# gonewest818/raytrace-clj

Measured on NVIDIA B200. Metric: samples_per_sec, higher is better.
Workload: dtype f32

## Files before the change

raytrace_clj_b200/csrc/rt_api.cu:

```cuda
#include "../../include/raytrace_b200.h"

#include <cuda_runtime.h>
#include <dlfcn.h>
#include <math_constants.h>
#include <nccl.h>

#include <algorithm>
#include <cmath>
#include <cstdio>
#include <cstdlib>
#include <cstring>
#include <atomic>
#include <mutex>
#include <thread>
#include <string>
#include <vector>

#include "rt_bvh_build.cuh"
#include "rt_kernels.cuh"

using namespace rt;

namespace {

constexpr int kR = 4;
constexpr int kBlock = 256;
constexpr int kMinBlocks = 1;
constexpr int kTileCap = 4096;

thread_local std::string g_create_error;

struct DeviceBuffers {
    int dev = 0;
    cudaStream_t stream = nullptr;
    cudaEvent_t ev0 = nullptr, ev1 = nullptr, ev_done = nullptr;
    void* scene_blob = nullptr;
    void* scene_stage = nullptr;
    size_t scene_bytes = 0;
    DevScene sc{};
    float* d_sum = nullptr;
    float* d_mean = nullptr;
    uint8_t* d_rgb8 = nullptr;
    size_t frame_px = 0;
    unsigned long long* d_counters = nullptr;
    struct WaveLane {
        float4* queue = nullptr;
        unsigned long long* best = nullptr;
        uint2* pairs = nullptr;
        uint2* cands = nullptr;
        double* cand_t = nullptr;
        unsigned* cand_count = nullptr;
        WaveState* state = nullptr;
        LaneStatus* h_status = nullptr;
        LaneStatus* d_status = nullptr;
        cudaEvent_t ev_done = nullptr;
        cudaStream_t stream = nullptr;
        cudaStream_t stage_stream = nullptr;
        cudaEvent_t ev_culled = nullptr, ev_shaded = nullptr;
        size_t entries = 0;
        bool best_clean = false;
    } lanes[kMaxLanes];
    cudaEvent_t ev_lane_start = nullptr;
    TraceRec* d_trace = nullptr;
    struct TraceMeta { const char* kernel; int lane, iter; };
    std::vector<TraceMeta> trace_meta;
    void* scratch = nullptr;
    size_t scratch_bytes = 0;
    int sm_count = 0, clock_khz = 0;
    char name[64] = {0};
    float last_ms = 0.f;
    bool timed = false;
    float4* bvh_nodes = nullptr;
    size_t bvh_cap = 0;
    int bvh_builder = 0, bvh_depth = 0;
    long long bvh_build_ns = 0;
    void* bvh_scratch = nullptr;
    size_t bvh_scratch_bytes = 0;
    int* h_bvh_depth = nullptr;
    cudaEvent_t ev_b0 = nullptr, ev_b1 = nullptr;
    void* h_stage = nullptr;
    size_t h_stage_bytes = 0;
    cudaEvent_t ev_r0 = nullptr, ev_r1 = nullptr;
    cudaEvent_t ev_chunk[4] = {};
};

struct NcclApi {
    void* handle = nullptr;
    ncclResult_t (*CommInitAll)(ncclComm_t*, int, const int*) = nullptr;
    ncclResult_t (*CommDestroy)(ncclComm_t) = nullptr;
    ncclResult_t (*Reduce)(const void*, void*, size_t, ncclDataType_t, ncclRedOp_t, int, ncclComm_t, cudaStream_t) = nullptr;
    ncclResult_t (*GroupStart)() = nullptr;
    ncclResult_t (*GroupEnd)() = nullptr;
    const char* (*GetErrorString)(ncclResult_t) = nullptr;
    std::vector<ncclComm_t> comms;
};

}

struct Options {
    int wave_lanes = 2;
    long long wave_capacity = 1ll << 24;
    int cull_claims = 2;
    int cull_ctas_per_sm = 4;
    int cull_shape = 0;
    int light_block = 128;
    long long tail_entries = 1 << 19;
    int tail_ctas_per_sm = 0;
    int tile_records = 1024;
    int direct_spheres = 1;
    int common_origin = 1;
    int reduce = 0;
    int rows = 0;
    int tail_block = 256;
    int tail_rays = 1;
    int tail_solo = 24;
    int tail_lpp = 32;
    int mega_regcap = 0;
    int wave_depth = 2;
    int cull_tc = 1;
    int tc_tiles_per_cta = 0;
    int tc_ctas = 0;
    int bvh_build = 1;
};

struct rt_ctx {
    std::mutex mu;
    std::string err;
    std::vector<DeviceBuffers> devs;
    Options opt;
    bool has_scene = false, has_cam = false;
    int n_spheres = 0;
    int n_total = 0;
    int n_list = 0, n_cull = 0;
    int cull_cap = 0, preloaded = 0;
    int tc_tiles = 0;
    std::vector<std::vector<float>> tc_scratch_rows;
    std::vector<int> tc_row_k;
    int generic = 0;
    int accel = RT_ACCEL_BRUTE_FORCE;
    bool bvh_dirty = true;
    double win_lo = 0.0, win_hi = 0.0;
    std::vector<float> h_c0r, h_c1, h_t0t1;
    std::vector<unsigned> h_flags;
    std::vector<double> h_bs_c0, h_bs_c1, h_bs_r;
    DevCamera cam{};
    std::atomic<uint64_t> n_launches{0};
    std::mutex err_mu;
    bool profile = false;
    double stage_ms[4] = {0, 0, 0, 0};
    double reduce_ms = 0.0;
    std::vector<bool> peer_ok;
    NcclApi nccl;
};

namespace {

int fail(rt_ctx* ctx, int code, const std::string& msg) {
    if (ctx) {
        std::lock_guard<std::mutex> lk(ctx->err_mu);
        ctx->err = msg;
    } else {
        g_create_error = msg;
    }
    return code;
}

#define RT_CUDA(ctx, expr)                                                                          \
    do {                                                                                            \
        cudaError_t e__ = (expr);                                                                   \
        if (e__ != cudaSuccess)                                                                     \
            return fail(ctx, RT_ERR_CUDA, std::string(#expr) + ": " + cudaGetErrorString(e__));     \
    } while (0)

int ensure_scratch(rt_ctx* ctx, DeviceBuffers& d, size_t bytes) {
    if (d.scratch_bytes >= bytes) return RT_OK;
    if (d.scratch) cudaFree(d.scratch);
    d.scratch = nullptr;
    d.scratch_bytes = 0;
    RT_CUDA(ctx, cudaMalloc(&d.scratch, bytes));
    d.scratch_bytes = bytes;
    return RT_OK;
}

int ensure_frame(rt_ctx* ctx, DeviceBuffers& d, size_t px) {
    if (d.frame_px >= px) return RT_OK;
    if (d.d_sum) cudaFree(d.d_sum);
    if (d.d_mean) cudaFree(d.d_mean);
    if (d.d_rgb8) cudaFree(d.d_rgb8);
    d.d_sum = d.d_mean = nullptr;
    d.d_rgb8 = nullptr;
    d.frame_px = 0;
    RT_CUDA(ctx, cudaMalloc(&d.d_sum, px * 3 * sizeof(float)));
    RT_CUDA(ctx, cudaMalloc(&d.d_mean, px * 3 * sizeof(float)));
    RT_CUDA(ctx, cudaMalloc(&d.d_rgb8, px * 3));
    d.frame_px = px;
    return RT_OK;
}


void free_lane(DeviceBuffers::WaveLane& L) {
    if (L.queue) cudaFree(L.queue);
    if (L.best) cudaFree(L.best);
    if (L.pairs) cudaFree(L.pairs);
    if (L.cands) cudaFree(L.cands);
    if (L.cand_t) cudaFree(L.cand_t);
    if (L.cand_count) cudaFree(L.cand_count);
    L.queue = nullptr; L.best = nullptr; L.pairs = nullptr; L.cands = nullptr; L.cand_t = nullptr; L.cand_count = nullptr;
    L.entries = 0;
}

void free_wave(DeviceBuffers& d) {
    for (auto& L : d.lanes) {
        free_lane(L);
        if (L.state) cudaFree(L.state);
        if (L.h_status) cudaFreeHost(L.h_status);
        if (L.ev_done) cudaEventDestroy(L.ev_done);
        if (L.stream) cudaStreamDestroy(L.stream);
        if (L.stage_stream) cudaStreamDestroy(L.stage_stream);
        if (L.ev_culled) cudaEventDestroy(L.ev_culled);
        if (L.ev_shaded) cudaEventDestroy(L.ev_shaded);
        L = DeviceBuffers::WaveLane();
    }
    if (d.ev_lane_start) cudaEventDestroy(d.ev_lane_start);
    d.ev_lane_start = nullptr;
    if (d.d_trace) cudaFree(d.d_trace);
    d.d_trace = nullptr;
}

int ensure_lane(rt_ctx* ctx, DeviceBuffers& d, int lane, size_t entries) {
    DeviceBuffers::WaveLane& L = d.lanes[lane];
    if (!L.state) {
        RT_CUDA(ctx, cudaMalloc(&L.state, sizeof(WaveState)));
        RT_CUDA(ctx, cudaHostAlloc(&L.h_status, sizeof(LaneStatus), cudaHostAllocMapped));
        RT_CUDA(ctx, cudaHostGetDevicePointer((void**)&L.d_status, L.h_status, 0));
        RT_CUDA(ctx, cudaEventCreateWithFlags(&L.ev_done, cudaEventDisableTiming));
        if (lane > 0) RT_CUDA(ctx, cudaStreamCreateWithFlags(&L.stream, cudaStreamNonBlocking));
        int prio_least = 0, prio_greatest = 0;
        RT_CUDA(ctx, cudaDeviceGetStreamPriorityRange(&prio_least, &prio_greatest));
        RT_CUDA(ctx, cudaStreamCreateWithPriority(&L.stage_stream, cudaStreamNonBlocking, prio_greatest));
        RT_CUDA(ctx, cudaEventCreateWithFlags(&L.ev_culled, cudaEventDisableTiming));
        RT_CUDA(ctx, cudaEventCreateWithFlags(&L.ev_shaded, cudaEventDisableTiming));
        if (!d.ev_lane_start) RT_CUDA(ctx, cudaEventCreateWithFlags(&d.ev_lane_start, cudaEventDisableTiming));
    }
    if (L.entries >= entries) return RT_OK;
    free_lane(L);
    RT_CUDA(ctx, cudaMalloc(&L.queue, entries * 2 * 3 * sizeof(float4)));
    RT_CUDA(ctx, cudaMalloc(&L.best, entries * 2 * sizeof(unsigned long long)));
    RT_CUDA(ctx, cudaMalloc(&L.pairs, entries * kPairsPerEntry * sizeof(uint2)));
    const size_t cand_slots = entries * kPairsPerEntry + (size_t)d.sm_count * 8 * 8 * 32;
    RT_CUDA(ctx, cudaMalloc(&L.cands, cand_slots * sizeof(uint2)));
    RT_CUDA(ctx, cudaMalloc(&L.cand_t, cand_slots * sizeof(double)));
    RT_CUDA(ctx, cudaMalloc(&L.cand_count, (size_t)d.sm_count * 8 * 8 * sizeof(unsigned)));
    L.entries = entries;
    L.best_clean = false;
    return RT_OK;
}

size_t align_up(size_t x, size_t a) { return (x + a - 1) / a * a; }

float round_up_f32(double x) {
    float f = (float)x;
    if ((double)f < x) f = nextafterf(f, INFINITY);
    return f;
}

size_t mega_smem_bytes(int cull_cap) { return (size_t)cull_cap * sizeof(float4) + Culler<kR, kBlock>::LIST_BYTES; }

template <typename Kern>
int configure_kernel(rt_ctx* ctx, Kern kern, size_t smem, int* blocks_per_sm) {
    RT_CUDA(ctx, cudaFuncSetAttribute(kern, cudaFuncAttributeMaxDynamicSharedMemorySize, (int)smem));
    int b = 0;
    RT_CUDA(ctx, cudaOccupancyMaxActiveBlocksPerMultiprocessor(&b, kern, kBlock, smem));
    if (b < 1) return fail(ctx, RT_ERR_CUDA, "kernel does not fit on an SM");
    *blocks_per_sm = b;
    return RT_OK;
}

long long env_ll(const char* name, long long dflt) {
    const char* v = getenv(name);
    return (v && *v) ? atoll(v) : dflt;
}
int env_int(const char* name, int dflt) { return (int)env_ll(name, dflt); }

Options options_from_env() {
    Options o;
    o.wave_lanes = env_int("RT_WAVE_LANES", o.wave_lanes);
    o.wave_capacity = env_ll("RT_WAVE_CAPACITY", o.wave_capacity);
    o.cull_claims = env_int("RT_CULL_CLAIMS", o.cull_claims);
    o.cull_ctas_per_sm = env_int("RT_CULL_CTAS_PER_SM", o.cull_ctas_per_sm);
    const char* shape = getenv("RT_CULL_SHAPE");
    if (shape && !strcmp(shape, "128x6")) o.cull_shape = 1;
    if (shape && !strcmp(shape, "256x2")) o.cull_shape = 2;
    o.light_block = env_int("RT_LIGHT_BLOCK", o.light_block);
    o.tail_entries = env_ll("RT_TAIL_ENTRIES", o.tail_entries);
    o.tail_ctas_per_sm = env_int("RT_TAIL_CTAS_PER_SM", o.tail_ctas_per_sm);
    o.tile_records = env_int("RT_TILE_RECORDS", o.tile_records);
    o.direct_spheres = env_int("RT_DIRECT_SPHERES", o.direct_spheres);
    o.common_origin = env_int("RT_COMMON_ORIGIN", o.common_origin);
    o.reduce = env_int("RT_REDUCE", o.reduce);
    o.rows = env_int("RT_ROWS", o.rows);
    o.wave_depth = env_int("RT_WAVE_DEPTH", o.wave_depth);
    o.tail_rays = env_int("RT_TAIL_RAYS", o.tail_rays);
    o.tail_solo = env_int("RT_TAIL_SOLO", o.tail_solo);
    o.tail_lpp = env_int("RT_TAIL_LPP", o.tail_lpp);
    o.tail_block = env_int("RT_TAIL_BLOCK", o.tail_block);
    o.cull_tc = env_int("RT_CULL_TC", o.cull_tc);
    o.tc_tiles_per_cta = env_int("RT_TC_TILES_PER_CTA", o.tc_tiles_per_cta);
    o.tc_ctas = env_int("RT_TC_CTAS", o.tc_ctas);
    o.bvh_build = env_int("RT_BVH_BUILD", o.bvh_build);
    return o;
}

template <int BLOCK, int MINB>
int cull_config(rt_ctx* ctx, size_t* smem, int* bps, void (**kern)(const WaveParams)) {
    *kern = wf_cull<kR, BLOCK, MINB>;
    *smem = (ctx->preloaded ? 2 : 1) * (size_t)ctx->cull_cap * sizeof(float4) + Culler<kR, BLOCK>::LIST_BYTES;
    RT_CUDA(ctx, cudaFuncSetAttribute(*kern, cudaFuncAttributeMaxDynamicSharedMemorySize, (int)*smem));
    RT_CUDA(ctx, cudaOccupancyMaxActiveBlocksPerMultiprocessor(bps, *kern, BLOCK, *smem));
    if (*bps < 1) return fail(ctx, RT_ERR_CUDA, "cull kernel does not fit on an SM");
    return RT_OK;
}

int launch_wave(rt_ctx* ctx, DeviceBuffers& d, const RenderParams& P, unsigned long long, cudaStream_t stream) {
    const Options& opt = ctx->opt;
    void (*cull)(const WaveParams) = nullptr;
    size_t smem = 0;
    int bps = 0, cull_block = 256, rc;
    if (opt.cull_shape == 2) rc = cull_config<256, 2>(ctx, &smem, &bps, &cull);
    else if (opt.cull_shape == 1) { rc = cull_config<128, 6>(ctx, &smem, &bps, &cull); cull_block = 128; }
    else { rc = cull_config<128, 5>(ctx, &smem, &bps, &cull); cull_block = 128; }
    if (rc) return rc;
    const int cull_ctas_env = opt.cull_ctas_per_sm;
    if (cull_ctas_env > 0) bps = std::min(bps, cull_ctas_env);
    const size_t cap_env = (size_t)std::max<long long>(64, opt.wave_capacity);
    const int lanes_env = std::max(1, std::min(kMaxLanes, opt.wave_lanes));
    const int n_lanes = (ctx->profile || P.total_work < 65536) ? 1 : lanes_env;
    const size_t capacity = align_up((size_t)std::min<unsigned long long>(cap_env / n_lanes, (P.total_work + n_lanes - 1) / n_lanes), 32);

    bool done[kMaxLanes] = {};
    const unsigned tail_entries = (unsigned)std::max<long long>(0, opt.tail_entries);
    const bool gen = ctx->generic != 0;
    const bool tail4 = opt.tail_rays == 4;
    const int tail_block = (gen || tail4) ? 256 : (opt.tail_block == 32 || opt.tail_block == 64 || opt.tail_block == 128 ? opt.tail_block : 256);
    const size_t tail_smem = (size_t)ctx->cull_cap * sizeof(float4) +
                             (tail4 ? Culler<4, 256>::LIST_BYTES : (size_t)Culler<1, 256>::LIST_WORDS * tail_block * sizeof(uint32_t));
    int tail_bps = 0;
    void (*k_tail)(const WaveParams) = gen ? wf_tail<256, true, 1> : (tail4 ? wf_tail<256, false, 4> : wf_tail<256, false, 1>);
    if (tail_block == 128) k_tail = wf_tail<128, false, 1>;
    if (tail_block == 64) k_tail = wf_tail<64, false, 1>;
    if (tail_block == 32) k_tail = wf_tail<32, false, 1>;
    void (*k_refine)(const WaveParams) = gen ? wf_refine<true> : wf_refine<false>;
    void (*k_shade)(const WaveParams) = gen ? wf_shade<true> : wf_shade<false>;
    RT_CUDA(ctx, cudaFuncSetAttribute(k_tail, cudaFuncAttributeMaxDynamicSharedMemorySize, (int)tail_smem));
    RT_CUDA(ctx, cudaOccupancyMaxActiveBlocksPerMultiprocessor(&tail_bps, k_tail, tail_block, tail_smem));
    const int tail_auto = (n_lanes > 1 ? 1 : std::max(1, std::min((int)(tail_bps * tail_block / 256), 2))) * (256 / tail_block);
    const int tail_grid = d.sm_count * (opt.tail_ctas_per_sm > 0 ? opt.tail_ctas_per_sm : tail_auto);
    const bool bvh = ctx->accel == RT_ACCEL_BVH;
    void (*k_bvh)(const WaveParams) = gen ? wf_bvh<true> : wf_bvh<false>;
    const bool tail_ok = tail_bps >= 1 && tail_entries > 0 && !ctx->profile && !bvh;
    const bool use_tc = opt.cull_tc != 0 && ctx->tc_tiles > 0 && !bvh && ((ctx->n_list >= tc::MIN_LEAVES && !ctx->generic) || opt.cull_tc == 3);
    const int tc_launch_tiles = std::min(ctx->tc_tiles, (int)tc::MAX_TILES);
    const int tc_slots = tc::slots_for(tc_launch_tiles, 227 * 1024);
    const size_t tc_smem = tc::smem_bytes(tc_launch_tiles, tc_slots);
    if (use_tc) RT_CUDA(ctx, cudaFuncSetAttribute(wf_cull_tc, cudaFuncAttributeMaxDynamicSharedMemorySize, (int)tc_smem));
    const int tc_per_cta = std::max(0, opt.tc_tiles_per_cta);
    const int tc_grid = opt.tc_ctas > 0 ? std::min(opt.tc_ctas, 4 * d.sm_count) : d.sm_count;
    auto launch_tc = [&](const WaveParams& Wl, int per_cta, unsigned ctas, cudaStream_t s_) {
        WaveParams Wt = Wl;
        Wt.claims_per_warp = per_cta;
        Wt.tc_slots = tc_slots;
        for (int t0 = 0, pass = 0; t0 < ctx->tc_tiles; t0 += tc::MAX_TILES, ++pass) {
            Wt.tc_tile0 = t0;
            Wt.tc_launch_tiles = std::min((int)tc::MAX_TILES, ctx->tc_tiles - t0);
            Wt.tc_pass = pass;
            wf_cull_tc<<<ctas, tc::THREADS, tc_smem, s_>>>(Wt);
            if (pass) ctx->n_launches += 1;
        }
    };

    const int light_block = std::max(64, std::min(256, opt.light_block / 32 * 32));
    const int light_grid = d.sm_count * 8 * 256 / light_block;
    const int cull_grid = d.sm_count * bps;
    const int claims_env = std::max(0, opt.cull_claims);
    const int claims = (ctx->profile || !ctx->preloaded || n_lanes < 2 || bvh) ? 0 : claims_env;
    const int cull_warps = cull_block / 32, resident_warps = cull_grid * cull_warps;
    unsigned n_bound[kMaxLanes];
    WaveParams W[kMaxLanes];
    cudaStream_t st[kMaxLanes];
    unsigned long long first = 0;
    for (int l = 0; l < n_lanes; ++l) {
        if ((rc = ensure_lane(ctx, d, l, capacity))) return rc;
        DeviceBuffers::WaveLane& L = d.lanes[l];
        W[l] = WaveParams{};
        W[l].base = P;
        W[l].queue[0] = L.queue;
        W[l].queue[1] = L.queue + 3 * capacity;
        W[l].best_t = L.best;
        W[l].best_key = L.best + L.entries;
        W[l].pairs = L.pairs;
        W[l].cands = L.cands;
        W[l].cand_t = L.cand_t;
        W[l].cand_count = L.cand_count;
        W[l].st = L.state;
        W[l].capacity = (int)capacity;
        W[l].pair_cap = (unsigned)std::min<size_t>(capacity * kPairsPerEntry, 0xfffffff0u);
        W[l].cur = 0;
        W[l].claims_per_warp = claims;
        W[l].resident_warps = claims ? resident_warps : 0;
        W[l].tail_solo = (unsigned)std::max(0, opt.tail_solo);
        W[l].tail_lpp = opt.tail_lpp == 8 ? 8u : (opt.tail_lpp == 16 ? 16u : 32u);
        st[l] = l == 0 ? stream : L.stream;
    }
    static const char* trace_path = getenv("RT_TRACE");
    constexpr int kTraceMax = 8192;
    const bool tracing = trace_path && *trace_path;
    if (tracing) {
        if (!d.d_trace) RT_CUDA(ctx, cudaMalloc(&d.d_trace, kTraceMax * sizeof(TraceRec)));
        static const std::vector<TraceRec> init((size_t)kTraceMax, TraceRec{~0ull, 0ull});
        RT_CUDA(ctx, cudaMemcpyAsync(d.d_trace, init.data(), init.size() * sizeof(TraceRec), cudaMemcpyHostToDevice, stream));
        d.trace_meta.clear();
    }
    auto trace_slot = [&](const char* kernel, int lane, int iter) -> TraceRec* {
        if (!tracing || (int)d.trace_meta.size() >= kTraceMax) return nullptr;
        d.trace_meta.push_back({kernel, lane, iter});
        return d.d_trace + (d.trace_meta.size() - 1);
    };
    int iter_no[kMaxLanes] = {};
    static const bool debug_sync = getenv("RT_DEBUG_SYNC") && *getenv("RT_DEBUG_SYNC") == '1';
    auto dbg = [&](const char* what, int lane, int it) -> int {
        if (!debug_sync) return RT_OK;
        cudaError_t e = cudaDeviceSynchronize();
        if (e != cudaSuccess) return fail(ctx, RT_ERR_CUDA, std::string(what) + " (lane " + std::to_string(lane) + ", iteration " + std::to_string(it) + "): " + cudaGetErrorString(e));
        return RT_OK;
    };
    unsigned count0[kMaxLanes];
    unsigned long long total0 = 0;
    for (int l = 0; l < n_lanes; ++l) {
        count0[l] = (unsigned)std::min<unsigned long long>(capacity, P.total_work - total0);
        total0 += count0[l];
        n_bound[l] = count0[l];
    }
    InitParams I{};
    I.n_lanes = n_lanes;
    I.work_counter = P.work_counter;
    I.counters = P.counters;
    I.total0 = total0;
    I.total_work = P.total_work;
    for (int l = 0; l < n_lanes; ++l) {
        DeviceBuffers::WaveLane& L = d.lanes[l];
        I.st[l] = L.state;
        I.first[l] = first;
        I.count[l] = count0[l];
        first += count0[l];
        if (!L.best_clean) {
            wf_fill_best<<<d.sm_count * 4, 256, 0, stream>>>(L.best, L.best + L.entries, L.entries);
            ctx->n_launches += 1;
        }
        L.best_clean = false;
    }
    wf_init<<<1, 1, 0, stream>>>(I);
    ctx->n_launches += 1;
    RT_CUDA(ctx, cudaGetLastError());
    RT_CUDA(ctx, cudaEventRecord(d.ev_lane_start, stream));
    for (int l = 1; l < n_lanes; ++l) RT_CUDA(ctx, cudaStreamWaitEvent(st[l], d.ev_lane_start, 0));

    const int depth = std::max(1, std::min(16, opt.wave_depth));
    int enq[kMaxLanes] = {}, seen[kMaxLanes] = {};
    bool tailed[kMaxLanes] = {};
    for (int l = 0; l < n_lanes; ++l) {
        DeviceBuffers::WaveLane& L = d.lanes[l];
        memset(L.h_status, 0, sizeof(LaneStatus));
        W[l].status = L.d_status;
        if (count0[l] == 0) done[l] = true;
    }
    std::vector<cudaEvent_t> evs;
    unsigned idle_spins = 0;
    for (;;) {
        bool progressed = false, all_done = true;
        for (int l = 0; l < n_lanes; ++l) {
            if (done[l]) continue;
            all_done = false;
            DeviceBuffers::WaveLane& L = d.lanes[l];
            while (!tailed[l] && enq[l] - seen[l] < depth) {
                cudaEvent_t e[5] = {nullptr, nullptr, nullptr, nullptr, nullptr};
                if (ctx->profile)
                    for (auto& x : e) { RT_CUDA(ctx, cudaEventCreate(&x)); evs.push_back(x); }
                if (ctx->profile) cudaEventRecord(e[0], st[l]);
                W[l].iter = (unsigned)(enq[l] + 1);
                const bool tc_now = use_tc && !(enq[l] == 0 && P.common_origin && opt.cull_tc == 2);
                if (bvh) {
                    W[l].trace = trace_slot("bvh", l, iter_no[l]);
                    k_bvh<<<light_grid, 128, 0, st[l]>>>(W[l]);
                    if (ctx->profile) { cudaEventRecord(e[1], st[l]); cudaEventRecord(e[2], st[l]); cudaEventRecord(e[3], st[l]); }
                    W[l].trace = trace_slot("shade", l, iter_no[l]);
                    k_shade<<<light_grid, light_block, 0, st[l]>>>(W[l]);
                    if (ctx->profile) cudaEventRecord(e[4], st[l]);
                    ctx->n_launches -= 2;
                } else if (claims) {
                    W[l].trace = trace_slot("cull", l, iter_no[l]);
                    if (debug_sync) {
                        WaveState hs{};
                        cudaMemcpy(&hs, W[l].st, sizeof hs, cudaMemcpyDeviceToHost);
                        fprintf(stderr, "lane %d iteration %d cur %d: in flight %u fresh %u | other queue %u %u | mode %u exhausted %u npairs %u\n", l, enq[l], W[l].cur,
                                hs.cnt[W[l].cur][0], hs.cnt[W[l].cur][1], hs.cnt[W[l].cur ^ 1][0], hs.cnt[W[l].cur ^ 1][1], hs.mode, hs.exhausted, hs.npairs);
                    }
                    if (tc_now) {
                        const unsigned tiles = (n_bound[l] + tc::TILE_M - 1) / tc::TILE_M;
                        const unsigned ctas = tc_per_cta ? (tiles + (unsigned)tc_per_cta - 1u) / (unsigned)tc_per_cta : (unsigned)tc_grid;
                        launch_tc(W[l], tc_per_cta, std::max(1u, ctas), st[l]);
                    } else {
                    const unsigned items = n_bound[l] / (32u * kR) + 2u * (unsigned)resident_warps + 8u;
                    const unsigned ctas = (items + (unsigned)(cull_warps * claims) - 1u) / (unsigned)(cull_warps * claims);
                    cull<<<ctas, cull_block, smem, st[l]>>>(W[l]);
                    }
                    if ((rc = dbg(tc_now ? "wf_cull_tc" : "wf_cull", l, enq[l]))) return rc;
                    RT_CUDA(ctx, cudaEventRecord(L.ev_culled, st[l]));
                    RT_CUDA(ctx, cudaStreamWaitEvent(L.stage_stream, L.ev_culled, 0));
                    W[l].trace = trace_slot("refine", l, iter_no[l]);
                    k_refine<<<light_grid, light_block, 0, L.stage_stream>>>(W[l]);
                    if ((rc = dbg("wf_refine", l, enq[l]))) return rc;
                    W[l].trace = trace_slot("tiebreak", l, iter_no[l]);
                    wf_tiebreak<<<light_grid, light_block, 0, L.stage_stream>>>(W[l]);
                    if ((rc = dbg("wf_tiebreak", l, enq[l]))) return rc;
                    W[l].trace = trace_slot("shade", l, iter_no[l]);
                    k_shade<<<light_grid, light_block, 0, L.stage_stream>>>(W[l]);
                    if ((rc = dbg("wf_shade", l, enq[l]))) return rc;
                    RT_CUDA(ctx, cudaEventRecord(L.ev_shaded, L.stage_stream));
                    RT_CUDA(ctx, cudaStreamWaitEvent(st[l], L.ev_shaded, 0));
                } else {
                    W[l].trace = trace_slot("cull", l, iter_no[l]);
                    if (tc_now) {
                        launch_tc(W[l], 0, (unsigned)tc_grid, st[l]);
                    } else {
                        cull<<<cull_grid, cull_block, smem, st[l]>>>(W[l]);
                    }
                    if (ctx->profile) cudaEventRecord(e[1], st[l]);
                    W[l].trace = trace_slot("refine", l, iter_no[l]);
                    k_refine<<<light_grid, light_block, 0, st[l]>>>(W[l]);
                    if (ctx->profile) cudaEventRecord(e[2], st[l]);
                    W[l].trace = trace_slot("tiebreak", l, iter_no[l]);
                    wf_tiebreak<<<light_grid, light_block, 0, st[l]>>>(W[l]);
                    if (ctx->profile) cudaEventRecord(e[3], st[l]);
                    W[l].trace = trace_slot("shade", l, iter_no[l]);
                    k_shade<<<light_grid, light_block, 0, st[l]>>>(W[l]);
                    if (ctx->profile) cudaEventRecord(e[4], st[l]);
                }
                RT_CUDA(ctx, cudaGetLastError());
                W[l].cur ^= 1;
                ++iter_no[l];
                ctx->n_launches += 4;
                ++enq[l];
                progressed = true;
            }
        }
        if (all_done) break;
        for (int l = 0; l < n_lanes; ++l) {
            if (done[l]) continue;
            DeviceBuffers::WaveLane& L = d.lanes[l];
            const volatile LaneStatus* hs = L.h_status;
            const unsigned seq = hs->seq;
            if ((int)seq == seen[l] && hs->mode != MODE_DONE) continue;
            std::atomic_thread_fence(std::memory_order_acquire);
            const unsigned n_next = hs->n_next, n_fresh = hs->n_fresh, exhausted = hs->exhausted, mode = hs->mode;
            if (hs->seq != seq) continue;
            seen[l] = (int)seq;
            progressed = true;
            if (exhausted) n_bound[l] = std::min(n_bound[l], n_next);
            if (mode == MODE_DONE) { done[l] = true; continue; }
            if (tail_ok && !tailed[l] && exhausted && n_fresh == 0 && n_next <= tail_entries) {
                W[l].iter = (unsigned)(enq[l] + 1);
                W[l].trace = trace_slot("tail", l, iter_no[l]);
                k_tail<<<tail_grid, tail_block, tail_smem, st[l]>>>(W[l]);
                if ((rc = dbg("wf_tail", l, enq[l]))) return rc;
                RT_CUDA(ctx, cudaGetLastError());
                ctx->n_launches += 1;
                tailed[l] = true;
            }
        }
        if (!progressed) {
            if (++idle_spins > 200) {
                if (cudaSuccess != cudaPeekAtLastError()) RT_CUDA(ctx, cudaGetLastError());
                if (idle_spins > 20000 && (idle_spins % 1000) == 0) {
                    for (int l = 0; l < n_lanes; ++l)
                        if (!done[l] && cudaStreamQuery(st[l]) == cudaSuccess && d.lanes[l].h_status->seq == (unsigned)seen[l] &&
                            enq[l] > seen[l])
                            return fail(ctx, RT_ERR_CUDA, "wavefront lane finished its queue without reporting status");
                }
                std::this_thread::yield();
            }
        } else {
            idle_spins = 0;
        }
    }
    for (int l = 1; l < n_lanes; ++l) {
        RT_CUDA(ctx, cudaEventRecord(d.lanes[l].ev_done, st[l]));
        RT_CUDA(ctx, cudaStreamWaitEvent(stream, d.lanes[l].ev_done, 0));
    }
    for (int l = 0; l < n_lanes; ++l) d.lanes[l].best_clean = true;
    if (ctx->profile) {
        RT_CUDA(ctx, cudaStreamSynchronize(stream));
        for (size_t i = 0; i + 4 < evs.size(); i += 5)
            for (int sgi = 0; sgi < 4; ++sgi) {
                float ms = 0.f;
                if (cudaEventElapsedTime(&ms, evs[i + sgi], evs[i + sgi + 1]) == cudaSuccess) ctx->stage_ms[sgi] += ms;
            }
        for (auto x : evs) cudaEventDestroy(x);
    }
    return RT_OK;
}

int launch_params(rt_ctx* ctx, DeviceBuffers& d, RenderParams& P, int variant, cudaStream_t stream);

int launch_render(rt_ctx* ctx, DeviceBuffers& d, int nx, int ny, int sample_begin, int sample_count, int row_offset,
                  int row_stride, int max_depth, uint64_t seed, int variant, float* d_sum, cudaStream_t stream) {
    RenderParams P{};
    P.sc = d.sc;
    P.cam = ctx->cam;
    P.nx = nx;
    P.ny = ny;
    P.sample_begin = sample_begin;
    P.sample_count = sample_count;
    P.row_offset = row_offset;
    P.row_stride = row_stride;
    P.rows_in_shard = (ny - row_offset + row_stride - 1) / row_stride;
    P.max_depth = max_depth;
    P.key = make_uint2((uint32_t)seed, (uint32_t)(seed >> 32));
    P.sum = d_sum;
    P.counters = d.d_counters;
    P.work_counter = d.d_counters + DC_COUNT;
    P.total_work = (unsigned long long)sample_count * (unsigned long long)nx * (unsigned long long)P.rows_in_shard;
    if ((sample_begin + sample_count) >= (1 << 24)) return fail(ctx, RT_ERR_ARG, "sample index must stay below 2^24");
    return launch_params(ctx, d, P, variant, stream);
}

int launch_params(rt_ctx* ctx, DeviceBuffers& d, RenderParams& P, int variant, cudaStream_t stream) {
    if (variant != RT_VARIANT_MEGAKERNEL && variant != RT_VARIANT_WAVEFRONT)
        return fail(ctx, RT_ERR_ARG, "unknown render variant");
    if (variant == RT_VARIANT_WAVEFRONT && P.max_depth > 255)
        return fail(ctx, RT_ERR_ARG, "the wavefront variant packs the depth in 8 bits: max_depth <= 255");
    P.sc = d.sc;
    P.cam = ctx->cam;
    P.counters = d.d_counters;
    P.work_counter = d.d_counters + DC_COUNT;
    P.cull_cap = ctx->cull_cap;
    P.preloaded = ctx->preloaded;
    P.common_origin = (ctx->opt.common_origin && (ctx->cam.type == CAM_PINHOLE || ctx->cam.lens_radius == 0.f)) ? 1 : 0;
    RT_CUDA(ctx, cudaMemsetAsync(P.work_counter, 0, sizeof(unsigned long long), stream));
    if (P.total_work == 0) return RT_OK;
    size_t smem = mega_smem_bytes(ctx->cull_cap);
    unsigned long long want = (P.total_work + (unsigned long long)kBlock * kR - 1) / ((unsigned long long)kBlock * kR);
    int bps = 0;
    if (variant == RT_VARIANT_MEGAKERNEL) {
        void (*kern)(const RenderParams) = ctx->generic ? mega_kernel<kR, kBlock, kMinBlocks, true>
                                           : (ctx->opt.mega_regcap ? mega_kernel<kR, kBlock, 2, false> : mega_kernel<kR, kBlock, kMinBlocks, false>);
        int rc = configure_kernel(ctx, kern, smem, &bps);
        if (rc) return rc;
        int grid = (int)std::min<unsigned long long>((unsigned long long)d.sm_count * bps, want);
        if (grid < 1) grid = 1;
        kern<<<grid, kBlock, smem, stream>>>(P);
        RT_CUDA(ctx, cudaGetLastError());
        ctx->n_launches += 1;
        return RT_OK;
    }
    return launch_wave(ctx, d, P, want, stream);
}

void build_cull_records(rt_ctx* ctx, double win_lo, double win_hi, float* cull_all, float* tc_out) {
    const double eps = std::ldexp(1.0, -20), u = std::ldexp(1.0, -24);
    for (int i = 0; i < ctx->n_spheres; ++i) {
        float* cull_a = i < ctx->n_list ? cull_all : cull_all + 4 * (size_t)(ctx->n_cull - ctx->n_list);
        double r = std::fabs(ctx->h_bs_r[(size_t)i]);
        double mid[3], half2 = 0.0, cmax = 0.0;
        const bool moving = (ctx->h_flags[i] & RT_SPHERE_MOVING) != 0;
        for (int c = 0; c < 3; ++c) {
            double p0 = ctx->h_bs_c0[3 * (size_t)i + c];
            if (moving) {
                double p1 = ctx->h_bs_c1[3 * (size_t)i + c], t0 = ctx->h_t0t1[2 * i], t1 = ctx->h_t0t1[2 * i + 1];
                double fa = (win_lo - t0) / (t1 - t0), fb = (win_hi - t0) / (t1 - t0);
                double pa = p0 * (1.0 - fa) + p1 * fa, pb = p0 * (1.0 - fb) + p1 * fb;
                mid[c] = 0.5 * (pa + pb);
                half2 += 0.25 * (pb - pa) * (pb - pa);
            } else {
                mid[c] = p0;
            }
            cmax = std::max(cmax, std::fabs(mid[c]));
        }
        double rb = r + std::sqrt(half2);
        double e = (moving || ctx->generic) ? std::ldexp(1.0, -21) * (cmax + rb) : 0.0;
        double cc = 0.0;
        for (int c = 0; c < 3; ++c) {
            const float neg = (float)(-mid[c]);
            cull_a[4 * i + c] = neg;
            cc += (double)neg * (double)neg;
        }
        double re = rb + e;
        double r2i = re * re * (1.0 + eps) + 48.0 * u * cc + 8.0 * u * re * re;
        cull_a[4 * i + 3] = round_up_f32(r2i - cc);
        if (tc_out && i < ctx->n_list) {
            const double c[3] = {-(double)cull_a[4 * i], -(double)cull_a[4 * i + 1], -(double)cull_a[4 * i + 2]};
            const double Wtc = re * re * (1.0 + eps) + 96.0 * u * cc + 24.0 * u * re * re - cc;
            float row[tc::KTOT];
            tc::sphere_slots(c, Wtc, row);
            ctx->tc_scratch_rows[(size_t)i].assign(row, row + tc::KTOT);
        }
    }
    for (int k = ctx->n_list; k < ctx->n_cull; ++k) {
        cull_all[4 * k] = cull_all[4 * k + 1] = cull_all[4 * k + 2] = 0.f;
        cull_all[4 * k + 3] = -INFINITY;
    }
    if (tc_out) {
        float pad[tc::KTOT];
        tc::padding_slots(pad);
        for (int p = 0; p < ctx->tc_tiles * tc::TILE_N; ++p) {
            const int k = ctx->tc_row_k[(size_t)p];
            const float* row = k >= 0 ? ctx->tc_scratch_rows[(size_t)k].data() : pad;
            float* tile = tc_out + (size_t)(p / tc::TILE_N) * (tc::B_TILE_BYTES / 4);
            for (int q = 0; q < tc::KTOT; ++q) tile[tc::canon_off(tc::TILE_N, p % tc::TILE_N, q) / 4] = row[q];
        }
    }
}

int ensure_window(rt_ctx* ctx, double lo, double hi) {
    if (lo >= ctx->win_lo && hi <= ctx->win_hi) return RT_OK;
    if (!(lo <= hi) || !std::isfinite(lo) || !std::isfinite(hi)) return fail(ctx, RT_ERR_ARG, "ray time is not finite");
    ctx->win_lo = std::min(ctx->win_lo, lo);
    ctx->win_hi = std::max(ctx->win_hi, hi);
    bool any_moving = false;
    for (unsigned f : ctx->h_flags) any_moving |= (f & RT_SPHERE_MOVING) != 0;
    if (!any_moving) return RT_OK;
    ctx->bvh_dirty = true;
    std::vector<float> cull((size_t)(ctx->n_cull + ctx->n_spheres - ctx->n_list) * 4);
    std::vector<float> tcr((size_t)ctx->tc_tiles * (tc::B_TILE_BYTES / 4));
    build_cull_records(ctx, ctx->win_lo, ctx->win_hi, cull.data(), tcr.empty() ? nullptr : tcr.data());
    if (cull.empty()) return RT_OK;
    for (auto& d : ctx->devs) {
        RT_CUDA(ctx, cudaSetDevice(d.dev));
        RT_CUDA(ctx, cudaDeviceSynchronize());
        RT_CUDA(ctx, cudaMemcpy((void*)d.sc.cull_a, cull.data(), cull.size() * sizeof(float), cudaMemcpyHostToDevice));
        if (!tcr.empty()) RT_CUDA(ctx, cudaMemcpy((void*)d.sc.cull_tc, tcr.data(), tcr.size() * sizeof(float), cudaMemcpyHostToDevice));
    }
    cudaSetDevice(ctx->devs[0].dev);
    return RT_OK;
}

struct BuildLeaf {
    float lo[3], hi[3];
    float c[3];
    int k;
};
int bvh_build_node(std::vector<BuildLeaf>& L, int begin, int end, std::vector<float>& nodes, float lo[3], float hi[3], int depth,
                   int* max_depth) {
    if (end - begin == 1) {
        for (int a = 0; a < 3; ++a) { lo[a] = L[(size_t)begin].lo[a]; hi[a] = L[(size_t)begin].hi[a]; }
        *max_depth = std::max(*max_depth, depth);
        return ~L[(size_t)begin].k;
    }
    float cmin[3] = {INFINITY, INFINITY, INFINITY}, cmax[3] = {-INFINITY, -INFINITY, -INFINITY};
    for (int i = begin; i < end; ++i)
        for (int a = 0; a < 3; ++a) { cmin[a] = std::min(cmin[a], L[(size_t)i].c[a]); cmax[a] = std::max(cmax[a], L[(size_t)i].c[a]); }
    int axis = 0;
    for (int a = 1; a < 3; ++a) if (cmax[a] - cmin[a] > cmax[axis] - cmin[axis]) axis = a;
    const int mid = begin + (end - begin + 1) / 2;
    std::nth_element(L.begin() + begin, L.begin() + mid, L.begin() + end,
                     [axis](const BuildLeaf& x, const BuildLeaf& y) { return x.c[axis] < y.c[axis]; });
    const size_t me = nodes.size() / 16;
    nodes.resize(nodes.size() + 16, 0.f);
    float llo[3], lhi[3], rlo[3], rhi[3];
    const int left = bvh_build_node(L, begin, mid, nodes, llo, lhi, depth + 1, max_depth);
    const int right = bvh_build_node(L, mid, end, nodes, rlo, rhi, depth + 1, max_depth);
    float* N = nodes.data() + 16 * me;
    N[0] = llo[0]; N[1] = llo[1]; N[2] = llo[2]; N[3] = lhi[0]; N[4] = lhi[1]; N[5] = lhi[2];
    N[6] = rlo[0]; N[7] = rlo[1]; N[8] = rlo[2]; N[9] = rhi[0]; N[10] = rhi[1]; N[11] = rhi[2];
    memcpy(&N[12], &left, 4);
    memcpy(&N[13], &right, 4);
    for (int a = 0; a < 3; ++a) { lo[a] = std::min(llo[a], rlo[a]); hi[a] = std::max(lhi[a], rhi[a]); }
    return (int)me;
}

int ensure_bvh_nodes(rt_ctx* ctx, DeviceBuffers& d, size_t bytes) {
    if (d.bvh_cap >= bytes) return RT_OK;
    if (d.bvh_nodes) cudaFree(d.bvh_nodes);
    d.bvh_nodes = nullptr;
    d.bvh_cap = 0;
    RT_CUDA(ctx, cudaMalloc(&d.bvh_nodes, bytes));
    d.bvh_cap = bytes;
    return RT_OK;
}

int bvh_build_host(rt_ctx* ctx) {
    const int n = ctx->n_list;
    std::vector<BuildLeaf> L((size_t)n);
    for (int k = 0; k < n; ++k) {
        BuildLeaf& b = L[(size_t)k];
        b.k = k;
        const bool moving = (ctx->h_flags[(size_t)k] & RT_SPHERE_MOVING) != 0;
        const double r = std::fabs(ctx->h_bs_r[(size_t)k]);
        for (int a = 0; a < 3; ++a) {
            double pa = ctx->h_bs_c0[3 * (size_t)k + a], pb = pa;
            if (moving) {
                const double p0 = ctx->h_bs_c0[3 * (size_t)k + a], p1 = ctx->h_bs_c1[3 * (size_t)k + a];
                const double t0 = ctx->h_t0t1[2 * k], t1 = ctx->h_t0t1[2 * k + 1];
                const double fa = (ctx->win_lo - t0) / (t1 - t0), fb = (ctx->win_hi - t0) / (t1 - t0);
                pa = p0 * (1.0 - fa) + p1 * fa;
                pb = p0 * (1.0 - fb) + p1 * fb;
            }
            const double lo = std::min(pa, pb) - r, hi = std::max(pa, pb) + r;
            const double m = 1e-6 * (std::fabs(lo) + std::fabs(hi) + r) + 1e-30;
            b.lo[a] = nextafterf((float)(lo - m), -INFINITY);
            b.hi[a] = nextafterf((float)(hi + m), INFINITY);
            b.c[a] = (float)(0.5 * (lo + hi));
        }
    }
    std::vector<float> nodes;
    nodes.reserve(16 * (size_t)std::max(1, n));
    float lo[3], hi[3];
    int depth = 1;
    if (n == 1) {
        nodes.assign(16, 0.f);
        for (int a = 0; a < 3; ++a) { nodes[(size_t)a] = nodes[6 + (size_t)a] = L[0].lo[a]; nodes[3 + (size_t)a] = nodes[9 + (size_t)a] = L[0].hi[a]; }
        const int leaf = ~0;
        memcpy(&nodes[12], &leaf, 4);
        memcpy(&nodes[13], &leaf, 4);
    } else {
        const int root = bvh_build_node(L, 0, n, nodes, lo, hi, 0, &depth);
        if (root != 0) return fail(ctx, RT_ERR_STATE, "BVH build: the root is not node 0");
    }
    for (auto& d : ctx->devs) {
        RT_CUDA(ctx, cudaSetDevice(d.dev));
        RT_CUDA(ctx, cudaDeviceSynchronize());
        const size_t bytes = nodes.size() * sizeof(float);
        if (int rc = ensure_bvh_nodes(ctx, d, bytes)) return rc;
        RT_CUDA(ctx, cudaMemcpy(d.bvh_nodes, nodes.data(), bytes, cudaMemcpyHostToDevice));
        d.sc.bvh = d.bvh_nodes;
        d.sc.bvh_nodes = (int)(nodes.size() / 16);
        d.bvh_builder = 0;
        d.bvh_depth = depth;
        d.bvh_build_ns = 0;
    }
    cudaSetDevice(ctx->devs[0].dev);
    return RT_OK;
}

int bvh_enqueue_device(rt_ctx* ctx, DeviceBuffers& d) {
    const int n = ctx->n_list;
    const int n_nodes = std::max(1, n - 1);
    RT_CUDA(ctx, cudaSetDevice(d.dev));
    RT_CUDA(ctx, cudaDeviceSynchronize());
    if (int rc = ensure_bvh_nodes(ctx, d, (size_t)n_nodes * 4 * sizeof(float4))) return rc;
    size_t sort_bytes = 0;
    RT_CUDA(ctx, cub::DeviceRadixSort::SortPairs(nullptr, sort_bytes, (const unsigned long long*)nullptr, (unsigned long long*)nullptr,
                                                 (const int*)nullptr, (int*)nullptr, n, 0, 3 * (int)kMortonAxisBits, d.stream));
    size_t off = 0;
    auto take = [&](size_t bytes) { const size_t o = off; off = align_up(off + bytes, 256); return o; };
    const size_t n_ = (size_t)n;
    const size_t o_c0 = take(n_ * 3 * 8), o_c1 = take(n_ * 3 * 8), o_r = take(n_ * 8), o_t = take(n_ * 2 * 4), o_fl = take(n_ * 4);
    const size_t o_box = take(n_ * 6 * 4), o_cb = take(6 * 4), o_code = take(n_ * 8), o_code2 = take(n_ * 8);
    const size_t o_leaf = take(n_ * 4), o_leaf2 = take(n_ * 4), o_par = take((2 * n_ - 1) * 4), o_arr = take((size_t)n_nodes * 4);
    const size_t o_h = take((size_t)n_nodes * 4), o_depth = take(4), o_sort = take(sort_bytes);
    if (d.bvh_scratch_bytes < off) {
        if (d.bvh_scratch) cudaFree(d.bvh_scratch);
        d.bvh_scratch = nullptr;
        d.bvh_scratch_bytes = 0;
        RT_CUDA(ctx, cudaMalloc(&d.bvh_scratch, off));
        d.bvh_scratch_bytes = off;
    }
    if (!d.h_bvh_depth) {
        RT_CUDA(ctx, cudaHostAlloc(&d.h_bvh_depth, sizeof(int), cudaHostAllocDefault));
        RT_CUDA(ctx, cudaEventCreate(&d.ev_b0));
        RT_CUDA(ctx, cudaEventCreate(&d.ev_b1));
    }
    char* S = (char*)d.bvh_scratch;
    const cudaStream_t st = d.stream;
    BvhLeafInput in{(const double*)(S + o_c0), (const double*)(S + o_c1), (const double*)(S + o_r), (const float*)(S + o_t),
                    (const unsigned*)(S + o_fl)};
    float* boxes = (float*)(S + o_box);
    unsigned* cb = (unsigned*)(S + o_cb);
    int* depth = (int*)(S + o_depth);
    RT_CUDA(ctx, cudaEventRecord(d.ev_b0, st));
    RT_CUDA(ctx, cudaMemcpyAsync(S + o_c0, ctx->h_bs_c0.data(), n_ * 3 * 8, cudaMemcpyHostToDevice, st));
    RT_CUDA(ctx, cudaMemcpyAsync(S + o_c1, ctx->h_bs_c1.data(), n_ * 3 * 8, cudaMemcpyHostToDevice, st));
    RT_CUDA(ctx, cudaMemcpyAsync(S + o_r, ctx->h_bs_r.data(), n_ * 8, cudaMemcpyHostToDevice, st));
    RT_CUDA(ctx, cudaMemcpyAsync(S + o_t, ctx->h_t0t1.data(), n_ * 2 * 4, cudaMemcpyHostToDevice, st));
    RT_CUDA(ctx, cudaMemcpyAsync(S + o_fl, ctx->h_flags.data(), n_ * 4, cudaMemcpyHostToDevice, st));
    RT_CUDA(ctx, cudaMemsetAsync(cb, 0xff, 3 * 4, st));
    RT_CUDA(ctx, cudaMemsetAsync(cb + 3, 0, 3 * 4, st));
    const int grid = (n + 255) / 256;
    bvh_leaf_boxes<<<grid, 256, 0, st>>>(in, n, ctx->win_lo, ctx->win_hi, boxes, cb);
    if (n == 1) {
        bvh_single_leaf<<<1, 32, 0, st>>>(boxes, d.bvh_nodes, depth);
    } else {
        unsigned long long* code = (unsigned long long*)(S + o_code);
        unsigned long long* code2 = (unsigned long long*)(S + o_code2);
        int* leaf = (int*)(S + o_leaf);
        int* leaf2 = (int*)(S + o_leaf2);
        int* parent = (int*)(S + o_par);
        bvh_morton<<<grid, 256, 0, st>>>(boxes, n, cb, code, leaf);
        RT_CUDA(ctx, cub::DeviceRadixSort::SortPairs(S + o_sort, sort_bytes, code, code2, leaf, leaf2, n, 0, 3 * (int)kMortonAxisBits, st));
        RT_CUDA(ctx, cudaMemsetAsync(S + o_arr, 0, (size_t)n_nodes * 4, st));
        bvh_hierarchy<<<(n - 1 + 255) / 256, 256, 0, st>>>(code2, leaf2, n, d.bvh_nodes, parent);
        bvh_fit<<<grid, 256, 0, st>>>(boxes, parent, n, d.bvh_nodes, (unsigned*)(S + o_arr), (int*)(S + o_h), depth);
    }
    RT_CUDA(ctx, cudaGetLastError());
    RT_CUDA(ctx, cudaMemcpyAsync(d.h_bvh_depth, depth, sizeof(int), cudaMemcpyDeviceToHost, st));
    RT_CUDA(ctx, cudaEventRecord(d.ev_b1, st));
    d.sc.bvh_nodes = n_nodes;
    return RT_OK;
}
// ... 749 lines not shown
        int bad = RT_OK;
        for (int g = 0; g < G; ++g)
            if (rcs[(size_t)g] && !bad) bad = rcs[(size_t)g];
        if (bad) {
            for (auto& dv : ctx->devs) { cudaSetDevice(dv.dev); cudaDeviceSynchronize(); }
            cudaSetDevice(ctx->devs[0].dev);
            return bad;
        }
    }
    DeviceBuffers& root = ctx->devs[0];
    RT_CUDA(ctx, cudaSetDevice(root.dev));
    ResolveParams P{};
    P.sum = root.d_sum; P.n_peers = 0; P.nx = nx; P.ny = ny; P.nr = nsamples;
    P.rgb8 = out_rgb8 ? root.d_rgb8 : nullptr;
    P.mean = out_linear_rgb ? root.d_mean : nullptr;
    P.sum_out = nullptr;
    const int total = nx * ny * 3;
    if (use_nccl) {
        NcclApi& N = ctx->nccl;
        for (int g = 1; g < G; ++g) RT_CUDA(ctx, cudaStreamWaitEvent(root.stream, ctx->devs[g].ev_done, 0));
        RT_CUDA(ctx, cudaEventRecord(root.ev_r0, root.stream));
        ncclResult_t nr = N.GroupStart();
        for (int g = 0; g < G && nr == ncclSuccess; ++g)
            nr = N.Reduce(ctx->devs[g].d_sum, ctx->devs[g].d_sum, (size_t)total, ncclFloat, ncclSum, 0, N.comms[(size_t)g], ctx->devs[g].stream);
        const ncclResult_t ge = N.GroupEnd();
        if (nr == ncclSuccess) nr = ge;
        if (nr != ncclSuccess) {
            for (auto& dv : ctx->devs) { cudaSetDevice(dv.dev); cudaDeviceSynchronize(); }
            cudaSetDevice(root.dev);
            return fail(ctx, RT_ERR_NCCL, std::string("ncclReduce: ") + N.GetErrorString(nr));
        }
        RT_CUDA(ctx, cudaSetDevice(root.dev));
        RT_CUDA(ctx, cudaEventRecord(root.ev_r1, root.stream));
        resolve_kernel<<<(total + 255) / 256, 256, 0, root.stream>>>(P);
    } else {
        for (int g = 1; g < G; ++g) {
            DeviceBuffers& d = ctx->devs[g];
            RT_CUDA(ctx, cudaStreamWaitEvent(root.stream, d.ev_done, 0));
            if (ctx->peer_ok[g]) {
                P.peers[P.n_peers++] = d.d_sum;
            } else {
                if ((rc = ensure_scratch(ctx, root, (size_t)(G - 1) * px * 3 * sizeof(float)))) return rc;
                float* stage = (float*)root.scratch + (size_t)(g - 1) * px * 3;
                RT_CUDA(ctx, cudaMemcpyPeerAsync(stage, root.dev, d.d_sum, d.dev, px * 3 * sizeof(float), root.stream));
                P.peers[P.n_peers++] = stage;
            }
        }
        RT_CUDA(ctx, cudaEventRecord(root.ev_r0, root.stream));
        resolve_kernel<<<(total + 255) / 256, 256, 0, root.stream>>>(P);
        RT_CUDA(ctx, cudaEventRecord(root.ev_r1, root.stream));
    }
    RT_CUDA(ctx, cudaGetLastError());
    ctx->n_launches += 1;
    auto host_pinned = [](const void* p) {
        cudaPointerAttributes at{};
        if (cudaPointerGetAttributes(&at, p) != cudaSuccess) { cudaGetLastError(); return false; }
        return at.type == cudaMemoryTypeHost;
    };
    const size_t b_lin = out_linear_rgb ? align_up(px * 3 * sizeof(float), 256) : 0, b_rgb = out_rgb8 ? px * 3 : 0;
    if (b_lin + b_rgb) {
        if ((rc = ensure_stage(ctx, root, b_lin + b_rgb))) return rc;
        constexpr int NCH = 4;
        for (auto& e : root.ev_chunk)
            if (!e) RT_CUDA(ctx, cudaEventCreateWithFlags(&e, cudaEventDisableTiming));
        struct Part { char* dst; const char* src; char* stage; size_t bytes; };
        const Part parts[2] = {{(char*)out_linear_rgb, (const char*)root.d_mean, (char*)root.h_stage, out_linear_rgb ? px * 3 * sizeof(float) : 0},
                               {(char*)out_rgb8, (const char*)root.d_rgb8, (char*)root.h_stage + b_lin, b_rgb}};
        for (const Part& pt : parts) {
            if (!pt.bytes) continue;
            if (host_pinned(pt.dst)) {
                RT_CUDA(ctx, cudaMemcpyAsync(pt.dst, pt.src, pt.bytes, cudaMemcpyDeviceToHost, root.stream));
                continue;
            }
            const size_t step = align_up((pt.bytes + NCH - 1) / NCH, 4096);
            for (int c = 0; c < NCH; ++c) {
                const size_t off = std::min(pt.bytes, (size_t)c * step), len = std::min(pt.bytes - off, step);
                if (len) RT_CUDA(ctx, cudaMemcpyAsync(pt.stage + off, pt.src + off, len, cudaMemcpyDeviceToHost, root.stream));
                RT_CUDA(ctx, cudaEventRecord(root.ev_chunk[c], root.stream));
            }
            for (int c = 0; c < NCH; ++c) {
                const size_t off = std::min(pt.bytes, (size_t)c * step), len = std::min(pt.bytes - off, step);
                RT_CUDA(ctx, cudaEventSynchronize(root.ev_chunk[c]));
                if (len) memcpy(pt.dst + off, pt.stage + off, len);
            }
        }
    }
    RT_CUDA(ctx, cudaStreamSynchronize(root.stream));
    for (int g = 1; g < G; ++g) {
        RT_CUDA(ctx, cudaSetDevice(ctx->devs[g].dev));
        RT_CUDA(ctx, cudaStreamSynchronize(ctx->devs[g].stream));
    }
    cudaSetDevice(root.dev);
    if (G > 1) {
        float ms = 0.f;
        if (cudaEventElapsedTime(&ms, root.ev_r0, root.ev_r1) == cudaSuccess) ctx->reduce_ms += ms;
        cudaGetLastError();
    }
    return RT_OK;
}

int rt_host_alloc(rt_ctx* ctx, size_t bytes, void** out) {
    if (!out || bytes == 0) return ctx ? fail(ctx, RT_ERR_ARG, "rt_host_alloc: bad arguments") : RT_ERR_ARG;
    *out = nullptr;
    if (ctx && !ctx->devs.empty()) cudaSetDevice(ctx->devs[0].dev);
    const cudaError_t e = cudaHostAlloc(out, bytes, cudaHostAllocPortable);
    if (e != cudaSuccess) {
        cudaGetLastError();
        return fail(ctx, RT_ERR_CUDA, std::string("cudaHostAlloc: ") + cudaGetErrorString(e));
    }
    return RT_OK;
}

int rt_host_free(rt_ctx* ctx, void* p) {
    if (!p) return RT_OK;
    const cudaError_t e = cudaFreeHost(p);
    if (e != cudaSuccess) {
        cudaGetLastError();
        return fail(ctx, RT_ERR_CUDA, std::string("cudaFreeHost: ") + cudaGetErrorString(e));
    }
    return RT_OK;
}

int rt_trace_paths(rt_ctx* ctx, int nx, int ny, int n, const int32_t* pixel, const int32_t* sample, int max_depth, uint64_t seed,
                   int variant, float* out_radiance, int32_t* out_nrays, int32_t* out_term, int log_bounces, rt_path_bounce* out_log) {
    int rc = check_ready(ctx);
    if (rc) return rc;
    std::lock_guard<std::mutex> lk(ctx->mu);
    if ((rc = check_camera_times(ctx))) return rc;
    if (nx <= 0 || ny <= 0 || n < 0 || max_depth < 0 || log_bounces < 0 || (n > 0 && (!pixel || !sample || !out_radiance || !out_nrays || !out_term)) ||
        (log_bounces > 0 && n > 0 && !out_log))
        return fail(ctx, RT_ERR_ARG, "bad trace_paths arguments");
    if ((long long)nx * ny > 0x7fffffffLL / 3) return fail(ctx, RT_ERR_ARG, "image too large");
    if (n == 0) return RT_OK;
    for (int q = 0; q < n; ++q)
        if (pixel[q] < 0 || pixel[q] >= nx * ny || sample[q] < 0 || sample[q] >= (1 << 24))
            return fail(ctx, RT_ERR_ARG, "pixel / sample index out of range");
    static_assert(sizeof(rt_path_bounce) == sizeof(PathBounce) && sizeof(PathBounce) == 40, "rt_path_bounce layout");
    DeviceBuffers& d = ctx->devs[0];
    RT_CUDA(ctx, cudaSetDevice(d.dev));
    const size_t b_i = align_up((size_t)n * 4, 256), b_f = align_up((size_t)n * 12, 256), b_l = align_up((size_t)n * log_bounces * sizeof(PathBounce), 256);
    char* buf = nullptr;
    RT_CUDA(ctx, cudaMalloc(&buf, 4 * b_i + b_f + b_l + 256));
    int* d_pix = (int*)buf;
    int* d_smp = (int*)(buf + b_i);
    int* d_nr = (int*)(buf + 2 * b_i);
    int* d_term = (int*)(buf + 3 * b_i);
    float* d_rad = (float*)(buf + 4 * b_i);
    PathBounce* d_log = log_bounces > 0 ? (PathBounce*)(buf + 4 * b_i + b_f) : nullptr;
    auto cleanup = [&](int code) { cudaStreamSynchronize(d.stream); cudaFree(buf); return code; };
    cudaError_t e;
    if ((e = cudaMemcpyAsync(d_pix, pixel, (size_t)n * 4, cudaMemcpyHostToDevice, d.stream)) != cudaSuccess ||
        (e = cudaMemcpyAsync(d_smp, sample, (size_t)n * 4, cudaMemcpyHostToDevice, d.stream)) != cudaSuccess ||
        (e = cudaMemsetAsync(d_nr, 0, 2 * b_i + b_f, d.stream)) != cudaSuccess ||
        (d_log && (e = cudaMemsetAsync(d_log, 0xff, (size_t)n * log_bounces * sizeof(PathBounce), d.stream)) != cudaSuccess))
        return cleanup(fail(ctx, RT_ERR_CUDA, std::string("trace_paths upload: ") + cudaGetErrorString(e)));
    RenderParams P{};
    P.nx = nx; P.ny = ny;
    P.sample_begin = 0; P.sample_count = 1;
    P.row_offset = 0; P.row_stride = 1; P.rows_in_shard = ny;
    P.max_depth = max_depth;
    P.key = make_uint2((uint32_t)seed, (uint32_t)(seed >> 32));
    P.sum = d_rad;
    P.total_work = (unsigned long long)n;
    P.path_pixel = d_pix; P.path_sample = d_smp; P.path_nrays = d_nr; P.path_term = d_term;
    P.path_log = d_log; P.path_log_n = log_bounces;
    if ((rc = launch_params(ctx, d, P, variant, d.stream))) return cleanup(rc);
    if ((e = cudaMemcpyAsync(out_radiance, d_rad, (size_t)n * 12, cudaMemcpyDeviceToHost, d.stream)) != cudaSuccess ||
        (e = cudaMemcpyAsync(out_nrays, d_nr, (size_t)n * 4, cudaMemcpyDeviceToHost, d.stream)) != cudaSuccess ||
        (e = cudaMemcpyAsync(out_term, d_term, (size_t)n * 4, cudaMemcpyDeviceToHost, d.stream)) != cudaSuccess ||
        (d_log && (e = cudaMemcpyAsync(out_log, d_log, (size_t)n * log_bounces * sizeof(PathBounce), cudaMemcpyDeviceToHost, d.stream)) != cudaSuccess) ||
        (e = cudaStreamSynchronize(d.stream)) != cudaSuccess)
        return cleanup(fail(ctx, RT_ERR_CUDA, std::string("trace_paths: ") + cudaGetErrorString(e)));
    if (out_log)
        for (size_t q = 0; q < (size_t)n * log_bounces; ++q)
            if (out_log[q].hit_id == -1 && std::isnan(out_log[q].t)) { memset(&out_log[q], 0, sizeof(rt_path_bounce)); out_log[q].hit_id = -2; }
    d.timed = false;
    return cleanup(RT_OK);
}

int rt_sample_device(rt_ctx* ctx, int kind, int n, uint64_t seed, float* out) {
    if (!ctx) return RT_ERR_ARG;
    std::lock_guard<std::mutex> lk(ctx->mu);
    if ((kind != 0 && kind != 1) || n < 0 || (n > 0 && !out)) return fail(ctx, RT_ERR_ARG, "bad sample_device arguments");
    if (n == 0) return RT_OK;
    DeviceBuffers& d = ctx->devs[0];
    RT_CUDA(ctx, cudaSetDevice(d.dev));
    const int dim = kind == 0 ? 3 : 2;
    int rc;
    if ((rc = ensure_scratch(ctx, d, (size_t)n * dim * 4))) return rc;
    sampler_kernel<<<(n + 255) / 256, 256, 0, d.stream>>>(kind, n, make_uint2((uint32_t)seed, (uint32_t)(seed >> 32)), (float*)d.scratch);
    RT_CUDA(ctx, cudaGetLastError());
    RT_CUDA(ctx, cudaMemcpyAsync(out, d.scratch, (size_t)n * dim * 4, cudaMemcpyDeviceToHost, d.stream));
    RT_CUDA(ctx, cudaStreamSynchronize(d.stream));
    return RT_OK;
}

int rt_trace_primary(rt_ctx* ctx, int n, const float* origins, const float* dirs, const float* times, double tmin,
                     double tmax, double* out_t, int32_t* out_id) {
    int rc = check_ready(ctx);
    if (rc) return rc;
    std::lock_guard<std::mutex> lk(ctx->mu);
    if (n < 0 || (n > 0 && (!origins || !dirs || !out_t || !out_id))) return fail(ctx, RT_ERR_ARG, "bad trace arguments");
    if (!(tmin >= 0.0)) return fail(ctx, RT_ERR_ARG, "tmin must be >= 0: the cull discards spheres behind the origin");
    if (n == 0) return RT_OK;
    {
        double lo = 0.0, hi = 0.0;
        if (times) {
            lo = INFINITY; hi = -INFINITY;
            for (int i = 0; i < n; ++i) { lo = std::min(lo, (double)times[i]); hi = std::max(hi, (double)times[i]); }
        }
        if ((rc = ensure_window(ctx, lo, hi))) return rc;
    }
    DeviceBuffers& d = ctx->devs[0];
    RT_CUDA(ctx, cudaSetDevice(d.dev));
    size_t b_o = align_up((size_t)n * 12, 256), b_t = align_up((size_t)n * 4, 256), b_ot = align_up((size_t)n * 8, 256);
    if ((rc = ensure_scratch(ctx, d, 2 * b_o + 2 * b_t + b_ot))) return rc;
    char* base = (char*)d.scratch;
    float* d_o = (float*)base;
    float* d_d = (float*)(base + b_o);
    float* d_tm = (float*)(base + 2 * b_o);
    int* d_id = (int*)(base + 2 * b_o + b_t);
    double* d_t = (double*)(base + 2 * b_o + 2 * b_t);
    RT_CUDA(ctx, cudaMemcpyAsync(d_o, origins, (size_t)n * 12, cudaMemcpyHostToDevice, d.stream));
    RT_CUDA(ctx, cudaMemcpyAsync(d_d, dirs, (size_t)n * 12, cudaMemcpyHostToDevice, d.stream));
    if (times) RT_CUDA(ctx, cudaMemcpyAsync(d_tm, times, (size_t)n * 4, cudaMemcpyHostToDevice, d.stream));
    if (ctx->accel == RT_ACCEL_BVH) {
        if ((rc = ensure_bvh(ctx))) return rc;
        TraceParamsB B{};
        B.sc = d.sc; B.n = n; B.origins = d_o; B.dirs = d_d; B.times = times ? d_tm : nullptr;
        B.tmin = tmin; B.tmax = tmax; B.out_t = d_t; B.out_id = d_id;
        B.stats = nullptr;
        if (ctx->generic) trace_bvh_kernel<true><<<(n + 127) / 128, 128, 0, d.stream>>>(B);
        else trace_bvh_kernel<false><<<(n + 127) / 128, 128, 0, d.stream>>>(B);
        RT_CUDA(ctx, cudaGetLastError());
        RT_CUDA(ctx, cudaMemcpyAsync(out_t, d_t, (size_t)n * 8, cudaMemcpyDeviceToHost, d.stream));
        RT_CUDA(ctx, cudaMemcpyAsync(out_id, d_id, (size_t)n * 4, cudaMemcpyDeviceToHost, d.stream));
        RT_CUDA(ctx, cudaStreamSynchronize(d.stream));
        return RT_OK;
    }
    TraceParams P{};
    P.sc = d.sc; P.n = n; P.origins = d_o; P.dirs = d_d; P.times = times ? d_tm : nullptr;
    P.tmin = tmin; P.tmax = tmax; P.out_t = d_t; P.out_id = d_id; P.cull_cap = ctx->cull_cap; P.preloaded = ctx->preloaded;
    void (*kern)(const TraceParams) = ctx->generic ? trace_kernel<kR, kBlock, true> : trace_kernel<kR, kBlock, false>;
    size_t smem = mega_smem_bytes(ctx->cull_cap);
    int bps = 0;
    if ((rc = configure_kernel(ctx, kern, smem, &bps))) return rc;
    int want = (int)(((long long)n + kBlock * kR - 1) / (kBlock * kR));
    int grid = std::max(1, std::min(d.sm_count * bps, want));
    kern<<<grid, kBlock, smem, d.stream>>>(P);
    RT_CUDA(ctx, cudaGetLastError());
    RT_CUDA(ctx, cudaMemcpyAsync(out_t, d_t, (size_t)n * 8, cudaMemcpyDeviceToHost, d.stream));
    RT_CUDA(ctx, cudaMemcpyAsync(out_id, d_id, (size_t)n * 4, cudaMemcpyDeviceToHost, d.stream));
    RT_CUDA(ctx, cudaStreamSynchronize(d.stream));
    return RT_OK;
}

int rt_cull_check(rt_ctx* ctx, int n, const float* origins, const float* dirs, const float* times, double tmin, double tmax,
                  uint64_t out[3]) {
    int rc = check_ready(ctx);
    if (rc) return rc;
    std::lock_guard<std::mutex> lk(ctx->mu);
    if (n < 0 || !out || (n > 0 && (!origins || !dirs))) return fail(ctx, RT_ERR_ARG, "bad cull_check arguments");
    if (!(tmin >= 0.0)) return fail(ctx, RT_ERR_ARG, "tmin must be >= 0: the cull discards spheres behind the origin");
    out[0] = out[1] = out[2] = 0;
    if (n == 0) return RT_OK;
    {
        double lo = 0.0, hi = 0.0;
        if (times) {
            lo = INFINITY; hi = -INFINITY;
            for (int i = 0; i < n; ++i) { lo = std::min(lo, (double)times[i]); hi = std::max(hi, (double)times[i]); }
        }
        if ((rc = ensure_window(ctx, lo, hi))) return rc;
    }
    DeviceBuffers& d = ctx->devs[0];
    RT_CUDA(ctx, cudaSetDevice(d.dev));
    size_t b_o = align_up((size_t)n * 12, 256), b_t = align_up((size_t)n * 4, 256);
    if ((rc = ensure_scratch(ctx, d, 2 * b_o + b_t + 256))) return rc;
    char* base = (char*)d.scratch;
    float* d_o = (float*)base;
    float* d_d = (float*)(base + b_o);
    float* d_tm = (float*)(base + 2 * b_o);
    unsigned long long* d_out = (unsigned long long*)(base + 2 * b_o + b_t);
    RT_CUDA(ctx, cudaMemcpyAsync(d_o, origins, (size_t)n * 12, cudaMemcpyHostToDevice, d.stream));
    RT_CUDA(ctx, cudaMemcpyAsync(d_d, dirs, (size_t)n * 12, cudaMemcpyHostToDevice, d.stream));
    if (times) RT_CUDA(ctx, cudaMemcpyAsync(d_tm, times, (size_t)n * 4, cudaMemcpyHostToDevice, d.stream));
    RT_CUDA(ctx, cudaMemsetAsync(d_out, 0, 3 * sizeof(unsigned long long), d.stream));
    if (ctx->opt.cull_tc && ctx->tc_tiles > 0) {
        const size_t cap = align_up(std::max<size_t>((size_t)n, 1u << 18), 128);
        if ((rc = ensure_lane(ctx, d, 0, cap))) return rc;
        DeviceBuffers::WaveLane& L = d.lanes[0];
        L.best_clean = false;
        const int words = (ctx->n_cull + 31) / 32;
        unsigned* d_mask = nullptr;
        RT_CUDA(ctx, cudaMalloc(&d_mask, (size_t)n * words * sizeof(unsigned)));
        RT_CUDA(ctx, cudaMemsetAsync(d_mask, 0, (size_t)n * words * sizeof(unsigned), d.stream));
        WaveParams W{};
        W.base.sc = d.sc;
        W.base.cam = ctx->cam;
        W.base.counters = d.d_counters;
        W.base.work_counter = d.d_counters + DC_COUNT;
        W.base.max_depth = 1;
        W.queue[0] = L.queue;
        W.queue[1] = L.queue + 3 * L.entries;
        W.best_t = L.best;
        W.best_key = L.best + L.entries;
        W.pairs = L.pairs;
        W.cands = L.cands;
        W.cand_t = L.cand_t;
        W.cand_count = L.cand_count;
        W.st = L.state;
        W.capacity = (int)L.entries;
        W.pair_cap = (unsigned)std::min<size_t>(L.entries * kPairsPerEntry, 0xfffffff0u);
        wf_fill_best<<<d.sm_count * 4, 256, 0, d.stream>>>(L.best, L.best + L.entries, L.entries);
#ifdef RT_TC_CHECK
        RT_CUDA(ctx, cudaMemsetAsync(L.pairs, 0xDD, (size_t)W.pair_cap * sizeof(uint2), d.stream));
#endif
        tc_check_fill<<<(n + 127) / 128, 128, 0, d.stream>>>(W, n, d_o, d_d, times ? d_tm : nullptr);
        const int launch_tiles = std::min(ctx->tc_tiles, (int)tc::MAX_TILES);
        W.tc_slots = tc::slots_for(launch_tiles, 227 * 1024);
        const size_t tc_smem = tc::smem_bytes(launch_tiles, W.tc_slots);
        RT_CUDA(ctx, cudaFuncSetAttribute(wf_cull_tc, cudaFuncAttributeMaxDynamicSharedMemorySize, (int)tc_smem));
        for (int t0 = 0, pass = 0; t0 < ctx->tc_tiles; t0 += tc::MAX_TILES, ++pass) {
            W.tc_tile0 = t0;
            W.tc_launch_tiles = std::min((int)tc::MAX_TILES, ctx->tc_tiles - t0);
            W.tc_pass = pass;
            wf_cull_tc<<<d.sm_count, tc::THREADS, tc_smem, d.stream>>>(W);
        }
        tc_check_mark<<<d.sm_count * 4, 256, 0, d.stream>>>(W, d_mask, words);
        tc_check_compare<<<(n + 127) / 128, 128, 0, d.stream>>>(W, n, tmin, tmax, d_mask, words, d_out);
        cudaError_t e = cudaStreamSynchronize(d.stream);
        cudaFree(d_mask);
        if (e != cudaSuccess) return fail(ctx, RT_ERR_CUDA, std::string("tensor-core cull check: ") + cudaGetErrorString(e));
    } else {
        cull_check_kernel<<<(n + 127) / 128, 128, 0, d.stream>>>(d.sc, n, d_o, d_d, times ? d_tm : nullptr, tmin, tmax, d_out);
    }
    RT_CUDA(ctx, cudaGetLastError());
    unsigned long long h[3];
    RT_CUDA(ctx, cudaMemcpyAsync(h, d_out, sizeof(h), cudaMemcpyDeviceToHost, d.stream));
    RT_CUDA(ctx, cudaStreamSynchronize(d.stream));
    for (int i = 0; i < 3; ++i) out[i] = h[i];
    return RT_OK;
}

int rt_generate_rays(rt_ctx* ctx, int n, int nx, int ny, const int32_t* ij, const int32_t* s, uint64_t seed,
                     float* out_origin, float* out_dir, float* out_time, float* out_rand) {
    if (!ctx) return RT_ERR_ARG;
    std::lock_guard<std::mutex> lk(ctx->mu);
    if (!ctx->has_cam) return fail(ctx, RT_ERR_STATE, "rt_set_camera has not been called");
    if (n < 0 || nx <= 0 || ny <= 0 || (n > 0 && (!ij || !s || !out_origin || !out_dir || !out_time)))
        return fail(ctx, RT_ERR_ARG, "bad generate_rays arguments");
    if (n == 0) return RT_OK;
    DeviceBuffers& d = ctx->devs[0];
    RT_CUDA(ctx, cudaSetDevice(d.dev));
    size_t b_ij = align_up((size_t)n * 8, 256), b_s = align_up((size_t)n * 4, 256), b_v = align_up((size_t)n * 12, 256),
           b_r = align_up((size_t)n * 20, 256);
    int rc;
    if ((rc = ensure_scratch(ctx, d, b_ij + 2 * b_s + 2 * b_v + b_r))) return rc;
    char* base = (char*)d.scratch;
    int* d_ij = (int*)base;
    int* d_s = (int*)(base + b_ij);
    float* d_o = (float*)(base + b_ij + b_s);
    float* d_d = (float*)(base + b_ij + b_s + b_v);
    float* d_t = (float*)(base + b_ij + b_s + 2 * b_v);
    float* d_r = (float*)(base + b_ij + 2 * b_s + 2 * b_v);
    RT_CUDA(ctx, cudaMemcpyAsync(d_ij, ij, (size_t)n * 8, cudaMemcpyHostToDevice, d.stream));
    RT_CUDA(ctx, cudaMemcpyAsync(d_s, s, (size_t)n * 4, cudaMemcpyHostToDevice, d.stream));
    genrays_kernel<<<(n + 255) / 256, 256, 0, d.stream>>>(ctx->cam, n, nx, ny, d_ij, d_s,
                                                         make_uint2((uint32_t)seed, (uint32_t)(seed >> 32)), d_o, d_d, d_t,
                                                         out_rand ? d_r : nullptr);
    RT_CUDA(ctx, cudaGetLastError());
    RT_CUDA(ctx, cudaMemcpyAsync(out_origin, d_o, (size_t)n * 12, cudaMemcpyDeviceToHost, d.stream));
    RT_CUDA(ctx, cudaMemcpyAsync(out_dir, d_d, (size_t)n * 12, cudaMemcpyDeviceToHost, d.stream));
    RT_CUDA(ctx, cudaMemcpyAsync(out_time, d_t, (size_t)n * 4, cudaMemcpyDeviceToHost, d.stream));
    if (out_rand) RT_CUDA(ctx, cudaMemcpyAsync(out_rand, d_r, (size_t)n * 20, cudaMemcpyDeviceToHost, d.stream));
    RT_CUDA(ctx, cudaStreamSynchronize(d.stream));
    return RT_OK;
}

int rt_shade_batch(rt_ctx* ctx, int n, const float* origins, const float* dirs, const float* times, const int32_t* hit_id,
                   const double* hit_t, const float* ball, const float* u01v, float* out_origin, float* out_dir,
                   float* out_atten, float* out_emitted, int32_t* out_flags) {
    int rc = check_ready(ctx);
    if (rc) return rc;
    std::lock_guard<std::mutex> lk(ctx->mu);
    if (n < 0 || (n > 0 && (!origins || !dirs || !hit_id || !hit_t || !ball || !u01v || !out_origin || !out_dir ||
                            !out_atten || !out_emitted || !out_flags)))
        return fail(ctx, RT_ERR_ARG, "bad shade_batch arguments");
    if (n == 0) return RT_OK;
    DeviceBuffers& d = ctx->devs[0];
    RT_CUDA(ctx, cudaSetDevice(d.dev));
    size_t b3 = align_up((size_t)n * 12, 256), b1 = align_up((size_t)n * 4, 256), b8 = align_up((size_t)n * 8, 256);
    if ((rc = ensure_scratch(ctx, d, 7 * b3 + 4 * b1 + b8))) return rc;
    char* p = (char*)d.scratch;
    float* d_o = (float*)p; p += b3;
    float* d_d = (float*)p; p += b3;
    float* d_ball = (float*)p; p += b3;
    float* d_oo = (float*)p; p += b3;
    float* d_od = (float*)p; p += b3;
    float* d_oa = (float*)p; p += b3;
    float* d_oe = (float*)p; p += b3;
    float* d_tm = (float*)p; p += b1;
    float* d_u = (float*)p; p += b1;
    int* d_id = (int*)p; p += b1;
    int* d_fl = (int*)p; p += b1;
    double* d_ht = (double*)p;
    RT_CUDA(ctx, cudaMemcpyAsync(d_o, origins, (size_t)n * 12, cudaMemcpyHostToDevice, d.stream));
    RT_CUDA(ctx, cudaMemcpyAsync(d_d, dirs, (size_t)n * 12, cudaMemcpyHostToDevice, d.stream));
    RT_CUDA(ctx, cudaMemcpyAsync(d_ball, ball, (size_t)n * 12, cudaMemcpyHostToDevice, d.stream));
    if (times) RT_CUDA(ctx, cudaMemcpyAsync(d_tm, times, (size_t)n * 4, cudaMemcpyHostToDevice, d.stream));
    RT_CUDA(ctx, cudaMemcpyAsync(d_u, u01v, (size_t)n * 4, cudaMemcpyHostToDevice, d.stream));
    RT_CUDA(ctx, cudaMemcpyAsync(d_id, hit_id, (size_t)n * 4, cudaMemcpyHostToDevice, d.stream));
    RT_CUDA(ctx, cudaMemcpyAsync(d_ht, hit_t, (size_t)n * 8, cudaMemcpyHostToDevice, d.stream));
    shade_kernel<<<(n + 255) / 256, 256, 0, d.stream>>>(d.sc, n, d_o, d_d, times ? d_tm : nullptr, d_id, d_ht, d_ball, d_u,
                                                       d_oo, d_od, d_oa, d_oe, d_fl);
    RT_CUDA(ctx, cudaGetLastError());
    RT_CUDA(ctx, cudaMemcpyAsync(out_origin, d_oo, (size_t)n * 12, cudaMemcpyDeviceToHost, d.stream));
    RT_CUDA(ctx, cudaMemcpyAsync(out_dir, d_od, (size_t)n * 12, cudaMemcpyDeviceToHost, d.stream));
    RT_CUDA(ctx, cudaMemcpyAsync(out_atten, d_oa, (size_t)n * 12, cudaMemcpyDeviceToHost, d.stream));
    RT_CUDA(ctx, cudaMemcpyAsync(out_emitted, d_oe, (size_t)n * 12, cudaMemcpyDeviceToHost, d.stream));
    RT_CUDA(ctx, cudaMemcpyAsync(out_flags, d_fl, (size_t)n * 4, cudaMemcpyDeviceToHost, d.stream));
    RT_CUDA(ctx, cudaStreamSynchronize(d.stream));
    return RT_OK;
}

int rt_measure_fp32_peak(rt_ctx* ctx, double* out_ffma_tflops, double* out_ffma2_tflops) {
    if (!ctx) return RT_ERR_ARG;
    std::lock_guard<std::mutex> lk(ctx->mu);
    DeviceBuffers& d = ctx->devs[0];
    RT_CUDA(ctx, cudaSetDevice(d.dev));
    const int blocks = d.sm_count * 8, threads = 256, iters = 1 << 15;
    int rc;
    if ((rc = ensure_scratch(ctx, d, (size_t)blocks * threads * 4))) return rc;
    float* out = (float*)d.scratch;
    double best[2] = {0, 0};
    for (int variant = 0; variant < 2; ++variant) {
        for (int rep = 0; rep < 4; ++rep) {
            RT_CUDA(ctx, cudaEventRecord(d.ev0, d.stream));
            if (variant == 0) ffma_peak_kernel<false><<<blocks, threads, 0, d.stream>>>(out, iters, 1.0000001f, 1e-7f);
            else ffma_peak_kernel<true><<<blocks, threads, 0, d.stream>>>(out, iters, 1.0000001f, 1e-7f);
            RT_CUDA(ctx, cudaGetLastError());
            RT_CUDA(ctx, cudaEventRecord(d.ev1, d.stream));
            RT_CUDA(ctx, cudaEventSynchronize(d.ev1));
            float ms = 0;
            RT_CUDA(ctx, cudaEventElapsedTime(&ms, d.ev0, d.ev1));
            double flops = 2.0 * 16.0 * (double)iters * (double)blocks * threads;
            if (rep > 0) best[variant] = std::max(best[variant], flops / (ms * 1e-3) / 1e12);
        }
    }
    if (out_ffma_tflops) *out_ffma_tflops = best[0];
    if (out_ffma2_tflops) *out_ffma2_tflops = best[1];
    d.timed = false;
    return RT_OK;
}

int rt_get_counters(rt_ctx* ctx, uint64_t out[RT_CTR_COUNT]) {
    if (!ctx || !out) return RT_ERR_ARG;
    std::lock_guard<std::mutex> lk(ctx->mu);
    unsigned long long dc[DC_COUNT];
    uint64_t total[DC_COUNT] = {0};
    float max_ms = 0.f;
    for (auto& d : ctx->devs) {
        RT_CUDA(ctx, cudaSetDevice(d.dev));
        RT_CUDA(ctx, cudaDeviceSynchronize());
        RT_CUDA(ctx, cudaMemcpy(dc, d.d_counters, sizeof(dc), cudaMemcpyDeviceToHost));
        for (int i = 0; i < DC_COUNT; ++i) total[i] += dc[i];
        if (!d.trace_meta.empty() && d.d_trace && getenv("RT_TRACE")) {
            std::vector<TraceRec> rec(d.trace_meta.size());
            RT_CUDA(ctx, cudaMemcpy(rec.data(), d.d_trace, rec.size() * sizeof(TraceRec), cudaMemcpyDeviceToHost));
            unsigned long long t0 = ~0ull;
            for (auto& r : rec) if (r.t_end) t0 = std::min(t0, r.t_start);
            if (FILE* f = fopen(getenv("RT_TRACE"), "a")) {
                fprintf(f, "# device %d, %zu launches: kernel lane iteration start_us end_us duration_us (%%globaltimer, relative to the first kernel)\n", d.dev, rec.size());
                for (size_t i = 0; i < rec.size(); ++i) {
                    if (!rec[i].t_end) continue;
                    fprintf(f, "%-9s %d %3d %10.1f %10.1f %9.1f\n", d.trace_meta[i].kernel, d.trace_meta[i].lane, d.trace_meta[i].iter,
                            (rec[i].t_start - t0) * 1e-3, (rec[i].t_end - t0) * 1e-3, (rec[i].t_end - rec[i].t_start) * 1e-3);
                }
                fclose(f);
            }
            d.trace_meta.clear();
        }
        if (d.timed) {
            float ms = 0.f;
            if (cudaEventElapsedTime(&ms, d.ev0, d.ev1) == cudaSuccess) d.last_ms = ms;
            cudaGetLastError();
        }
        max_ms = std::max(max_ms, d.last_ms);
    }
    cudaSetDevice(ctx->devs[0].dev);
    memset(out, 0, sizeof(uint64_t) * RT_CTR_COUNT);
    out[RT_CTR_RAYS] = total[DC_RAYS];
    out[RT_CTR_SPHERE_TESTS] = total[DC_RAYS] * (uint64_t)ctx->n_spheres;
    out[RT_CTR_SAMPLES] = total[DC_SAMPLES];
    out[RT_CTR_TERM_LIGHT] = total[DC_TERM_LIGHT];
    out[RT_CTR_TERM_ABSORB] = total[DC_TERM_ABSORB];
    out[RT_CTR_TERM_DEPTH] = total[DC_TERM_DEPTH];
    out[RT_CTR_TERM_MISS] = total[DC_TERM_MISS];
    out[RT_CTR_KERNEL_NS] = (uint64_t)((double)max_ms * 1e6);
    out[RT_CTR_CANDIDATES] = total[DC_CANDIDATES];
    out[RT_CTR_DIRECT_TESTS] = total[DC_DIRECT];
    out[RT_CTR_BVH_NODE_TESTS] = total[DC_BVH_NODES];
    if (ctx->accel == RT_ACCEL_BVH) out[RT_CTR_SPHERE_TESTS] = total[DC_CANDIDATES] + total[DC_DIRECT];
    out[RT_CTR_KERNEL_LAUNCHES] = ctx->n_launches.load();
    out[RT_CTR_CULL_NS] = (uint64_t)(ctx->stage_ms[0] * 1e6);
    out[RT_CTR_REFINE_NS] = (uint64_t)(ctx->stage_ms[1] * 1e6);
    out[RT_CTR_TIEBREAK_NS] = (uint64_t)(ctx->stage_ms[2] * 1e6);
    out[RT_CTR_SHADE_NS] = (uint64_t)(ctx->stage_ms[3] * 1e6);
    out[RT_CTR_REDUCE_NS] = (uint64_t)(ctx->reduce_ms * 1e6);
    return RT_OK;
}

int rt_reset_counters(rt_ctx* ctx) {
    if (!ctx) return RT_ERR_ARG;
    std::lock_guard<std::mutex> lk(ctx->mu);
    for (auto& d : ctx->devs) {
        RT_CUDA(ctx, cudaSetDevice(d.dev));
        RT_CUDA(ctx, cudaDeviceSynchronize());
        RT_CUDA(ctx, cudaMemset(d.d_counters, 0, (DC_COUNT + 1) * sizeof(unsigned long long)));
    }
    cudaSetDevice(ctx->devs[0].dev);
    ctx->n_launches = 0;
    for (double& x : ctx->stage_ms) x = 0.0;
    ctx->reduce_ms = 0.0;
    return RT_OK;
}

int rt_set_profile(rt_ctx* ctx, int on) {
    if (!ctx) return RT_ERR_ARG;
    std::lock_guard<std::mutex> lk(ctx->mu);
    ctx->profile = on != 0;
    return RT_OK;
}

}
```

raytrace_clj_b200/csrc/rt_cull_tc.cuh:

```cuda

namespace tc {

constexpr int EW = 16;
constexpr int PG = 1;
constexpr int PW = 4 * PG;
constexpr int THREADS = (EW + 1 + PW) * 32;
constexpr int MAX_SLOTS = 4;
constexpr int TILE_M = 128;
constexpr int TILE_N = 256;
constexpr int KTOT = 32;
constexpr int A_BYTES = TILE_M * KTOT * 4;
constexpr int B_TILE_BYTES = TILE_N * KTOT * 4;
constexpr int MAX_TILES = 4;
constexpr int MIN_LEAVES = 160;
constexpr int CAND_CAP = 256;
constexpr int PAIR_CHUNK = 64;
constexpr float RAY_DEFLATE = 1.0f - 5.0e-6f;
constexpr float DEAD = -1.0e30f;

__host__ __device__ inline size_t canon_off(int rows, int r, int k) {
    return (size_t)(k / 4) * ((size_t)rows * 16) + (size_t)(r / 8) * 128 + (size_t)(r % 8) * 16 + (size_t)(k % 4) * 4;
}
inline size_t smem_bytes(int tiles, int slots) {
    return (size_t)tiles * B_TILE_BYTES + (size_t)tiles * TILE_N * (16 + 4) + (size_t)slots * (A_BYTES + TILE_M * 32) + (size_t)EW * CAND_CAP * 4 + 1024;
}
inline int slots_for(int tiles, size_t smem_limit) {
    int s = MAX_SLOTS;
    while (s > 2 && smem_bytes(tiles, s) > smem_limit) --s;
    return s;
}

__device__ __forceinline__ uint32_t smem_u32(const void* p) { return (uint32_t)__cvta_generic_to_shared(p); }
__device__ __forceinline__ void mbar_init(uint64_t* bar, int count) {
    asm volatile("mbarrier.init.shared::cta.b64 [%0], %1;" ::"r"(smem_u32(bar)), "r"(count) : "memory");
}
__device__ __forceinline__ void mbar_arrive(uint64_t* bar) {
    asm volatile("mbarrier.arrive.shared::cta.b64 _, [%0];" ::"r"(smem_u32(bar)) : "memory");
}
__device__ __forceinline__ bool mbar_try_wait(uint64_t* bar, uint32_t parity) {
    uint32_t ok;
    asm volatile("{\n .reg .pred p;\n mbarrier.try_wait.parity.shared::cta.b64 p, [%1], %2;\n selp.u32 %0, 1, 0, p;\n}"
                 : "=r"(ok) : "r"(smem_u32(bar)), "r"(parity) : "memory");
    return ok != 0;
}
__device__ __forceinline__ void mbar_wait(uint64_t* bar, uint32_t parity) {
    for (unsigned spin = 0; spin < 0x40000000u; ++spin)
        if (mbar_try_wait(bar, parity)) return;
    __trap();
}
__device__ __forceinline__ uint64_t make_desc(uint32_t saddr, uint32_t lbo_bytes, uint32_t sbo_bytes) {
    return (uint64_t)((saddr >> 4) & 0x3fffu) | ((uint64_t)((lbo_bytes >> 4) & 0x3fffu) << 16) | ((uint64_t)((sbo_bytes >> 4) & 0x3fffu) << 32) |
           (1ull << 46);
}
#ifndef RT_TC_NBLK
#define RT_TC_NBLK 1
#endif
constexpr int NBLK = RT_TC_NBLK;
constexpr int BLOCK_N = TILE_N / NBLK;
constexpr int BLOCK_WARPS = EW / NBLK;
constexpr uint32_t IDESC = (1u << 4) | (2u << 7) | (2u << 10) | ((uint32_t)(BLOCK_N >> 3) << 17) | ((uint32_t)(TILE_M >> 4) << 24);
__device__ __forceinline__ void mma_tf32(uint32_t d_tmem, uint64_t adesc, uint64_t bdesc, uint32_t accumulate) {
    asm volatile("{\n .reg .pred p;\n setp.ne.b32 p, %4, 0;\n tcgen05.mma.cta_group::1.kind::tf32 [%0], %1, %2, %3, p;\n}"
                 ::"r"(d_tmem), "l"(adesc), "l"(bdesc), "r"(IDESC), "r"(accumulate) : "memory");
}
__device__ __forceinline__ void mma_commit(uint64_t* bar) {
    asm volatile("tcgen05.commit.cta_group::1.mbarrier::arrive::one.shared::cluster.b64 [%0];" ::"r"(smem_u32(bar)) : "memory");
}
#define RT_TMEM_LD32(taddr, v)                                                                                                \
    asm volatile("tcgen05.ld.sync.aligned.32x32b.x32.b32 "                                                                   \
                 "{%0, %1, %2, %3, %4, %5, %6, %7, %8, %9, %10, %11, %12, %13, %14, %15, "                                   \
                 "%16, %17, %18, %19, %20, %21, %22, %23, %24, %25, %26, %27, %28, %29, %30, %31}, [%32];"                   \
                 : "=r"(v[0]), "=r"(v[1]), "=r"(v[2]), "=r"(v[3]), "=r"(v[4]), "=r"(v[5]), "=r"(v[6]), "=r"(v[7]),           \
                   "=r"(v[8]), "=r"(v[9]), "=r"(v[10]), "=r"(v[11]), "=r"(v[12]), "=r"(v[13]), "=r"(v[14]), "=r"(v[15]),     \
                   "=r"(v[16]), "=r"(v[17]), "=r"(v[18]), "=r"(v[19]), "=r"(v[20]), "=r"(v[21]), "=r"(v[22]), "=r"(v[23]),   \
                   "=r"(v[24]), "=r"(v[25]), "=r"(v[26]), "=r"(v[27]), "=r"(v[28]), "=r"(v[29]), "=r"(v[30]), "=r"(v[31])    \
                 : "r"(taddr))
__device__ __forceinline__ void tmem_wait_ld() { asm volatile("tcgen05.wait::ld.sync.aligned;" ::: "memory"); }
__device__ __forceinline__ void fence_before() { asm volatile("tcgen05.fence::before_thread_sync;" ::: "memory"); }
__device__ __forceinline__ void fence_after() { asm volatile("tcgen05.fence::after_thread_sync;" ::: "memory"); }
__device__ __forceinline__ void fence_async_smem() { asm volatile("fence.proxy.async.shared::cta;" ::: "memory"); }

__host__ __device__ inline float tf32_rn(float x) {
#ifdef __CUDA_ARCH__
    return __uint_as_float((__float_as_uint(x) + 0x1000u) & 0xffffe000u);
#else
    uint32_t b; memcpy(&b, &x, 4); b = (b + 0x1000u) & 0xffffe000u; memcpy(&x, &b, 4); return x;
#endif
}
__device__ __forceinline__ void split2(float x, float& hi, float& lo) {
    hi = tf32_rn(x);
    lo = tf32_rn(x - hi);
}

inline void sphere_slots(const double c[3], double W, float out[KTOT]) {
    auto sp2 = [](double x, float& hi, float& lo) { hi = tf32_rn((float)x); lo = tf32_rn((float)(x - (double)hi)); };
    float wh = tf32_rn((float)W), wl = tf32_rn((float)(W - (double)wh)), wl2 = tf32_rn((float)(W - (double)wh - (double)wl));
    float ch[3], cl[3], dh[3], dl[3], eh[3], el[3];
    for (int i = 0; i < 3; ++i) { sp2(c[i], ch[i], cl[i]); sp2(c[i] * c[i], dh[i], dl[i]); }
    sp2(2.0 * c[0] * c[1], eh[0], el[0]); sp2(2.0 * c[0] * c[2], eh[1], el[1]); sp2(2.0 * c[1] * c[2], eh[2], el[2]);
    const float s[KTOT] = {1.f, 1.f, wh, wl, ch[0], cl[0], ch[0], wl2, ch[1], cl[1], ch[1], el[2], ch[2], cl[2], ch[2], eh[2],
                           dh[0], dl[0], dh[0], dh[1], dl[1], dh[1], dh[2], dl[2], dh[2], eh[0], el[0], eh[0], eh[1], el[1], eh[1], eh[2]};
    for (int k = 0; k < KTOT; ++k) out[k] = s[k];
}
inline void padding_slots(float out[KTOT]) {
    for (int k = 0; k < KTOT; ++k) out[k] = 0.f;
    out[0] = 1.f;
    out[2] = DEAD;
}

struct Smem {
    float* B;
    float4* rec;
    int* row_k;
    unsigned char* A0;
    float4* ray0;
    uint32_t* cand;
    uint64_t* a_ready;
    uint64_t* a_free;
    uint64_t* ray_free;
    uint64_t* d_full;
    uint64_t* d_empty;
    int* tile_of;
    uint32_t* tmem_base;
    unsigned* cand_n;
    __device__ __forceinline__ float* A(unsigned s) const { return reinterpret_cast<float*>(A0 + (size_t)s * A_BYTES); }
    __device__ __forceinline__ float4* ray(unsigned s) const { return ray0 + (size_t)s * TILE_M * 2; }
};
__device__ __forceinline__ Smem carve(unsigned char* base, int tiles, int slots) {
    Smem S;
    S.B = reinterpret_cast<float*>(base);
    unsigned char* p = base + (size_t)tiles * B_TILE_BYTES;
    S.rec = reinterpret_cast<float4*>(p);
    p += (size_t)tiles * TILE_N * 16;
    S.row_k = reinterpret_cast<int*>(p);
    p += (size_t)tiles * TILE_N * 4;
    S.A0 = p;
    p += (size_t)slots * A_BYTES;
    S.ray0 = reinterpret_cast<float4*>(p);
    p += (size_t)slots * TILE_M * 32;
    S.cand = reinterpret_cast<uint32_t*>(p);
    p += (size_t)EW * CAND_CAP * 4;
    uint64_t* bars = reinterpret_cast<uint64_t*>(p);
    S.a_ready = bars; S.a_free = bars + MAX_SLOTS; S.ray_free = bars + 2 * MAX_SLOTS;
    S.d_full = bars + 3 * MAX_SLOTS; S.d_empty = bars + 3 * MAX_SLOTS + 2 * NBLK;
    int* ints = reinterpret_cast<int*>(bars + 3 * MAX_SLOTS + 4 * NBLK);
    S.tile_of = ints;
    S.tmem_base = reinterpret_cast<uint32_t*>(ints + MAX_SLOTS);
    S.cand_n = reinterpret_cast<unsigned*>(ints + MAX_SLOTS + 4);
    return S;
}

}

#ifdef RT_TC_CHECK
#define TC_CHECK(cond, what, a, b) do { if (!(cond)) { printf("wf_cull_tc check failed: %s (%u, %u) block %u thread %u\n", what, (unsigned)(a), (unsigned)(b), blockIdx.x, threadIdx.x); __trap(); } } while (0)
#else
#define TC_CHECK(cond, what, a, b)
#endif

__device__ __forceinline__ void tc_produce_ray(const WaveParams& W, const tc::Smem& S, int slot, int rl, bool live, unsigned v, unsigned n_g,
                                               unsigned p0, unsigned long long gen_base, int cur) {
    const RenderParams& P = W.base;
    float f[tc::KTOT];
    float4 r0, r1;
    if (live) {
        float4* qc = cur ? W.queue[1] : W.queue[0];
        float4 a, b;
        if (v >= n_g && W.tc_pass != 0) {
            const size_t e = (size_t)(p0 + (v - n_g));
            a = qc[3 * e];
            b = qc[3 * e + 1];
        } else if (v >= n_g) {
            float4 c;
            float4* q = qc + 3 * (size_t)(p0 + (v - n_g));
            TC_CHECK(p0 + (v - n_g) < (unsigned)W.capacity, "fresh entry", p0 + (v - n_g), W.capacity);
            TC_CHECK(gen_base + (v - n_g) < P.total_work, "work item", (unsigned)(gen_base + (v - n_g)), (unsigned)P.total_work);
            make_path(P, gen_base + (v - n_g), a, b, c);
            q[0] = a; q[1] = b; q[2] = c;
        } else {
            TC_CHECK(v < (unsigned)W.capacity, "entry in flight", v, W.capacity);
            a = qc[3 * (size_t)v];
            b = qc[3 * (size_t)v + 1];
        }
        const float aa = fmaf(b.z, b.z, fmaf(b.y, b.y, b.x * b.x));
        const float inv = rsqrtf(aa);
        const float qq = fmaf(a.z, a.z, fmaf(a.y, a.y, a.x * a.x));
        {
            const float s = inv * ((1.0f + 0.5f * CULL_EPS) * 0.70710678118654752f);
            const float hx = b.x * s, hy = b.y * s, hz = b.z * s;
            r0 = make_float4(hx, hy, hz, fmaf(a.z, hz, fmaf(a.y, hy, a.x * hx)));
            r1 = make_float4(-2.0f * a.x, -2.0f * a.y, -2.0f * a.z, qq * RAY_DEFLATE);
        }
        const float s = inv * (1.0f + 0.5f * CULL_EPS);
        const float hx = b.x * s, hy = b.y * s, hz = b.z * s;
        const float Pd = fmaf(a.z, hz, fmaf(a.y, hy, a.x * hx));
        const float g0 = fmaf(Pd, Pd, -(qq * tc::RAY_DEFLATE));
        const float gx = 2.0f * fmaf(-Pd, hx, a.x), gy = 2.0f * fmaf(-Pd, hy, a.y), gz = 2.0f * fmaf(-Pd, hz, a.z);
        float h_, l_;
        tc::split2(g0, h_, l_); f[0] = h_; f[1] = l_;
        f[2] = 1.f; f[3] = 1.f; f[7] = 1.f;
        tc::split2(gx, h_, l_); f[4] = h_; f[5] = h_; f[6] = l_;
        tc::split2(gy, h_, l_); f[8] = h_; f[9] = h_; f[10] = l_;
        tc::split2(gz, h_, l_); f[12] = h_; f[13] = h_; f[14] = l_;
        tc::split2(hx * hx, h_, l_); f[16] = h_; f[17] = h_; f[18] = l_;
        tc::split2(hy * hy, h_, l_); f[19] = h_; f[20] = h_; f[21] = l_;
        tc::split2(hz * hz, h_, l_); f[22] = h_; f[23] = h_; f[24] = l_;
        tc::split2(hx * hy, h_, l_); f[25] = h_; f[26] = h_; f[27] = l_;
        tc::split2(hx * hz, h_, l_); f[28] = h_; f[29] = h_; f[30] = l_;
        tc::split2(hy * hz, h_, l_); f[31] = h_; f[11] = h_; f[15] = l_;
    } else {
#pragma unroll
        for (int k = 0; k < tc::KTOT; ++k) f[k] = 0.f;
        f[0] = tc::DEAD;
        f[2] = 1.f;
        r0 = make_float4(1.f, 0.f, 0.f, 0.f);
        r1 = make_float4(0.f, 0.f, 0.f, CUDART_INF_F);
    }
    unsigned char* Ab = reinterpret_cast<unsigned char*>(S.A((unsigned)slot)) + (size_t)(rl >> 3) * 128 + (size_t)(rl & 7) * 16;
#pragma unroll
    for (int kc = 0; kc < tc::KTOT / 4; ++kc)
        *reinterpret_cast<float4*>(Ab + (size_t)kc * (tc::TILE_M * 16)) = make_float4(f[4 * kc], f[4 * kc + 1], f[4 * kc + 2], f[4 * kc + 3]);
    S.ray((unsigned)slot)[2 * rl] = r0;
    S.ray((unsigned)slot)[2 * rl + 1] = r1;
}

struct TcEmit {
    unsigned pos, end;
    unsigned next;
    bool ahead;
    unsigned pads;
};
__device__ __forceinline__ void tc_pad(const WaveParams& W, TcEmit& E, unsigned from, unsigned to, unsigned lane) {
    TC_CHECK(to <= W.pair_cap, "pad", from, to);
#ifdef RT_TC_CHECK
    for (unsigned i = from + lane; i < to; i += 32) W.pairs[i] = make_uint2(PAIR_NULL, (blockIdx.x << 8) | (threadIdx.x >> 5));
#else
    for (unsigned i = from + lane; i < to; i += 32) W.pairs[i] = make_uint2(PAIR_NULL, 0u);
#endif
    if (to > from) E.pads += to - from;
}
__device__ __forceinline__ void tc_request(const WaveParams& W, TcEmit& E, unsigned lane) {
    unsigned b = 0;
    if (lane == 0) b = atomicAdd(&W.st->npairs, (unsigned)tc::PAIR_CHUNK);
    E.next = b;
    E.ahead = true;
}

__device__ __forceinline__ void tc_emit(const WaveParams& W, TcEmit& E, bool emit, unsigned entry, unsigned k, unsigned lane) {
    const unsigned bal = __ballot_sync(0xffffffffu, emit);
    const unsigned total = __popc(bal);
    if (total == 0) return;
    if (E.pos + total > E.end) {
        tc_pad(W, E, E.pos, E.end, lane);
        if (!E.ahead) tc_request(W, E, lane);
        const unsigned b = __shfl_sync(0xffffffffu, E.next, 0);
        E.pos = min(b, W.pair_cap);
        E.end = min(b + (unsigned)tc::PAIR_CHUNK, W.pair_cap);
        tc_request(W, E, lane);
    }
    if (emit) {
        const unsigned w = E.pos + __popc(bal & ((1u << lane) - 1u));
        TC_CHECK(entry < (unsigned)W.capacity && k < (unsigned)W.base.sc.n_list, "pair", entry, k);
        if (w < E.end) W.pairs[w] = make_uint2(entry, k);
        else W.best_key[entry] = BEST_KEY_OVERFLOW;
    }
    E.pos = min(E.pos + total, E.end);
}

__device__ __forceinline__ bool tc_confirm(const tc::Smem& S, float4 r0, float4 r1, unsigned row, int& kk) {
    const float4 R = S.rec[row];
    kk = S.row_k[row];
    const float cc = fmaf(R.x, r0.x, fmaf(R.y, r0.y, fmaf(R.z, r0.z, r0.w)));
    const float s = fmaf(R.x, r1.x, fmaf(R.y, r1.y, fmaf(R.z, r1.z, R.w)));
    const float key = fmaf(-cc, fabsf(cc), fmaf(cc, cc, s - r1.w));
    return (__float_as_uint(key) >> 31) == 0u && kk >= 0;
}

__device__ __noinline__ void tc_redo_fp32(const WaveParams& W, const tc::Smem& S, int slot, unsigned tile, unsigned n, unsigned n_g, unsigned n_p,
                                          int tiles, unsigned cb, unsigned rl) {
    if (tile * tc::TILE_M + rl >= n) return;
    const float4 r0 = S.ray((unsigned)slot)[2 * rl], r1 = S.ray((unsigned)slot)[2 * rl + 1];
    const unsigned entry = wf_entry(tile * tc::TILE_M + rl, n_g, n_p, (unsigned)W.capacity);
    for (int j = 0; j < tiles; ++j)
        for (unsigned q = 0; q < 64u; ++q) {
            int kk;
            if (!tc_confirm(S, r0, r1, (unsigned)j * tc::TILE_N + cb * 64u + q, kk)) continue;
            const unsigned w = atomicAdd(&W.st->npairs, 1u);
            if (w < W.pair_cap) W.pairs[w] = make_uint2(entry, (unsigned)kk);
            else W.best_key[entry] = BEST_KEY_OVERFLOW;
        }
}

__device__ __forceinline__ void tc_drain(const WaveParams& W, const tc::Smem& S, int slot, unsigned tile, unsigned n_g, unsigned n_p,
                                         const uint32_t* cand, unsigned ncand, TcEmit& E, unsigned lane) {
    for (unsigned base = 0; base < ncand; base += 32) {
        const unsigned idx = base + lane;
        bool emit = false;
        unsigned k = 0, entry = 0;
        if (idx < ncand) {
            const uint32_t c = cand[idx];
            const unsigned rl = c >> 20, row = c & 0xfffffu;
            TC_CHECK(rl < 128u && row < (unsigned)W.tc_launch_tiles * 256u, "candidate", c, ncand);
            int kk;
            emit = tc_confirm(S, S.ray((unsigned)slot)[2 * rl], S.ray((unsigned)slot)[2 * rl + 1], row, kk);
            k = (unsigned)kk;
            entry = wf_entry(tile * tc::TILE_M + rl, n_g, n_p, (unsigned)W.capacity);
        }
        tc_emit(W, E, emit, entry, k, lane);
    }
}

#ifdef RT_TC_TIMING
#define TC_T(var) const long long var = clock64()
#define TC_ACC(slot, since) tacc[slot] += clock64() - (since)
#else
#define TC_T(var)
#define TC_ACC(slot, since)
#endif
__global__ void __launch_bounds__(tc::THREADS, 1) wf_cull_tc(const __grid_constant__ WaveParams W) {
    TraceScope trace(W.trace);
    const RenderParams& P = W.base;
    extern __shared__ __align__(1024) unsigned char tc_smem[];
    if (W.st->mode != MODE_RUN) return;
    const unsigned n_g = W.st->cnt[W.cur][0], n_p = W.st->cnt[W.cur][1], n = n_g + n_p;
    if (n == 0) return;
    const unsigned long long gen_base = W.st->gen_base[W.cur];
    const unsigned p0 = (unsigned)W.capacity - n_p;
    const int tiles = W.tc_launch_tiles;
    const unsigned slots = (unsigned)W.tc_slots;
    const tc::Smem S = tc::carve(tc_smem, tiles, (int)slots);
    const unsigned tid = threadIdx.x, warp = tid >> 5, lane = tid & 31u;
    if (blockIdx.x == 0 && tid == 0 && W.tc_pass == 0) atomicAdd(&P.counters[DC_RAYS], (unsigned long long)n);

    const unsigned total_tiles = (n + tc::TILE_M - 1) / tc::TILE_M;
    const unsigned per_cta = W.claims_per_warp > 0 ? (unsigned)W.claims_per_warp : (total_tiles + gridDim.x - 1) / gridDim.x;
    const unsigned first = blockIdx.x * per_cta, last = min(first + per_cta, total_tiles);
    if (first >= last) return;

    if (tid == 0) {
        for (unsigned i = 0; i < slots; ++i) {
            tc::mbar_init(&S.a_ready[i], tc::TILE_M);
            tc::mbar_init(&S.a_free[i], 1);
            tc::mbar_init(&S.ray_free[i], tc::EW);
        }
        for (int i = 0; i < 2 * tc::NBLK; ++i) {
            tc::mbar_init(&S.d_full[i], 1);
            tc::mbar_init(&S.d_empty[i], tc::BLOCK_WARPS);
        }
        asm volatile("fence.mbarrier_init.release.cluster;" ::: "memory");
    }
    if (warp == tc::EW) {
        asm volatile("tcgen05.alloc.cta_group::1.sync.aligned.shared::cta.b32 [%0], %1;" ::"r"(tc::smem_u32(S.tmem_base)), "r"(512) : "memory");
        asm volatile("tcgen05.relinquish_alloc_permit.cta_group::1.sync.aligned;" ::: "memory");
    }
    if (tid < tc::EW) S.cand_n[tid] = 0u;
    {
        const float4* src = reinterpret_cast<const float4*>(P.sc.cull_tc) + (size_t)W.tc_tile0 * (tc::B_TILE_BYTES / 16);
        float4* dst = reinterpret_cast<float4*>(S.B);
        const int n4 = tiles * (tc::B_TILE_BYTES / 16);
        for (int i = (int)tid; i < n4; i += tc::THREADS) dst[i] = __ldg(&src[i]);
        for (int i = (int)tid; i < tiles * tc::TILE_N; i += tc::THREADS) {
            const int k = __ldg(&P.sc.tc_row_k[(size_t)W.tc_tile0 * tc::TILE_N + i]);
            S.row_k[i] = k;
            S.rec[i] = k >= 0 ? __ldg(&P.sc.cull_a[k]) : make_float4(0.f, 0.f, 0.f, -CUDART_INF_F);
        }
    }
    tc::fence_async_smem();
    tc::fence_before();
    __syncthreads();
    tc::fence_after();
    const uint32_t tmem = *S.tmem_base;
    const unsigned n_it = last - first;
#ifdef RT_TC_TIMING
    long long tacc[6] = {0, 0, 0, 0, 0, 0};
    const long long t_begin = clock64();
#endif

    if (warp > tc::EW) {
        const unsigned pt = tid - (tc::EW + 1) * 32, rl = pt & (tc::TILE_M - 1), q = pt / tc::TILE_M;
        for (unsigned it = q; it <= n_it; it += tc::PG) {
            const unsigned s = it % slots, ph = (it / slots) & 1u;
            TC_T(t0);
            if (it >= slots) {
                tc::mbar_wait(&S.a_free[s], ph ^ 1u);
                TC_ACC(0, t0);
                TC_T(t1);
                tc::mbar_wait(&S.ray_free[s], ph ^ 1u);
                TC_ACC(1, t1);
            }
            TC_T(t2);
            if (it < n_it) {
                const unsigned v = (first + it) * tc::TILE_M + rl;
                tc_produce_ray(W, S, (int)s, (int)rl, v < n, v, n_g, p0, gen_base, W.cur);
            }
            TC_ACC(2, t2);
            if (rl == 0) S.tile_of[s] = it < n_it ? (int)(first + it) : -1;
            tc::fence_async_smem();
            tc::mbar_arrive(&S.a_ready[s]);
        }
    } else if (warp == tc::EW) {
        if (lane == 0) {
            const unsigned total = n_it * (unsigned)tiles;
            unsigned gi[tc::NBLK];
#pragma unroll
            for (int c = 0; c < tc::NBLK; ++c) gi[c] = 0;
            unsigned ready_tiles = 0, freed_tiles = 0;
            const uint32_t b_base = tc::smem_u32(S.B);
            for (unsigned idle = 0;;) {
                bool left = false, progressed = false;
#pragma unroll
                for (int c = 0; c < tc::NBLK; ++c) {
                    const unsigned gq = gi[c];
                    if (gq >= total) continue;
                    left = true;
                    const unsigned it = gq / (unsigned)tiles, jt = gq - it * (unsigned)tiles, s = it % slots, b = gq & 1u;
                    if (it >= ready_tiles) {
                        if (!tc::mbar_try_wait(&S.a_ready[s], (it / slots) & 1u)) continue;
                        ready_tiles = it + 1;
                    }
                    if (!tc::mbar_try_wait(&S.d_empty[b * tc::NBLK + c], ((gq >> 1) & 1u) ^ 1u)) continue;
                    tc::fence_after();
                    const uint32_t a_addr = tc::smem_u32(S.A(s));
                    const uint32_t b_addr = b_base + jt * tc::B_TILE_BYTES + (uint32_t)c * (tc::BLOCK_N / 8) * 128;
#pragma unroll
                    for (int kk = 0; kk < tc::KTOT / 8; ++kk)
                        tc::mma_tf32(tmem + b * tc::TILE_N + (uint32_t)c * tc::BLOCK_N, tc::make_desc(a_addr + kk * 2 * tc::TILE_M * 16, tc::TILE_M * 16, 128),
                                     tc::make_desc(b_addr + kk * 2 * tc::TILE_N * 16, tc::TILE_N * 16, 128), kk > 0);
                    tc::mma_commit(&S.d_full[b * tc::NBLK + c]);
                    gi[c] = gq + 1;
                    progressed = true;
                }
                unsigned mn = gi[0];
#pragma unroll
                for (int c = 1; c < tc::NBLK; ++c) mn = min(mn, gi[c]);
                for (const unsigned done = mn / (unsigned)tiles; freed_tiles < done; ++freed_tiles) tc::mma_commit(&S.a_free[freed_tiles % slots]);
                if (!left) break;
                if (progressed) idle = 0;
                else if (++idle > 0x20000000u) __trap();
            }
            tc::mbar_wait(&S.a_free[(n_it - 1) % slots], ((n_it - 1) / slots) & 1u);
        }
        __syncwarp();
    } else {
        const unsigned rl = (warp & 3u) * 32u + lane;
        const unsigned cb = warp >> 2;
        const unsigned blk = warp / tc::BLOCK_WARPS;
        const uint32_t t_lane = ((warp & 3u) * 32u) << 16;
        uint32_t* cand = S.cand + warp * tc::CAND_CAP;
        unsigned* cand_n = S.cand_n + warp;
        TcEmit E{0u, 0u, 0u, false, 0u};
        unsigned g = 0;
        for (unsigned it = 0; it < n_it; ++it) {
            const unsigned s = it % slots, a_ph = (it / slots) & 1u, tile = first + it;
            for (int j = 0; j < tiles; ++j, ++g) {
                const unsigned b = g & 1u;
                TC_T(t0);
                tc::mbar_wait(&S.d_full[b * tc::NBLK + blk], (g >> 1) & 1u);
                TC_ACC(0, t0);
                tc::fence_after();
                const uint32_t taddr = tmem + t_lane + b * tc::TILE_N + cb * 64u;
                unsigned m0, m1;
                TC_T(t1);
                {
                    uint32_t v0[32], v1[32];
                    RT_TMEM_LD32(taddr, v0);
                    RT_TMEM_LD32(taddr + 32u, v1);
                    tc::tmem_wait_ld();
                    tc::fence_before();
                    __syncwarp();
                    if (lane == 0) tc::mbar_arrive(&S.d_empty[b * tc::NBLK + blk]);
                    unsigned w0 = 0u, w1 = 0u;
#pragma unroll
                    for (int q = 0; q < 32; ++q) { w0 = __funnelshift_l(v0[q], w0, 1); w1 = __funnelshift_l(v1[q], w1, 1); }
                    const bool live_ray = tile * tc::TILE_M + rl < n;
                    m0 = live_ray ? ~w0 : 0u; m1 = live_ray ? ~w1 : 0u;
                }
                TC_ACC(1, t1);
                TC_T(t2);
                const unsigned row0 = (unsigned)j * tc::TILE_N + cb * 64u;
#ifdef RT_TC_CHECK
                {
                    const unsigned char* Ab = reinterpret_cast<const unsigned char*>(S.A(s));
                    const unsigned char* Bb = reinterpret_cast<const unsigned char*>(S.B) + (size_t)j * tc::B_TILE_BYTES;
                    for (int q = 0; q < 64; ++q) {
                        double acc = 0.0, mag = 0.0;
                        for (int k = 0; k < tc::KTOT; ++k) {
                            const double x = (double)*reinterpret_cast<const float*>(Ab + tc::canon_off(tc::TILE_M, (int)rl, k)) *
                                             (double)*reinterpret_cast<const float*>(Bb + tc::canon_off(tc::TILE_N, (int)(cb * 64u) + q, k));
                            acc += x; mag += fabs(x);
                        }
                        const unsigned culled = ((q < 32 ? ~m0 : ~m1) >> (31 - (q & 31))) & 1u;
                        if (acc > 1e-4 * mag && culled && mag < 1e20)
                            printf("TMEM mismatch: tile %u ray %u col %u (row %u) double %g (mag %g) but sign bit set; block %u warp %u buffer %u g %u\n", tile, rl, (unsigned)q, row0 + q,
                                   acc, mag, blockIdx.x, warp, b, g);
                        if (acc < -1e-4 * mag && !culled)
                            printf("TMEM mismatch: tile %u ray %u col %u (row %u) double %g (mag %g) but sign bit clear; block %u warp %u buffer %u g %u\n", tile, rl, (unsigned)q, row0 + q,
                                   acc, mag, blockIdx.x, warp, b, g);
                    }
                }
#endif
#pragma unroll
                for (int h = 0; h < 2; ++h) {
                    unsigned mm = h ? m1 : m0;
                    while (mm != 0u) {
                        const int bit = 31 - __clz((int)mm);
                        mm &= ~(1u << bit);
                        const unsigned pos = atomicAdd(cand_n, 1u);
                        if (pos < (unsigned)tc::CAND_CAP) cand[pos] = (rl << 20) | (row0 + (unsigned)h * 32u + (unsigned)(31 - bit));
                    }
                }
                TC_ACC(2, t2);
            }
            TC_T(t3);
            __syncwarp();
            const unsigned raw = *cand_n;
            const bool overflowed = raw > (unsigned)tc::CAND_CAP;
            const unsigned ncand = overflowed ? 0u : raw;
            if (overflowed) {
                tc::mbar_wait(&S.a_ready[s], a_ph);
                tc_redo_fp32(W, S, (int)s, tile, n, n_g, n_p, tiles, cb, rl);
                __syncwarp();
            }
#ifdef RT_TC_CHECK
            if (lane == 0 && ncand > 48u && n < 300u)
                printf("big candidate list: block %u warp %u tile %u it %u ncand %u raw %u first %x %x %x %x last %x\n", blockIdx.x, warp, tile, it, ncand, raw, cand[0], cand[1], cand[2], cand[3], cand[ncand - 1]);
#endif
            if (ncand) {
                tc::mbar_wait(&S.a_ready[s], a_ph);
                tc_drain(W, S, (int)s, tile, n_g, n_p, cand, ncand, E, lane);
            }
            __syncwarp();
            if (lane == 0) {
                *cand_n = 0u;
                tc::mbar_arrive(&S.ray_free[s]);
            }
            __syncwarp();
            TC_ACC(3, t3);
        }
        tc_pad(W, E, E.pos, E.end, lane);
        if (E.ahead) {
            const unsigned b = __shfl_sync(0xffffffffu, E.next, 0);
            tc_pad(W, E, min(b, W.pair_cap), min(b + (unsigned)tc::PAIR_CHUNK, W.pair_cap), lane);
            if (lane == 0 && E.pads) atomicAdd(&W.st->pad, E.pads);
        }
    }
#ifdef RT_TC_TIMING
    if (blockIdx.x == 0 && lane == 0 && n_it > 8)
        printf("tc warp %2u (%s) tiles %u total %lld : %lld %lld %lld %lld cycles per tile\n", warp, warp < tc::EW ? "epi: d_full wait, ld+shf, cand, drain" : (warp == tc::EW ? "mma: a_ready wait, d_empty wait, issue" : "prod: a_free wait, ray_free wait, produce"),
               n_it, (clock64() - t_begin) / n_it, tacc[0] / n_it, tacc[1] / n_it, tacc[2] / n_it, tacc[3] / n_it);
#endif
    tc::fence_before();
    __syncthreads();
    if (warp == tc::EW) asm volatile("tcgen05.dealloc.cta_group::1.sync.aligned.b32 %0, %1;" ::"r"(tmem), "r"(512) : "memory");
}

__global__ void tc_check_fill(const __grid_constant__ WaveParams W, int n, const float* origins, const float* dirs, const float* times) {
    const int i = blockIdx.x * blockDim.x + threadIdx.x;
    if (i == 0) {
        WaveState* st = W.st;
        st->cnt[0][0] = (unsigned)n; st->cnt[0][1] = 0; st->cnt[1][0] = 0; st->cnt[1][1] = 0;
        st->gen_base[0] = 0; st->gen_base[1] = 0;
        st->batch = 0; st->npairs = 0; st->exhausted = 1; st->done = 0; st->mode = MODE_RUN; st->pad = 0;
    }
    if (i >= n) return;
    float4* q = W.queue[0] + 3 * (size_t)i;
    q[0] = make_float4(origins[3 * i], origins[3 * i + 1], origins[3 * i + 2], times ? times[i] : 0.f);
    q[1] = make_float4(dirs[3 * i], dirs[3 * i + 1], dirs[3 * i + 2], 0.f);
    q[2] = make_float4(0.f, 0.f, 0.f, 0.f);
}
__global__ void tc_check_mark(const __grid_constant__ WaveParams W, unsigned* mask, int words) {
    const unsigned npairs = min(W.st->npairs, W.pair_cap);
#ifdef RT_TC_CHECK
    if (blockIdx.x == 0 && threadIdx.x == 0 && W.st->cnt[0][0] < 300u) {
        for (unsigned c0 = 0; c0 < npairs; c0 += 64) {
            unsigned never = 0, real = 0, tag0 = 0xffffffffu, tags = 0;
            for (unsigned i = c0; i < min(c0 + 64u, npairs); ++i) {
                const uint2 pr = W.pairs[i];
                if (pr.x == 0xddddddddu) ++never;
                else if (pr.x == PAIR_NULL) { if (pr.y != tag0) { ++tags; tag0 = pr.y; } }
                else ++real;
            }
            if (never || tags > 1 || real)
                printf("chunk %u: never written %u, real %u, pad-tag changes %u (last tag block %u warp %u)  first entries (%x %x) (%x %x) (%x %x) ... (%x %x)\n", c0, never, real, tags,
                       tag0 >> 8, tag0 & 255u, W.pairs[c0].x, W.pairs[c0].y, W.pairs[c0 + 1].x, W.pairs[c0 + 1].y, W.pairs[c0 + 2].x, W.pairs[c0 + 2].y, W.pairs[c0 + 63].x, W.pairs[c0 + 63].y);
        }
        printf("npairs %u pad counter %u\n", W.st->npairs, W.st->pad);
    }
#endif
    for (unsigned i = blockIdx.x * blockDim.x + threadIdx.x; i < npairs; i += gridDim.x * blockDim.x) {
        const uint2 pr = W.pairs[i];
        if (pr.x != PAIR_NULL && pr.x < (unsigned)W.capacity) atomicOr(&mask[(size_t)pr.x * words + (pr.y >> 5)], 1u << (pr.y & 31u));
    }
}
__global__ void __launch_bounds__(128) tc_check_compare(const __grid_constant__ WaveParams W, int n, double tmin, double tmax, const unsigned* mask,
                                                        int words, unsigned long long* out) {
    const DevScene& sc = W.base.sc;
    const int idx = blockIdx.x * blockDim.x + threadIdx.x;
    unsigned long long lost = 0, surv = 0, cand = 0;
    if (idx < n) {
        const float4 a = W.queue[0][3 * (size_t)idx], b = W.queue[0][3 * (size_t)idx + 1];
        const bool overflow = W.best_key[idx] == BEST_KEY_OVERFLOW;
        for (int k = 0; k < sc.n_list; ++k) {
            const bool kept = overflow || ((mask[(size_t)idx * words + (k >> 5)] >> (k & 31)) & 1u);
            const double t = sc.generic ? refine_leaf<true>(&W.base.sc, k, a.x, a.y, a.z, b.x, b.y, b.z, a.w, tmin, tmax, false, make_uint2(0u, 0u), 0u, 0u, 0u)
                                        : refine_leaf<false>(&W.base.sc, k, a.x, a.y, a.z, b.x, b.y, b.z, a.w, tmin, tmax, false, make_uint2(0u, 0u), 0u, 0u, 0u);
            surv += kept ? 1u : 0u;
            if (t < CUDART_INF) {
                cand++;
                lost += kept ? 0u : 1u;
#ifdef RT_TC_CHECK
                if (!kept) printf("lost pair: ray %d leaf %d t %.9g  o (%.9g %.9g %.9g) d (%.9g %.9g %.9g)\n", idx, k, t, a.x, a.y, a.z, b.x, b.y, b.z);
#endif
            }
        }
    }
    if (lost) atomicAdd(&out[0], lost);
    if (surv) atomicAdd(&out[1], surv);
    if (cand) atomicAdd(&out[2], cand);
}
```

raytrace_clj_b200/csrc/rt_kernels.cuh:

```cuda
#pragma once

#include "rt_device.cuh"

namespace rt {

#define RT_FOR_R _Pragma("unroll") for (int r = 0; r < R; ++r)

struct PathBounce {
    float o[3];
    float time;
    float d[3];
    int hit_id;
    double t;
};

struct RenderParams {
    DevScene sc;
    DevCamera cam;
    int nx, ny;
    int sample_begin, sample_count;
    int row_offset, row_stride, rows_in_shard;
    int max_depth;
    uint2 key;
    float* sum;
// ... 32 lines not shown

template <bool GEN>
__device__ __forceinline__ double refine_leaf(const DevScene* sc, int k, float ox, float oy, float oz, float dx, float dy, float dz,
                                              float time, double tmin, double tmax, bool has_ctx, uint2 key, uint32_t pixel,
                                              uint32_t sample, uint32_t bounce) {
    if (!GEN)
        return refine_candidate(sc->ex_c0r, sc->ex_c1, sc->ex_t0t1, sc->flags, k, ox, oy, oz, dx, dy, dz, time, tmin, tmax);
    float mu = 0.5f;
    if (has_ctx && __ldg(&sc->prim_type[k]) == PRIM_MEDIUM) mu = medium_uniform(key, pixel, sample, bounce, __ldg(&sc->orig_id[k]));
    return refine_generic(sc, k, ox, oy, oz, dx, dy, dz, time, tmin, tmax, mu);
}

__device__ __forceinline__ float4 lds128(unsigned addr) {
    float4 v;
    asm("ld.shared.v4.f32 {%0, %1, %2, %3}, [%4];" : "=f"(v.x), "=f"(v.y), "=f"(v.z), "=f"(v.w) : "r"(addr));
    return v;
}
__device__ __forceinline__ unsigned smem_addr(const void* p) {
    unsigned a = (unsigned)__cvta_generic_to_shared(p);
    asm volatile("" : "+r"(a));
    return a;
}

__device__ __forceinline__ int slice_lo(int n, int part, int parts) { return (int)(((long long)n * part) / parts); }

constexpr int GROUP = 32;
constexpr int CHUNK_GROUPS = 16;
constexpr int CHUNK = GROUP * CHUNK_GROUPS;
constexpr int CULL_PAD = 8;
constexpr float RAY_DEFLATE = 1.0f - 3.2e-6f;

template <int R, int BLOCK, bool COMMON = false>
struct Culler {
    float hx[R], hy[R], hz[R];
    float mx[R], my[R], mz[R];
    float P[R];
    float Q[R];
    float cox, coy, coz;

    static constexpr int LIST_WORDS = CHUNK_GROUPS * R;
    static constexpr size_t LIST_BYTES = (size_t)LIST_WORDS * BLOCK * sizeof(uint32_t);

    __device__ __forceinline__ void set_ray(int r, float o_x, float o_y, float o_z, float d_x, float d_y, float d_z) {
        float a = fmaf(d_z, d_z, fmaf(d_y, d_y, d_x * d_x));
        float s = rsqrtf(a) * ((1.0f + 0.5f * CULL_EPS) * 0.70710678118654752f);
        hx[r] = d_x * s; hy[r] = d_y * s; hz[r] = d_z * s;
        mx[r] = -2.0f * o_x; my[r] = -2.0f * o_y; mz[r] = -2.0f * o_z;
        P[r] = fmaf(o_z, hz[r], fmaf(o_y, hy[r], o_x * hx[r]));
        Q[r] = fmaf(o_z, o_z, fmaf(o_y, o_y, o_x * o_x)) * RAY_DEFLATE;
    }
    __device__ __forceinline__ void kill(int r) {
        hx[r] = 1.f; hy[r] = 0.f; hz[r] = 0.f;
        mx[r] = my[r] = mz[r] = 0.f;
        P[r] = 0.f;
        Q[r] = CUDART_INF_F;
    }

    __device__ __forceinline__ void pin() {
        if (COMMON) {
            RT_FOR_R asm volatile("" : "+f"(hx[r]), "+f"(hy[r]), "+f"(hz[r]), "+f"(P[r]));
        } else {
            RT_FOR_R asm volatile("" : "+f"(hx[r]), "+f"(hy[r]), "+f"(hz[r]), "+f"(mx[r]), "+f"(my[r]), "+f"(mz[r]), "+f"(P[r]), "+f"(Q[r]));
        }
    }

    static __device__ __forceinline__ unsigned list_begin(const uint32_t* list) {
        return (unsigned)__cvta_generic_to_shared(list + threadIdx.x);
    }
    static __device__ __forceinline__ unsigned word(const uint32_t* list, int g, int r) {
        return list[(g * R + r) * BLOCK + threadIdx.x];
    }

    static __device__ __forceinline__ float4 common_record(float4 S, float o_x, float o_y, float o_z) {
        const float m_x = -2.0f * o_x, m_y = -2.0f * o_y, m_z = -2.0f * o_z;
        const float q = fmaf(o_z, o_z, fmaf(o_y, o_y, o_x * o_x)) * RAY_DEFLATE;
        S.w = fmaf(S.x, m_x, fmaf(S.y, m_y, fmaf(S.z, m_z, S.w))) - q;
        return S;
    }

    __device__ __forceinline__ unsigned key_bits(const float4 S, int r) const {
        float c = fmaf(S.x, hx[r], fmaf(S.y, hy[r], fmaf(S.z, hz[r], P[r])));
        if (COMMON) return __float_as_uint(fmaf(-c, fabsf(c), fmaf(c, c, S.w)));
        float s = fmaf(S.x, mx[r], fmaf(S.y, my[r], fmaf(S.z, mz[r], S.w)));
        return __float_as_uint(fmaf(-c, fabsf(c), fmaf(c, c, s - Q[r])));
    }

    __device__ __forceinline__ unsigned long long cull_chunk(unsigned sa, int count, uint32_t* list) const {
        unsigned la = list_begin(list);
        unsigned nzr[R];
        RT_FOR_R nzr[r] = 0u;
        const int full = count / GROUP;
        for (int g = 0; g < full; ++g, la += R * BLOCK * 4) {
            unsigned acc[R];
            RT_FOR_R acc[r] = 0u;
#pragma unroll 8
            for (int u = 0; u < GROUP; ++u, sa += 16) {
                const float4 S = lds128(sa);
                RT_FOR_R acc[r] = __funnelshift_l(key_bits(S, r), acc[r], 1);
            }
            RT_FOR_R {
                asm volatile("st.shared.u32 [%0], %1;" ::"r"(la + (unsigned)(r * BLOCK * 4)), "r"(acc[r]) : "memory");
                nzr[r] |= (acc[r] != 0xffffffffu ? 1u : 0u) << g;
            }
        }
        const int rem = count - full * GROUP;
        if (rem) {
            unsigned acc[R];
            RT_FOR_R acc[r] = 0xffffffffu;
            for (int u = 0; u < rem; u += CULL_PAD) {
#pragma unroll
                for (int v = 0; v < CULL_PAD; ++v, sa += 16) {
                    const float4 S = lds128(sa);
                    RT_FOR_R acc[r] = __funnelshift_l(key_bits(S, r), acc[r], 1);
                }
            }
            RT_FOR_R {
                asm volatile("st.shared.u32 [%0], %1;" ::"r"(la + (unsigned)(r * BLOCK * 4)), "r"(acc[r]) : "memory");
                nzr[r] |= (acc[r] != 0xffffffffu ? 1u : 0u) << full;
            }
        }
        unsigned long long nz = 0ull;
        RT_FOR_R nz |= (unsigned long long)nzr[r] << (16 * r);
        return nz;
    }

    template <class Sink>
    __device__ __forceinline__ void run_range(const float4* s_cull, int s0, int s1, int kbase, uint32_t* list, Sink& sink) {
        for (int c0 = s0; c0 < s1; c0 += CHUNK) {
            const int cc = min(CHUNK, s1 - c0);
            const unsigned long long nz = cull_chunk(smem_addr(s_cull + c0), cc, list);
            sink.flush(list, nz, cc, kbase + c0);
        }
    }

    template <class Sink>
    __device__ __forceinline__ void run(const DevScene& sc, float4* s_cull, int cap, bool preloaded, uint32_t* list,
                                        Sink& sink) {
        pin();
        for (int base = 0; base < sc.n_cull; base += cap) {
            const int count = min(cap, sc.n_cull - base);
            if (!preloaded) {
                __syncthreads();
                for (int i = threadIdx.x; i < count; i += BLOCK) {
                    float4 S = __ldg(&sc.cull_a[base + i]);
                    if (COMMON) S = common_record(S, cox, coy, coz);
                    s_cull[i] = S;
                }
                __syncthreads();
            }
            run_range(s_cull, 0, count, base, list, sink);
        }
    }

    template <class Sink>
    __device__ __forceinline__ void run_slice(const DevScene& sc, float4* s_cull, uint32_t* list, Sink& sink, int part,
                                              int parts) {
        pin();
        const int groups = (sc.n_cull + GROUP - 1) / GROUP;
        const int s0 = slice_lo(groups, part, parts) * GROUP, s1 = min(slice_lo(groups, part + 1, parts) * GROUP, sc.n_cull);
        run_range(s_cull, s0, s1, 0, list, sink);
    }
};

__device__ __forceinline__ void preload_scene(const DevScene& sc, float4* s_cull, int block) {
    for (int i = threadIdx.x; i < sc.n_cull; i += block) s_cull[i] = __ldg(&sc.cull_a[i]);
    __syncthreads();
}

template <int R, int BLOCK>
struct SurvivorIter {
    unsigned long long z;
    unsigned sv;
    int g, r, m, full, rem;
    __device__ __forceinline__ void begin(unsigned long long nz, int count) {
        z = nz; sv = 0u; g = 0; r = 0; m = 0;
        full = count / GROUP; rem = count - full * GROUP;
    }
    __device__ __forceinline__ bool next(const uint32_t* list, int& ray, int& k) {
        if (sv == 0u) {
            if (z == 0ull) return false;
            const int i = __ffsll((long long)z) - 1;
            z &= z - 1ull;
            r = i >> 4;
            g = i & 15;
            m = g < full ? GROUP : rem;
            sv = ~Culler<R, BLOCK>::word(list, g, r);
        }
        const int bit = __ffs(sv) - 1;
        sv &= sv - 1u;
        ray = r;
        k = g * GROUP + (m - 1 - bit);
        return true;
    }
};

template <int R, int BLOCK, bool GEN = false>
struct RefineSink {
    float ox[R], oy[R], oz[R];
    float dx[R], dy[R], dz[R];
    float tm[R];
    double best_t[R];
    int best_k[R];
    unsigned best_tie[R];
    unsigned ncand;
    double tmin, tmax;
    const DevScene* sc;
    bool has_ctx;
    uint2 key;
    uint32_t pix[R], smp[R], bounce[R];

    __device__ __forceinline__ void begin() {
        RT_FOR_R {
            best_t[r] = CUDART_INF;
            best_k[r] = -1;
            best_tie[r] = 0xffffffffu;
        }
    }

    __device__ __forceinline__ void refine(int r, int k) {
        float sox = ox[0], soy = oy[0], soz = oz[0], sdx = dx[0], sdy = dy[0], sdz = dz[0], stm = tm[0];
        uint32_t spix = 0, ssmp = 0, sb = 0;
        if (has_ctx) { spix = pix[0]; ssmp = smp[0]; sb = bounce[0]; }
#pragma unroll
        for (int q = 1; q < R; ++q)
            if (r == q) {
                sox = ox[q]; soy = oy[q]; soz = oz[q]; sdx = dx[q]; sdy = dy[q]; sdz = dz[q]; stm = tm[q];
                if (has_ctx) { spix = pix[q]; ssmp = smp[q]; sb = bounce[q]; }
            }
        const double t = refine_leaf<GEN>(sc, k, sox, soy, soz, sdx, sdy, sdz, stm, tmin, tmax, has_ctx, key, spix, ssmp, sb);
        ncand++;
        if (t < CUDART_INF) {
            const unsigned tie = __ldg(&sc->tie_hi[k]);
#pragma unroll
            for (int q = 0; q < R; ++q)
                if (r == q && (t < best_t[q] || (t == best_t[q] && tie < best_tie[q]))) {
                    best_t[q] = t;
                    best_k[q] = k;
                    best_tie[q] = tie;
                }
        }
    }

    __device__ __forceinline__ void flush(const uint32_t* list, unsigned long long nz, int count, int kbase) {
        SurvivorIter<R, BLOCK> it;
        it.begin(nz, count);
        int r, k;
        while (it.next(list, r, k)) refine(r, kbase + k);
    }

    __device__ __forceinline__ unsigned direct(unsigned live) {
        unsigned nd = 0;
        for (int k = sc->n_list; k < sc->n; ++k)
            for (int r = 0; r < R; ++r)
                if ((live >> r) & 1u) { refine(r, k); ++nd; }
        ncand -= nd;
        return nd;
    }
};

struct alignas(8) WaveState {
    unsigned cnt[2][2];
    unsigned long long gen_base[2];
    unsigned batch;
    unsigned npairs;
    unsigned exhausted;
    unsigned done;
    unsigned mode;
    unsigned pad;
};
enum { MODE_RUN = 0, MODE_DONE = 2 };
struct LaneStatus {
    unsigned n_next;
    unsigned n_fresh;
    unsigned exhausted;
    unsigned mode;
    unsigned seq;
    unsigned pad[3];
};
__device__ __forceinline__ unsigned wf_entry(unsigned i, unsigned n_g, unsigned n_p, unsigned capacity) {
    return i < n_g ? i : capacity - n_p + (i - n_g);
}

struct TraceRec {
    unsigned long long t_start, t_end;
};
__device__ __forceinline__ unsigned long long global_timer_ns() {
    unsigned long long t;
    asm volatile("mov.u64 %0, %globaltimer;" : "=l"(t));
    return t;
}
struct TraceScope {
    TraceRec* rec;
    __device__ __forceinline__ explicit TraceScope(TraceRec* r) : rec(r) {
        if (rec && threadIdx.x == 0) atomicMin(&rec->t_start, global_timer_ns());
    }
    __device__ __forceinline__ ~TraceScope() {
        if (rec && threadIdx.x == 0) atomicMax(&rec->t_end, global_timer_ns());
    }
};

struct WaveParams {
    RenderParams base;
    float4* queue[2];
    unsigned long long* best_t;
    unsigned long long* best_key;
    uint2* pairs;
    uint2* cands;
    double* cand_t;
    unsigned* cand_count;
    WaveState* st;
    int capacity;
    unsigned pair_cap;
    int cur;
    int claims_per_warp;
    int resident_warps;
    volatile LaneStatus* status;
    unsigned iter;
    TraceRec* trace;
    int tc_slots;
    int tc_tile0, tc_launch_tiles;
    int tc_pass;
    unsigned tail_solo;
    unsigned tail_lpp;
};
__device__ __forceinline__ void publish_status(const WaveParams& W, unsigned n_next, unsigned n_fresh, unsigned exhausted, unsigned mode,
                                               unsigned seq) {
    if (!W.status) return;
    W.status->n_next = n_next;
    W.status->n_fresh = n_fresh;
    W.status->exhausted = exhausted;
    W.status->mode = mode;
    __threadfence_system();
    W.status->seq = seq;
}

constexpr unsigned long long BEST_T_INIT = 0x7ff0000000000000ull;
constexpr unsigned long long BEST_KEY_MISS = ~0ull;
constexpr unsigned long long BEST_KEY_OVERFLOW = 0ull;
constexpr unsigned PAIR_NULL = 0xffffffffu;

__device__ __forceinline__ unsigned warp_claim(unsigned* counter, bool pred, unsigned lane) {
    unsigned m = __ballot_sync(0xffffffffu, pred);
    unsigned base = 0;
    if (m) {
        int leader = __ffs(m) - 1;
        if ((int)lane == leader) base = atomicAdd(counter, (unsigned)__popc(m));
        base = __shfl_sync(0xffffffffu, base, leader);
    }
    return base + __popc(m & ((1u << lane) - 1u));
}

__device__ __forceinline__ void make_path(const RenderParams& P, unsigned long long w, float4& a, float4& b, float4& c) {
    const unsigned pshard = (unsigned)P.nx * (unsigned)P.rows_in_shard;
    unsigned s_local, q;
    if (P.total_work <= 0xffffffffull) {
        s_local = (unsigned)w / pshard;
        q = (unsigned)w - s_local * pshard;
    } else {
        s_local = (unsigned)(w / pshard);
        q = (unsigned)(w - (unsigned long long)s_local * pshard);
    }
    int row_local = (int)(q / (unsigned)P.nx);
    int i = (int)(q - (unsigned)row_local * (unsigned)P.nx);
    int j = P.row_offset + row_local * P.row_stride;
    uint32_t pix = (uint32_t)j * (uint32_t)P.nx + (uint32_t)i;
    uint32_t smp = (uint32_t)(P.sample_begin + (int)s_local);
    uint32_t slot = pix;
    if (P.path_pixel) {
        pix = (uint32_t)__ldg(&P.path_pixel[w]);
        smp = (uint32_t)__ldg(&P.path_sample[w]);
        j = (int)(pix / (uint32_t)P.nx);
        i = (int)(pix - (uint32_t)j * (uint32_t)P.nx);
        slot = (uint32_t)w;
    }
    float3 o, d;
    float tmv;
    generate_ray(P.cam, P.nx, P.ny, i, j, pix, smp, P.key, o, d, tmv, nullptr);
    a = make_float4(o.x, o.y, o.z, tmv);
    b = make_float4(d.x, d.y, d.z, __uint_as_float(slot));
    c = make_float4(1.f, 1.f, 1.f, __uint_as_float((smp << 8) | (uint32_t)P.max_depth));
}

constexpr int kMaxLanes = 2;
struct InitParams {
    WaveState* st[kMaxLanes];
    unsigned long long first[kMaxLanes];
    unsigned count[kMaxLanes];
    int n_lanes;
    unsigned long long* work_counter;
    unsigned long long* counters;
    unsigned long long total0, total_work;
};
__global__ void wf_init(const InitParams I) {
    for (int l = 0; l < I.n_lanes; ++l) {
        WaveState* st = I.st[l];
        st->cnt[0][0] = 0; st->cnt[0][1] = I.count[l];
        st->cnt[1][0] = 0; st->cnt[1][1] = 0;
        st->gen_base[0] = I.first[l]; st->gen_base[1] = 0;
        st->batch = 0; st->npairs = 0; st->done = 0; st->mode = I.count[l] ? MODE_RUN : MODE_DONE; st->pad = 0;
        st->exhausted = I.total0 >= I.total_work ? 1u : 0u;
    }
    *I.work_counter = I.total0;
    atomicAdd(&I.counters[DC_SAMPLES], I.total0);
}
__global__ void wf_fill_best(unsigned long long* best_t, unsigned long long* best_key, size_t n) {
    for (size_t i = blockIdx.x * (size_t)blockDim.x + threadIdx.x; i < n; i += (size_t)gridDim.x * blockDim.x) {
        best_t[i] = 0x7ff0000000000000ull;
        best_key[i] = ~0ull;
    }
}

template <int R, int BLOCK>
struct PairSink {
    unsigned idx0;
    unsigned n;
    unsigned n_g, p0;
    __device__ __forceinline__ unsigned entry(unsigned v) const { return v < n_g ? v : p0 + (v - n_g); }
    unsigned long long live;
    uint2* pairs;
    unsigned pair_cap;
    unsigned long long* best_key;
    WaveState* st;

    __device__ __forceinline__ void flush(const uint32_t* list, unsigned long long nz, int count, int kbase) {
        nz &= live;
        if (!__any_sync(0xffffffffu, nz != 0ull)) return;
        const unsigned lane = threadIdx.x & 31u;
        unsigned np = 0;
        for (unsigned long long z = nz; z; z &= z - 1ull) {
            const int i = __ffsll((long long)z) - 1;
            np += __popc(~Culler<R, BLOCK>::word(list, i & 15, i >> 4));
        }
        unsigned incl = np;
#pragma unroll
        for (int d = 1; d < 32; d <<= 1) {
            unsigned v = __shfl_up_sync(0xffffffffu, incl, d);
            if ((int)lane >= d) incl += v;
        }
        const unsigned total = __shfl_sync(0xffffffffu, incl, 31);
        unsigned base = 0;
        if (lane == 0) base = atomicAdd(&st->npairs, total);
        base = __shfl_sync(0xffffffffu, base, 0);
        const bool fits = base + total <= pair_cap;
        unsigned w = base + incl - np;
        SurvivorIter<R, BLOCK> it;
        it.begin(nz, count);
        int r, k;
        while (it.next(list, r, k)) {
            const unsigned v = idx0 + 32u * (unsigned)r;
            if (fits) {
                pairs[w] = make_uint2(entry(v), (unsigned)(kbase + k));
            } else {
                if (w < pair_cap) pairs[w] = make_uint2(PAIR_NULL, 0u);
                if (v < n) best_key[entry(v)] = BEST_KEY_OVERFLOW;
            }
            ++w;
        }
    }
};

constexpr unsigned ITEM_NONE = 0xffffffffu;
constexpr unsigned ITEM_STOP = 0xfffffffeu;
struct Scope {
    unsigned bid, nblk;
};
__device__ __forceinline__ Scope grid_scope() { return Scope{blockIdx.x, gridDim.x}; }
template <int R, int BLOCK, bool COMMON>
__device__ __forceinline__ unsigned wf_cull_batches(const WaveParams& W, Scope sc_, int cur, unsigned e0, unsigned e1, unsigned n_g,
                                                    unsigned p0, unsigned long long gen0, int parts, unsigned item0, unsigned claimed,
                                                    int& budget, float4* s_cull, uint32_t* s_list) {
    if (claimed == ITEM_STOP) return ITEM_STOP;
    const RenderParams& P = W.base;
    const unsigned lane = threadIdx.x & 31u, warp = threadIdx.x >> 5, warps = BLOCK / 32;
    const unsigned n_batches = (e1 - e0 + 32 * R - 1) / (32 * R);
    const unsigned n_items = n_batches * (unsigned)parts;
    Culler<R, BLOCK, COMMON> K;
    K.cox = P.cam.origin.x; K.coy = P.cam.origin.y; K.coz = P.cam.origin.z;
    PairSink<R, BLOCK> sink;
    sink.n = e1;
    sink.n_g = n_g;
    sink.p0 = p0;
    sink.pairs = W.pairs;
    sink.pair_cap = W.pair_cap;
    sink.best_key = W.best_key;
    sink.st = W.st;
    unsigned item = sc_.bid * warps + warp;
    const unsigned uniform_end = (n_items + warps - 1) / warps * warps;
    for (;;) {
        if (P.preloaded) {
            if (claimed != ITEM_NONE) {
                item = claimed;
                claimed = ITEM_NONE;
            } else {
                unsigned b = 0;
                if (lane == 0) b = atomicAdd(&W.st->batch, 1u);
                item = __shfl_sync(0xffffffffu, b, 0);
            }
            if (item >= item0 + n_items) return item;
            item -= item0;
        } else {
            if (item - warp >= uniform_end) break;
        }
        const unsigned batch = item / (unsigned)parts, part = item - batch * (unsigned)parts;
        sink.idx0 = e0 + batch * (32 * R) + lane;
        sink.live = 0ull;
        RT_FOR_R {
            const unsigned v = sink.idx0 + 32 * r;
            if (v < e1 && batch < n_batches) {
                float4* qc = cur ? W.queue[1] : W.queue[0];
                float4 a, b;
                if (v >= n_g) {
                    float4 c;
                    float4* q = qc + 3 * (size_t)(p0 + (v - n_g));
                    make_path(P, gen0 + (v - n_g), a, b, c);
                    if (part == 0) { q[0] = a; q[1] = b; q[2] = c; }
                } else {
                    a = qc[3 * (size_t)v];
                    b = qc[3 * (size_t)v + 1];
                }
                K.set_ray(r, a.x, a.y, a.z, b.x, b.y, b.z);
                sink.live |= 0xffffull << (16 * r);
            } else {
                K.kill(r);
            }
        }
        if (parts > 1) K.run_slice(P.sc, s_cull, s_list, sink, (int)part, parts);
        else           K.run(P.sc, s_cull, P.cull_cap, P.preloaded != 0, s_list, sink);
        item += sc_.nblk * warps;
        if (P.preloaded && budget > 0 && --budget == 0) return ITEM_STOP;
    }
    return ITEM_NONE;
}

template <int R, int BLOCK>
__device__ __forceinline__ void wf_cull_body(const WaveParams& W, Scope sc_, int cur, unsigned n_g, unsigned n_p, unsigned long long gen_base,
                                             float4* s_cull, float4* s_cullc, uint32_t* s_list) {
    const RenderParams& P = W.base;
    const unsigned n = n_g + n_p, p0 = (unsigned)W.capacity - n_p;
    if (sc_.bid == 0 && threadIdx.x == 0) atomicAdd(&P.counters[DC_RAYS], (unsigned long long)n);
    const unsigned grid_warps = W.resident_warps > 0 ? (unsigned)W.resident_warps : sc_.nblk * (BLOCK / 32);
    int budget = W.claims_per_warp;
    const unsigned n_c = P.common_origin ? n_p : 0u, n_v = n - n_c;
    const unsigned long long genC = gen_base - p0;
    if (R > 1 && !P.preloaded) {
        if (n_c) wf_cull_batches<R, BLOCK, true>(W, sc_, cur, p0, p0 + n_c, 0u, 0u, genC + 0u, 1, 0u, ITEM_NONE, budget, s_cull, s_list);
        if (n_v) wf_cull_batches<R, BLOCK, false>(W, sc_, cur, 0u, n_v, n_g, p0, gen_base, 1, 0u, ITEM_NONE, budget, s_cull, s_list);
    } else if (R > 1 && n >= grid_warps * 64u) {
        const unsigned tail = grid_warps * 64u, per = 32u * R;
        const unsigned g_rest0 = min(n_v, tail), p_rest0 = min(n_c, tail - g_rest0);
        const unsigned g_bulk = (n_v - g_rest0) / per * per, p_bulk = (n_c - p_rest0) / per * per;
        unsigned items = 0;
        unsigned next = wf_cull_batches<R, BLOCK, true>(W, sc_, cur, p0, p0 + p_bulk, 0u, 0u, genC, 1, items, ITEM_NONE, budget, s_cullc, s_list);
        items += p_bulk / per;
        next = wf_cull_batches<R, BLOCK, false>(W, sc_, cur, 0u, g_bulk, n_g, p0, gen_base, 1, items, next, budget, s_cull, s_list);
        items += g_bulk / per;
        next = wf_cull_batches<1, BLOCK, true>(W, sc_, cur, p0 + p_bulk, p0 + n_c, 0u, 0u, genC, 1, items, next, budget, s_cullc, s_list);
        items += (n_c - p_bulk + 31u) / 32u;
        wf_cull_batches<1, BLOCK, false>(W, sc_, cur, g_bulk, n_v, n_g, p0, gen_base, 1, items, next, budget, s_cull, s_list);
    } else {
        const unsigned b1 = (n + 31) / 32;
        int parts = 1;
        if (P.preloaded)
            while (parts < 16 && b1 * (unsigned)parts * 2u <= grid_warps) parts *= 2;
        unsigned next = ITEM_NONE, items = 0;
        if (n_c) {
            next = wf_cull_batches<1, BLOCK, true>(W, sc_, cur, p0, p0 + n_c, 0u, 0u, genC, parts, 0u, ITEM_NONE, budget, P.preloaded ? s_cullc : s_cull, s_list);
            items = (n_c + 31u) / 32u * (unsigned)parts;
        }
        if (n_v) wf_cull_batches<1, BLOCK, false>(W, sc_, cur, 0u, n_v, n_g, p0, gen_base, parts, items, next, budget, s_cull, s_list);
    }
}

template <int R, int BLOCK, int MINB>
__global__ void __launch_bounds__(BLOCK, MINB) wf_cull(const __grid_constant__ WaveParams W) {
    TraceScope trace(W.trace);
    const RenderParams& P = W.base;
    extern __shared__ float4 smem_f4[];
    float4* s_cull = smem_f4;
    uint32_t* s_list = reinterpret_cast<uint32_t*>(smem_f4 + P.cull_cap);
    float4* s_cullc = reinterpret_cast<float4*>(s_list + Culler<R, BLOCK>::LIST_WORDS * BLOCK);
    if (W.st->mode != MODE_RUN) return;
    const unsigned n_g = W.st->cnt[W.cur][0], n_p = W.st->cnt[W.cur][1];
    if (n_g + n_p == 0) return;
    const unsigned long long gen_base = W.st->gen_base[W.cur];
    if (P.preloaded) {
        preload_scene(P.sc, s_cull, BLOCK);
        if (n_p && P.common_origin)
            for (int i = threadIdx.x; i < P.sc.n_cull; i += BLOCK)
                s_cullc[i] = Culler<R, BLOCK, true>::common_record(s_cull[i], P.cam.origin.x, P.cam.origin.y, P.cam.origin.z);
    }
    __syncthreads();
    wf_cull_body<R, BLOCK>(W, grid_scope(), W.cur, n_g, n_p, gen_base, s_cull, s_cullc, s_list);
}

#include "rt_cull_tc.cuh"

__device__ __forceinline__ unsigned wf_cand_region(const WaveParams& W, unsigned total_warps) {
    return ((W.pair_cap + total_warps * 32u - 1u) / (total_warps * 32u)) * 32u;
}

template <bool GEN>
__device__ __forceinline__ void wf_refine_body(const WaveParams& W, const DevScene* scp, Scope sc_, int cur) {
    const RenderParams& P = W.base;
    const unsigned npairs = min(W.st->npairs, W.pair_cap);
    const unsigned lane = threadIdx.x & 31u;
    if (sc_.bid == 0 && threadIdx.x == 0) {
        W.st->batch = 0;
        W.st->cnt[cur ^ 1][0] = 0;
        W.st->cnt[cur ^ 1][1] = 0;
        atomicAdd(&P.counters[DC_CANDIDATES], (unsigned long long)(npairs - min(npairs, W.st->pad)));
        W.st->pad = 0;
    }
    const unsigned total_warps = sc_.nblk * (blockDim.x >> 5);
    const unsigned warp_id = sc_.bid * (blockDim.x >> 5) + (threadIdx.x >> 5);
    const size_t region = (size_t)warp_id * wf_cand_region(W, total_warps);
    unsigned cnt = 0;
    const unsigned stride = sc_.nblk * blockDim.x;
    const unsigned i_first = sc_.bid * blockDim.x + threadIdx.x;
    uint2 pr_next = i_first < npairs ? W.pairs[i_first] : make_uint2(PAIR_NULL, 0u);
    for (unsigned i0 = i_first - lane; i0 < npairs; i0 += stride) {
        const uint2 pr = pr_next;
        const unsigned i_next = i0 + lane + stride;
        pr_next = i_next < npairs ? W.pairs[i_next] : make_uint2(PAIR_NULL, 0u);
        bool cand = false;
        double t = CUDART_INF;
        if (pr.x != PAIR_NULL) {
            const float4* qc = cur ? W.queue[1] : W.queue[0];
            const float4 a = qc[3 * (size_t)pr.x], b = qc[3 * (size_t)pr.x + 1];
            const unsigned long long seen = __ldcg(&W.best_t[pr.x]);
            if (!GEN) {
                t = refine_candidate(P.sc.ex_c0r, P.sc.ex_c1, P.sc.ex_t0t1, P.sc.flags, (int)pr.y, a.x, a.y, a.z, b.x, b.y, b.z,
                                     a.w, 0.001, (double)FLT_MAX);
            } else {
                uint32_t pixq = 0, smpq = 0, bq = 0;
                if (__ldg(&P.sc.prim_type[pr.y]) == PRIM_MEDIUM) {
                    const uint32_t sd = __float_as_uint(qc[3 * (size_t)pr.x + 2].w);
                    pixq = rng_pixel(P, __float_as_uint(b.w));
                    smpq = sd >> 8;
                    bq = (uint32_t)(P.max_depth - (int)(sd & 255u) + 1);
                }
                t = refine_leaf<true>(scp, (int)pr.y, a.x, a.y, a.z, b.x, b.y, b.z, a.w, 0.001, (double)FLT_MAX, true, P.key, pixq, smpq, bq);
            }
            const unsigned long long tb = (unsigned long long)__double_as_longlong(t);
            if (t < CUDART_INF && tb <= seen) {
                atomicMin(&W.best_t[pr.x], tb);
                cand = true;
            }
        }
        const unsigned m = __ballot_sync(0xffffffffu, cand);
        if (cand) {
            const size_t slot = region + cnt + __popc(m & ((1u << lane) - 1u));
            W.cands[slot] = pr;
            W.cand_t[slot] = t;
        }
        cnt += __popc(m);
    }
    if (lane == 0) W.cand_count[warp_id] = cnt;
}
template <bool GEN>
__global__ void __launch_bounds__(256) wf_refine(const __grid_constant__ WaveParams W) {
    if (W.st->mode != MODE_RUN) return;
    TraceScope trace(W.trace);
    wf_refine_body<GEN>(W, &W.base.sc, grid_scope(), W.cur);
}

__device__ __forceinline__ void wf_tiebreak_body(const WaveParams& W, Scope sc_) {
    const RenderParams& P = W.base;
    const unsigned lane = threadIdx.x & 31u;
    const unsigned total_warps = sc_.nblk * (blockDim.x >> 5);
    const unsigned warp_id = sc_.bid * (blockDim.x >> 5) + (threadIdx.x >> 5);
    const size_t region = (size_t)warp_id * wf_cand_region(W, total_warps);
    const unsigned cnt = W.cand_count[warp_id];
    for (unsigned j = lane; j < cnt; j += 32) {
        const uint2 pr = W.cands[region + j];
        if ((unsigned long long)__double_as_longlong(W.cand_t[region + j]) == W.best_t[pr.x])
            atomicMin(&W.best_key[pr.x], (((unsigned long long)__ldg(&P.sc.tie_hi[pr.y])) << 32) | pr.y);
    }
}
__global__ void __launch_bounds__(256) wf_tiebreak(const __grid_constant__ WaveParams W) {
    if (W.st->mode != MODE_RUN) return;
    TraceScope trace(W.trace);
    wf_tiebreak_body(W, grid_scope());
}

template <bool GEN>
__device__ __noinline__ void exact_closest_hit(const DevScene* sc, float ox, float oy, float oz, float dx, float dy, float dz,
                                               float tm, uint2 key, uint32_t pixel, uint32_t sample, uint32_t bounce, double* out_t,
                                               int* out_k) {
    double best = CUDART_INF;
    int bk = -1;
    unsigned btie = 0xffffffffu;
    for (int k = 0; k < sc->n; ++k) {
        double t = refine_leaf<GEN>(sc, k, ox, oy, oz, dx, dy, dz, tm, 0.001, (double)FLT_MAX, true, key, pixel, sample, bounce);
        if (t < CUDART_INF) {
            unsigned tie = __ldg(&sc->tie_hi[k]);
            if (t < best || (t == best && tie < btie)) { best = t; bk = k; btie = tie; }
        }
    }
    *out_t = best;
    *out_k = bk;
}

template <bool GEN>
__device__ __forceinline__ unsigned wf_shade_body(const WaveParams& W, const DevScene* scp, Scope sc_, int cur, unsigned* s_ctr) {
    const RenderParams& P = W.base;
    const unsigned n_g = W.st->cnt[cur][0], n_p = W.st->cnt[cur][1], n = n_g + n_p;
    const unsigned lane = threadIdx.x & 31u;
    const float4* qc = cur ? W.queue[1] : W.queue[0];
    float4* qn = cur ? W.queue[0] : W.queue[1];
    if (sc_.bid == 0 && threadIdx.x == 0) W.st->npairs = 0;
    unsigned n_direct = 0;
    const unsigned stride = sc_.nblk * blockDim.x;
    for (unsigned idx0 = sc_.bid * blockDim.x + threadIdx.x - lane; idx0 < n; idx0 += stride) {
        const bool have = idx0 + lane < n;
        const unsigned idx = wf_entry(idx0 + lane, n_g, n_p, (unsigned)W.capacity);
        bool cont = false;
        float4 a, b, c;
        if (have) {
            a = qc[3 * (size_t)idx]; b = qc[3 * (size_t)idx + 1]; c = qc[3 * (size_t)idx + 2];
            unsigned long long key = W.best_key[idx];
            const uint32_t slot = __float_as_uint(b.w), sd = __float_as_uint(c.w);
            const uint32_t pix = rng_pixel(P, slot);
            const uint32_t smp = sd >> 8;
            const int depth = (int)(sd & 255u);
            const uint32_t bounce = (uint32_t)(P.max_depth - depth + 1);
            int k = (int)(unsigned)key;
            double td = __longlong_as_double((long long)W.best_t[idx]);
            W.best_key[idx] = BEST_KEY_MISS;
            W.best_t[idx] = BEST_T_INIT;
            if (key == BEST_KEY_OVERFLOW) {
                exact_closest_hit<GEN>(scp, a.x, a.y, a.z, b.x, b.y, b.z, a.w, P.key, pix, smp, bounce, &td, &k);
                key = k < 0 ? BEST_KEY_MISS : 1ull;
            } else {
                for (int kd = P.sc.n_list; kd < P.sc.n; ++kd) {
                    ++n_direct;
                    const double t = refine_leaf<GEN>(scp, kd, a.x, a.y, a.z, b.x, b.y, b.z, a.w, 0.001, (double)FLT_MAX, true, P.key, pix,
                                                      smp, bounce);
                    const unsigned long long kk = (((unsigned long long)__ldg(&P.sc.tie_hi[kd])) << 32) | (unsigned)kd;
                    if (t < td || (t < CUDART_INF && t == td && kk < key)) {
                        td = t;
                        key = kk;
                        k = kd;
                    }
                }
            }
            const bool hit = key != BEST_KEY_MISS;
            if (P.path_pixel) path_log_ray(P, slot, (int)bounce - 1, a, b, hit ? k : -1, hit ? td : CUDART_INF);
            if (!hit) {
                atomicAdd(&s_ctr[DC_TERM_MISS], 1u);
                if (P.path_pixel) path_log_end(P, slot, (int)bounce, TERM_MISS);
            } else {
                float3 o = f3(a.x, a.y, a.z), d = f3(b.x, b.y, b.z);
                float3 att, em;
                int reason = TERM_NONE;
                float tmv = a.w;
                ScatterRng rng{P.key, pix, smp, bounce, nullptr, nullptr};
                cont = shade_hit<GEN>(P.sc, scp, k, (float)td, o, d, tmv, depth > 0, rng, att, em, reason);
                if (em.x != 0.f || em.y != 0.f || em.z != 0.f) {
                    float* dst = P.sum + (size_t)slot * 3;
                    atomicAdd(dst + 0, c.x * em.x);
                    atomicAdd(dst + 1, c.y * em.y);
                    atomicAdd(dst + 2, c.z * em.z);
                }
                if (cont) {
                    a = make_float4(o.x, o.y, o.z, tmv);
                    b = make_float4(d.x, d.y, d.z, b.w);
                    c = make_float4(c.x * att.x, c.y * att.y, c.z * att.z, __uint_as_float((smp << 8) | (uint32_t)(depth - 1)));
                } else {
                    atomicAdd(&s_ctr[reason == TERM_LIGHT ? DC_TERM_LIGHT
                                     : reason == TERM_ABSORB ? DC_TERM_ABSORB : DC_TERM_DEPTH], 1u);
                    if (P.path_pixel) path_log_end(P, slot, (int)bounce, reason);
                }
            }
        }
        const unsigned mc = __ballot_sync(0xffffffffu, cont);
        if (mc) {
            unsigned base = 0u;
            if (lane == 0) base = atomicAdd(&W.st->cnt[cur ^ 1][0], (unsigned)__popc(mc));
            base = __shfl_sync(0xffffffffu, base, 0);
            if (cont) {
                float4* q = qn + 3 * (size_t)(base + __popc(mc & ((1u << lane) - 1u)));
                q[0] = a; q[1] = b; q[2] = c;
            }
        }
    }
    if (n_direct) atomicAdd(&s_ctr[DC_DIRECT], n_direct);
    return 0u;
}

template <bool GEN>
__global__ void __launch_bounds__(256, GEN ? 1 : 0) wf_shade(const __grid_constant__ WaveParams W) {
    if (W.st->mode != MODE_RUN) return;
    TraceScope trace(W.trace);
    const RenderParams& P = W.base;
    __shared__ unsigned s_ctr[DC_COUNT];
    if (threadIdx.x < DC_COUNT) s_ctr[threadIdx.x] = 0;
    __syncthreads();
    wf_shade_body<GEN>(W, &W.base.sc, grid_scope(), W.cur, s_ctr);
    __syncthreads();
    if (threadIdx.x < DC_COUNT && s_ctr[threadIdx.x]) atomicAdd(&P.counters[threadIdx.x], (unsigned long long)s_ctr[threadIdx.x]);
    if (threadIdx.x == 0) {
        __threadfence();
        if (atomicAdd(&W.st->done, 1u) == gridDim.x - 1) {
            __threadfence();
            W.st->done = 0;
            const unsigned n_cont = *(volatile unsigned*)&W.st->cnt[W.cur ^ 1][0];
            const unsigned want = (unsigned)W.capacity - n_cont;
            unsigned n_fresh = 0;
            unsigned long long base = 0ull;
            if (!W.st->exhausted && want) {
                base = atomicAdd(P.work_counter, (unsigned long long)want);
                if (base < P.total_work) n_fresh = (unsigned)min((unsigned long long)want, P.total_work - base);
                if (base + want >= P.total_work) W.st->exhausted = 1u;
            }
            W.st->cnt[W.cur ^ 1][1] = n_fresh;
            W.st->gen_base[W.cur ^ 1] = base;
            if (n_fresh) atomicAdd(&P.counters[DC_SAMPLES], (unsigned long long)n_fresh);
            if (n_cont + n_fresh == 0) W.st->mode = MODE_DONE;
            __threadfence();
            publish_status(W, n_cont + n_fresh, n_fresh, W.st->exhausted, W.st->mode, W.iter);
        }
    }
}

struct TraceParamsB {
    DevScene sc;
    int n;
    const float* origins;
    const float* dirs;
    const float* times;
    double tmin, tmax;
    double* out_t;
    int* out_id;
    unsigned long long* stats;
};

struct BvhHit {
    double t;
    int k;
    unsigned tie;
    unsigned n_leaf, n_node;
};
template <bool GEN>
__device__ __forceinline__ BvhHit bvh_closest(const DevScene* sc, float ox, float oy, float oz, float dx, float dy, float dz, float time,
                                              double tmin, double tmax, bool has_ctx, uint2 key, uint32_t pixel, uint32_t sample,
                                              uint32_t bounce) {
    BvhHit H{CUDART_INF, -1, 0xffffffffu, 0u, 0u};
    const float ix = 1.0f / dx, iy = 1.0f / dy, iz = 1.0f / dz;
    const float e = 2.4e-7f * fmaxf(fmaxf(fabsf(ox), fabsf(oy)), fabsf(oz));
    const float tlo = (float)tmin * (1.0f - 1e-6f);
    float thi = tmax >= (double)FLT_MAX ? FLT_MAX : __double2float_ru(tmax);
    int stack[48];
    int sp = 0, node = 0;
    for (;;) {
        if (node >= 0) {
            const float4 A = __ldg(&sc->bvh[4 * node]), B = __ldg(&sc->bvh[4 * node + 1]), C = __ldg(&sc->bvh[4 * node + 2]);
            const int4 D = __ldg(reinterpret_cast<const int4*>(&sc->bvh[4 * node + 3]));
            H.n_node += 2;
            float a0 = ((A.x - e) - ox) * ix, a1 = ((A.w + e) - ox) * ix, b0 = ((A.y - e) - oy) * iy, b1 = ((B.x + e) - oy) * iy,
                  c0 = ((A.z - e) - oz) * iz, c1 = ((B.y + e) - oz) * iz;
            float ln = fmaxf(fmaxf(fminf(a0, a1), fminf(b0, b1)), fmaxf(fminf(c0, c1), tlo));
            float lf = fminf(fminf(fmaxf(a0, a1), fmaxf(b0, b1)), fminf(fmaxf(c0, c1), thi));
            a0 = ((B.z - e) - ox) * ix; a1 = ((C.y + e) - ox) * ix; b0 = ((B.w - e) - oy) * iy; b1 = ((C.z + e) - oy) * iy;
            c0 = ((C.x - e) - oz) * iz; c1 = ((C.w + e) - oz) * iz;
            float rn = fmaxf(fmaxf(fminf(a0, a1), fminf(b0, b1)), fmaxf(fminf(c0, c1), tlo));
            float rf = fminf(fminf(fmaxf(a0, a1), fmaxf(b0, b1)), fminf(fmaxf(c0, c1), thi));
            const bool hl = ln <= lf * 1.0000005f + 1e-30f, hr = rn <= rf * 1.0000005f + 1e-30f;
            if (hl && hr) {
                const bool left_first = ln <= rn;
                stack[sp++] = left_first ? D.y : D.x;
                node = left_first ? D.x : D.y;
                continue;
            }
            if (hl) { node = D.x; continue; }
            if (hr) { node = D.y; continue; }
        } else {
            const int k = ~node;
            H.n_leaf++;
            const double t = refine_leaf<GEN>(sc, k, ox, oy, oz, dx, dy, dz, time, tmin, tmax, has_ctx, key, pixel, sample, bounce);
            if (t < CUDART_INF) {
                const unsigned tie = __ldg(&sc->tie_hi[k]);
                if (t < H.t || (t == H.t && tie < H.tie)) {
                    H.t = t; H.k = k; H.tie = tie;
                    thi = fminf(thi, __double2float_ru(t));
                }
            }
        }
        if (sp == 0) break;
        node = stack[--sp];
    }
    return H;
}

template <bool GEN>
__global__ void __launch_bounds__(128, GEN ? 1 : 0) wf_bvh(const __grid_constant__ WaveParams W) {
    if (W.st->mode != MODE_RUN) return;
    TraceScope trace(W.trace);
    const RenderParams& P = W.base;
    __shared__ unsigned s_ctr[DC_COUNT];
    if (threadIdx.x < DC_COUNT) s_ctr[threadIdx.x] = 0;
    __syncthreads();
    const int cur = W.cur;
    const unsigned n_g = W.st->cnt[cur][0], n_p = W.st->cnt[cur][1], n = n_g + n_p, p0 = (unsigned)W.capacity - n_p;
    const unsigned long long gen_base = W.st->gen_base[cur];
    float4* qc = cur ? W.queue[1] : W.queue[0];
    unsigned n_leaf = 0, n_node = 0;
    for (unsigned v = blockIdx.x * blockDim.x + threadIdx.x; v < n; v += gridDim.x * blockDim.x) {
        float4 a, b, c;
        unsigned idx;
        if (v >= n_g) {
            idx = p0 + (v - n_g);
            make_path(P, gen_base + (v - n_g), a, b, c);
            float4* q = qc + 3 * (size_t)idx;
            q[0] = a; q[1] = b; q[2] = c;
        } else {
            idx = v;
            a = qc[3 * (size_t)idx]; b = qc[3 * (size_t)idx + 1]; c = qc[3 * (size_t)idx + 2];
        }
        const uint32_t sd = __float_as_uint(c.w);
        const BvhHit H = bvh_closest<GEN>(&W.base.sc, a.x, a.y, a.z, b.x, b.y, b.z, a.w, 0.001, (double)FLT_MAX, true, P.key,
                                          rng_pixel(P, __float_as_uint(b.w)), sd >> 8, (uint32_t)(P.max_depth - (int)(sd & 255u) + 1));
        n_leaf += H.n_leaf; n_node += H.n_node;
        if (H.k >= 0) {
            W.best_t[idx] = (unsigned long long)__double_as_longlong(H.t);
            W.best_key[idx] = ((unsigned long long)H.tie << 32) | (unsigned)H.k;
        }
    }
    atomicAdd(&s_ctr[DC_CANDIDATES], n_leaf);
    atomicAdd(&s_ctr[DC_BVH_NODES], n_node);
    __syncthreads();
    if (threadIdx.x < DC_COUNT && s_ctr[threadIdx.x]) atomicAdd(&P.counters[threadIdx.x], (unsigned long long)s_ctr[threadIdx.x]);
    if (blockIdx.x == 0 && threadIdx.x == 0) {
        atomicAdd(&P.counters[DC_RAYS], (unsigned long long)n);
        W.st->batch = 0;
        W.st->npairs = 0;
        W.st->cnt[cur ^ 1][0] = 0;
        W.st->cnt[cur ^ 1][1] = 0;
    }
}

template <bool GEN>
__global__ void __launch_bounds__(128) trace_bvh_kernel(const __grid_constant__ TraceParamsB P) {
    const int idx = blockIdx.x * blockDim.x + threadIdx.x;
    if (idx >= P.n) return;
    const float ox = P.origins[3 * idx], oy = P.origins[3 * idx + 1], oz = P.origins[3 * idx + 2];
    const float dx = P.dirs[3 * idx], dy = P.dirs[3 * idx + 1], dz = P.dirs[3 * idx + 2];
    const float tm = P.times ? P.times[idx] : 0.f;
    BvhHit H = bvh_closest<GEN>(&P.sc, ox, oy, oz, dx, dy, dz, tm, P.tmin, P.tmax, false, make_uint2(0u, 0u), 0u, 0u, 0u);
    for (int k = P.sc.n_list; k < P.sc.n; ++k) {
        const double t = refine_leaf<GEN>(&P.sc, k, ox, oy, oz, dx, dy, dz, tm, P.tmin, P.tmax, false, make_uint2(0u, 0u), 0u, 0u, 0u);
        const unsigned tie = __ldg(&P.sc.tie_hi[k]);
        if (t < H.t || (t < CUDART_INF && t == H.t && tie < H.tie)) { H.t = t; H.k = k; H.tie = tie; }
    }
    P.out_t[idx] = H.t;
    P.out_id[idx] = H.k >= 0 ? __ldg(&P.sc.orig_id[H.k]) : -1;
    if (P.stats) {
        atomicAdd(&P.stats[0], (unsigned long long)H.n_leaf);
        atomicAdd(&P.stats[1], (unsigned long long)H.n_node);
    }
}

template <bool GEN>
__device__ __forceinline__ void wf_solo_paths(const WaveParams& W, const DevScene* scp, const float4* qc, unsigned n, unsigned* claim,
                                              const float4* s_cull, unsigned* s_ctr) {
    const RenderParams& P = W.base;
    const unsigned lane = threadIdx.x & 31u;
    const unsigned lpp = W.tail_lpp;
    const unsigned sub = lane & (lpp - 1u), lead = lane & ~(lpp - 1u);
    bool active = false;
    float4 a = make_float4(0.f, 0.f, 0.f, 0.f), b = a, c = a;
    uint32_t slot = 0u, pix = 0u;
    unsigned n_rays = 0, n_cand = 0, n_direct = 0;
    for (;;) {
        unsigned i = 0xffffffffu;
        if (!active && sub == 0u) i = atomicAdd(claim, 1u);
        i = __shfl_sync(0xffffffffu, i, (int)lead);
        if (!active && i < n) {
            a = qc[3 * (size_t)i]; b = qc[3 * (size_t)i + 1]; c = qc[3 * (size_t)i + 2];
            slot = __float_as_uint(b.w);
            pix = rng_pixel(P, slot);
            active = true;
        }
        if (!__any_sync(0xffffffffu, active)) break;
        const uint32_t sd = __float_as_uint(c.w), smp = sd >> 8;
        const int depth = (int)(sd & 255u);
        const uint32_t bounce = (uint32_t)(P.max_depth - depth + 1);
        Culler<1, 32, false> K;
        K.set_ray(0, a.x, a.y, a.z, b.x, b.y, b.z);
        if (active && sub == 0u) ++n_rays;
        unsigned long long bt = BEST_T_INIT, bkey = BEST_KEY_MISS;
        for (int base = 0; base < P.sc.n; base += 64 * (int)lpp) {
            unsigned long long mask = 0ull;
            if (active) {
                const int jn = min(64, (P.sc.n - base + (int)lpp - 1) / (int)lpp);
#pragma unroll 4
                for (int j = 0; j < jn; ++j) {
                    const int s = base + (int)lpp * j + (int)sub;
                    bool pass = s < P.sc.n;
                    if (s < P.sc.n_list) {
                        const float4 S = P.preloaded ? s_cull[s] : __ldg(&P.sc.cull_a[s]);
                        pass = (int)K.key_bits(S, 0) >= 0;
                    }
                    mask |= (unsigned long long)(pass ? 1u : 0u) << j;
                }
            }
            while (__any_sync(0xffffffffu, mask != 0ull)) {
                if (mask) {
                    const int s = base + (int)lpp * (__ffsll((long long)mask) - 1) + (int)sub;
                    mask &= mask - 1ull;
                    if (s < P.sc.n_list) ++n_cand; else ++n_direct;
                    const double t = refine_leaf<GEN>(scp, s, a.x, a.y, a.z, b.x, b.y, b.z, a.w, 0.001, (double)FLT_MAX, true, P.key, pix, smp,
                                                      bounce);
                    const unsigned long long tb = (unsigned long long)__double_as_longlong(t);
                    const unsigned long long kk = (((unsigned long long)__ldg(&P.sc.tie_hi[s])) << 32) | (unsigned)s;
                    if (t < CUDART_INF && (tb < bt || (tb == bt && kk < bkey))) { bt = tb; bkey = kk; }
                }
            }
        }
        for (unsigned dlt = lpp >> 1; dlt; dlt >>= 1) {
            const unsigned long long ot = __shfl_xor_sync(0xffffffffu, bt, (int)dlt), ok = __shfl_xor_sync(0xffffffffu, bkey, (int)dlt);
            if (ot < bt || (ot == bt && ok < bkey)) { bt = ot; bkey = ok; }
        }
        if (active) {
            const bool hit = bkey != BEST_KEY_MISS;
            const int k = (int)(unsigned)bkey;
            const double td = __longlong_as_double((long long)bt);
            if (P.path_pixel && sub == 0u) path_log_ray(P, slot, (int)bounce - 1, a, b, hit ? k : -1, hit ? td : CUDART_INF);
            int reason = TERM_MISS;
            bool cont = false;
            if (hit) {
                float3 o = f3(a.x, a.y, a.z), d = f3(b.x, b.y, b.z);
                float3 att, em;
                float tmv = a.w;
                ScatterRng rng{P.key, pix, smp, bounce, nullptr, nullptr};
                reason = TERM_NONE;
                cont = shade_hit<GEN>(P.sc, scp, k, (float)td, o, d, tmv, depth > 0, rng, att, em, reason);
                if (sub == 0u && (em.x != 0.f || em.y != 0.f || em.z != 0.f)) {
                    float* dst = P.sum + (size_t)slot * 3;
                    atomicAdd(dst + 0, c.x * em.x);
                    atomicAdd(dst + 1, c.y * em.y);
                    atomicAdd(dst + 2, c.z * em.z);
                }
                if (cont) {
                    a = make_float4(o.x, o.y, o.z, tmv);
                    b = make_float4(d.x, d.y, d.z, b.w);
                    c = make_float4(c.x * att.x, c.y * att.y, c.z * att.z, __uint_as_float((smp << 8) | (uint32_t)(depth - 1)));
                }
            }
            if (!cont) {
                if (sub == 0u) {
                    atomicAdd(&s_ctr[reason == TERM_MISS ? DC_TERM_MISS : reason == TERM_LIGHT ? DC_TERM_LIGHT
                                     : reason == TERM_ABSORB ? DC_TERM_ABSORB : DC_TERM_DEPTH], 1u);
                    if (P.path_pixel) path_log_end(P, slot, (int)bounce, reason);
                }
                active = false;
            }
        }
    }
    if (n_rays) atomicAdd(&s_ctr[DC_RAYS], n_rays);
    if (n_cand) atomicAdd(&s_ctr[DC_CANDIDATES], n_cand);
    if (n_direct) atomicAdd(&s_ctr[DC_DIRECT], n_direct);
}

constexpr int kPairsPerEntry = 8;
template <int BLOCK, bool GEN, int TR>
__global__ void __launch_bounds__(BLOCK, GEN ? 1 : 2) wf_tail(const __grid_constant__ WaveParams W) {
    const RenderParams& P = W.base;
    extern __shared__ float4 smem_f4[];
    float4* s_cull = smem_f4;
    uint32_t* s_list = reinterpret_cast<uint32_t*>(smem_f4 + P.cull_cap);
    __shared__ unsigned s_ctr[DC_COUNT];
    __shared__ WaveState s_st;
    if (W.st->mode == MODE_DONE) return;
    TraceScope trace(W.trace);
    int cur = W.cur;
    const unsigned n_all = W.st->cnt[cur][0];
    const unsigned K = ((n_all + gridDim.x - 1) / gridDim.x + 31u) / 32u * 32u;
    const unsigned first = blockIdx.x * K;
    if (first < n_all) {
        if (threadIdx.x < DC_COUNT) s_ctr[threadIdx.x] = 0;
        if (threadIdx.x == 0) {
            s_st.cnt[cur][0] = min(K, n_all - first);
            s_st.cnt[cur ^ 1][0] = 0;
            s_st.cnt[0][1] = s_st.cnt[1][1] = 0;
            s_st.gen_base[0] = s_st.gen_base[1] = 0ull;
            s_st.batch = 0;
            s_st.npairs = 0;
            s_st.exhausted = 1;
            s_st.done = 0;
            s_st.mode = MODE_RUN;
            s_st.pad = 0;
        }
        const unsigned warps = BLOCK / 32;
        WaveParams L = W;
        L.queue[0] = W.queue[0] + 3 * (size_t)first;
        L.queue[1] = W.queue[1] + 3 * (size_t)first;
        L.best_t = W.best_t + first;
        L.best_key = W.best_key + first;
        L.pairs = W.pairs + (size_t)first * kPairsPerEntry;
        L.pair_cap = min(K, (unsigned)W.capacity - first) * kPairsPerEntry;
        const size_t cand_slice = (size_t)wf_cand_region(L, warps) * warps;
        L.cands = W.cands + (size_t)blockIdx.x * cand_slice;
        L.cand_t = W.cand_t + (size_t)blockIdx.x * cand_slice;
        L.cand_count = W.cand_count + blockIdx.x * warps;
        L.st = &s_st;
        L.status = nullptr;
        L.capacity = (int)K;
        L.claims_per_warp = 0;
        L.resident_warps = 0;
        if (P.preloaded) preload_scene(P.sc, s_cull, BLOCK);
        const Scope solo{0u, 1u};
        for (;;) {
            __syncthreads();
            const unsigned n = *(volatile unsigned*)&s_st.cnt[cur][0];
#ifdef RT_TAIL_DIAG
            const bool diag = (blockIdx.x == 0 || blockIdx.x == gridDim.x / 2) && threadIdx.x == 0;
            unsigned long long dt0 = global_timer_ns();
#endif
            if (n <= W.tail_solo) {
                if (n) wf_solo_paths<GEN>(L, &W.base.sc, cur ? L.queue[1] : L.queue[0], n, &s_st.done, s_cull, s_ctr);
#ifdef RT_TAIL_DIAG
                __syncthreads();
                if (diag) printf("tail cta %u solo n %u: %llu ns\n", blockIdx.x, n, global_timer_ns() - dt0);
#endif
                break;
            }
            wf_cull_body<TR, BLOCK>(L, solo, cur, n, 0u, 0ull, s_cull, nullptr, s_list);
            __syncthreads();
#ifdef RT_TAIL_DIAG
            unsigned long long dt1 = global_timer_ns();
            const unsigned np_ = s_st.npairs;
#endif
            wf_refine_body<GEN>(L, &W.base.sc, solo, cur);
            __syncthreads();
#ifdef RT_TAIL_DIAG
            unsigned long long dt2 = global_timer_ns();
#endif
            wf_tiebreak_body(L, solo);
            __syncthreads();
#ifdef RT_TAIL_DIAG
            unsigned long long dt3 = global_timer_ns();
#endif
            wf_shade_body<GEN>(L, &W.base.sc, solo, cur, s_ctr);
#ifdef RT_TAIL_DIAG
            __syncthreads();
            if (diag) printf("tail cta %u n %u pairs %u: cull %llu refine %llu tie %llu shade %llu ns\n", blockIdx.x, n, np_, dt1 - dt0, dt2 - dt1, dt3 - dt2, global_timer_ns() - dt3);
#endif
            cur ^= 1;
        }
        __syncthreads();
        if (threadIdx.x < DC_COUNT && s_ctr[threadIdx.x]) atomicAdd(&P.counters[threadIdx.x], (unsigned long long)s_ctr[threadIdx.x]);
    }
    if (threadIdx.x == 0) {
        __threadfence();
        if (atomicAdd(&W.st->done, 1u) == gridDim.x - 1) {
            W.st->done = 0;
            W.st->cnt[0][0] = W.st->cnt[0][1] = W.st->cnt[1][0] = W.st->cnt[1][1] = 0;
            W.st->mode = MODE_DONE;
            __threadfence();
            publish_status(W, 0u, 0u, 1u, MODE_DONE, W.iter);
        }
    }
}


struct MegaShade {
    float4 o_t;
    float4 d_c;
    float4 att_r;
    float4 em;
};
template <bool GEN>
__device__ __noinline__ MegaShade mega_shade_one(const DevScene* scp, int k, float t, float ox, float oy, float oz, float dx, float dy,
                                                 float dz, float time, int allow_scatter, uint2 key, uint32_t pix, uint32_t smp,
                                                 uint32_t bounce) {
    float3 o = f3(ox, oy, oz), d = f3(dx, dy, dz), att, em;
    int reason = TERM_NONE;
    ScatterRng rng{key, pix, smp, bounce, nullptr, nullptr};
    const bool cont = shade_hit<GEN>(*scp, scp, k, t, o, d, time, allow_scatter != 0, rng, att, em, reason);
    MegaShade m;
    m.o_t = make_float4(o.x, o.y, o.z, time);
    m.d_c = make_float4(d.x, d.y, d.z, cont ? 1.f : 0.f);
    m.att_r = make_float4(att.x, att.y, att.z, (float)reason);
    m.em = make_float4(em.x, em.y, em.z, 0.f);
    return m;
}

template <int R, int BLOCK, int MINB, bool GEN>
__global__ void __launch_bounds__(BLOCK, MINB) mega_kernel(const __grid_constant__ RenderParams P) {
    extern __shared__ float4 smem_f4[];
    float4* s_cull = smem_f4;
    uint32_t* s_list = reinterpret_cast<uint32_t*>(smem_f4 + P.cull_cap);
    __shared__ unsigned s_ctr[DC_COUNT];
    if (threadIdx.x < DC_COUNT) s_ctr[threadIdx.x] = 0;
    if (P.preloaded) preload_scene(P.sc, s_cull, BLOCK);
    __syncthreads();

    Culler<R, BLOCK> K;
    RefineSink<R, BLOCK, GEN> I;
    I.tmin = 0.001;
    I.tmax = (double)FLT_MAX;
    I.ncand = 0;
    I.sc = &P.sc;
    I.has_ctx = true;
    I.key = P.key;

    float ar[R], ag[R], ab[R];
    uint32_t slot[R];
    uint32_t (&pix)[R] = I.pix, (&smp)[R] = I.smp;
    int depth[R];
    bool alive[R];
    RT_FOR_R { alive[r] = false; I.ox[r] = I.oy[r] = I.oz[r] = I.tm[r] = 0.f; I.dx[r] = 1.f; I.dy[r] = I.dz[r] = 0.f; pix[r] = smp[r] = slot[r] = 0u; I.bounce[r] = 0u; }
    unsigned n_rays = 0, n_samples = 0, n_direct = 0;
    const unsigned lane = threadIdx.x & 31u;
    const unsigned pshard = (unsigned)P.nx * (unsigned)P.rows_in_shard;

    for (;;) {
        RT_FOR_R {
            unsigned need = __ballot_sync(0xffffffffu, !alive[r]);
            if (need) {
                int leader = __ffs(need) - 1;
                unsigned long long base = 0;
                if ((int)lane == leader) base = atomicAdd(P.work_counter, (unsigned long long)__popc(need));
                base = __shfl_sync(0xffffffffu, base, leader);
                unsigned long long w = base + __popc(need & ((1u << lane) - 1u));
                if (!alive[r] && w < P.total_work) {
                    unsigned s_local = (unsigned)(w / pshard);
                    unsigned q = (unsigned)(w - (unsigned long long)s_local * pshard);
                    int row_local = (int)(q / (unsigned)P.nx);
                    int i = (int)(q - (unsigned)row_local * (unsigned)P.nx);
                    int j = P.row_offset + row_local * P.row_stride;
                    pix[r] = (uint32_t)j * (uint32_t)P.nx + (uint32_t)i;
                    smp[r] = (uint32_t)(P.sample_begin + (int)s_local);
                    slot[r] = pix[r];
                    if (P.path_pixel) {
                        pix[r] = (uint32_t)__ldg(&P.path_pixel[w]);
                        smp[r] = (uint32_t)__ldg(&P.path_sample[w]);
                        j = (int)(pix[r] / (uint32_t)P.nx);
                        i = (int)(pix[r] - (uint32_t)j * (uint32_t)P.nx);
                        slot[r] = (uint32_t)w;
                    }
                    float3 o, d;
                    generate_ray(P.cam, P.nx, P.ny, i, j, pix[r], smp[r], P.key, o, d, I.tm[r], nullptr);
                    I.ox[r] = o.x; I.oy[r] = o.y; I.oz[r] = o.z;
                    I.dx[r] = d.x; I.dy[r] = d.y; I.dz[r] = d.z;
                    ar[r] = ag[r] = ab[r] = 1.0f;
                    depth[r] = P.max_depth;
                    alive[r] = true;
                    n_samples++;
                }
            }
        }
        bool any_alive = false;
        RT_FOR_R any_alive |= alive[r];
        if (P.preloaded) {
            if (!__any_sync(0xffffffffu, any_alive)) break;
        } else {
            if (!__syncthreads_or(any_alive)) break;
        }

        unsigned live = 0;
        RT_FOR_R {
            if (alive[r]) { K.set_ray(r, I.ox[r], I.oy[r], I.oz[r], I.dx[r], I.dy[r], I.dz[r]); n_rays++; live |= 1u << r; }
            else K.kill(r);
            I.bounce[r] = (uint32_t)(P.max_depth - depth[r] + 1);
        }
        I.begin();
        K.run(P.sc, s_cull, P.cull_cap, P.preloaded != 0, s_list, I);
        n_direct += I.direct(live);

        RT_FOR_R {
            if (alive[r]) {
                if (P.path_pixel)
                    path_log_ray(P, slot[r], (int)I.bounce[r] - 1, make_float4(I.ox[r], I.oy[r], I.oz[r], I.tm[r]),
                                 make_float4(I.dx[r], I.dy[r], I.dz[r], 0.f), I.best_k[r], I.best_t[r]);
                if (I.best_k[r] < 0) {
                    alive[r] = false;
                    atomicAdd(&s_ctr[DC_TERM_MISS], 1u);
                    if (P.path_pixel) path_log_end(P, slot[r], (int)I.bounce[r], TERM_MISS);
                } else {
                    const MegaShade ms = mega_shade_one<GEN>(&P.sc, I.best_k[r], (float)I.best_t[r], I.ox[r], I.oy[r], I.oz[r], I.dx[r], I.dy[r],
                                                             I.dz[r], I.tm[r], depth[r] > 0 ? 1 : 0, P.key, pix[r], smp[r], I.bounce[r]);
                    const float3 o = f3(ms.o_t.x, ms.o_t.y, ms.o_t.z), d = f3(ms.d_c.x, ms.d_c.y, ms.d_c.z);
                    const float3 att = f3(ms.att_r.x, ms.att_r.y, ms.att_r.z), em = f3(ms.em.x, ms.em.y, ms.em.z);
                    const bool cont = ms.d_c.w != 0.f;
                    const int reason = (int)ms.att_r.w;
                    I.tm[r] = ms.o_t.w;
                    if (em.x != 0.f || em.y != 0.f || em.z != 0.f) {
                        float* dst = P.sum + (size_t)slot[r] * 3;
                        atomicAdd(dst + 0, ar[r] * em.x);
                        atomicAdd(dst + 1, ag[r] * em.y);
                        atomicAdd(dst + 2, ab[r] * em.z);
                    }
                    if (cont) {
                        ar[r] *= att.x; ag[r] *= att.y; ab[r] *= att.z;
                        I.ox[r] = o.x; I.oy[r] = o.y; I.oz[r] = o.z;
                        I.dx[r] = d.x; I.dy[r] = d.y; I.dz[r] = d.z;
                        depth[r]--;
                    } else {
                        alive[r] = false;
                        atomicAdd(&s_ctr[reason == TERM_LIGHT ? DC_TERM_LIGHT
                                         : reason == TERM_ABSORB ? DC_TERM_ABSORB : DC_TERM_DEPTH], 1u);
                        if (P.path_pixel) path_log_end(P, slot[r], (int)I.bounce[r], reason);
                    }
                }
            }
        }
    }

    atomicAdd(&s_ctr[DC_RAYS], n_rays);
    atomicAdd(&s_ctr[DC_SAMPLES], n_samples);
    atomicAdd(&s_ctr[DC_CANDIDATES], I.ncand);
    atomicAdd(&s_ctr[DC_DIRECT], n_direct);
    __syncthreads();
    if (threadIdx.x < DC_COUNT && s_ctr[threadIdx.x]) atomicAdd(&P.counters[threadIdx.x], (unsigned long long)s_ctr[threadIdx.x]);
}

struct TraceParams {
    DevScene sc;
    int n;
    const float* origins;
    const float* dirs;
    const float* times;
    double tmin, tmax;
    double* out_t;
    int* out_id;
    int cull_cap, preloaded;
};

template <int R, int BLOCK, bool GEN>
__global__ void __launch_bounds__(BLOCK) trace_kernel(const __grid_constant__ TraceParams P) {
    extern __shared__ float4 smem_f4[];
    float4* s_cull = smem_f4;
    uint32_t* s_list = reinterpret_cast<uint32_t*>(smem_f4 + P.cull_cap);
    if (P.preloaded) preload_scene(P.sc, s_cull, BLOCK);
    __syncthreads();
    Culler<R, BLOCK> K;
    RefineSink<R, BLOCK, GEN> I;
    I.tmin = P.tmin;
    I.tmax = P.tmax;
    I.ncand = 0;
    I.sc = &P.sc;
    I.has_ctx = false;
    for (long long base = (long long)blockIdx.x * BLOCK * R; base < P.n; base += (long long)gridDim.x * BLOCK * R) {
        unsigned live = 0;
        RT_FOR_R {
            long long idx = base + (long long)r * BLOCK + threadIdx.x;
            if (idx < P.n) {
                I.ox[r] = P.origins[3 * idx]; I.oy[r] = P.origins[3 * idx + 1]; I.oz[r] = P.origins[3 * idx + 2];
                I.dx[r] = P.dirs[3 * idx]; I.dy[r] = P.dirs[3 * idx + 1]; I.dz[r] = P.dirs[3 * idx + 2];
                I.tm[r] = P.times ? P.times[idx] : 0.f;
                K.set_ray(r, I.ox[r], I.oy[r], I.oz[r], I.dx[r], I.dy[r], I.dz[r]);
                live |= 1u << r;
            } else {
                I.ox[r] = I.oy[r] = I.oz[r] = I.tm[r] = 0.f;
                I.dx[r] = 1.f; I.dy[r] = 0.f; I.dz[r] = 0.f;
                K.kill(r);
            }
        }
        I.begin();
        K.run(P.sc, s_cull, P.cull_cap, P.preloaded != 0, s_list, I);
        I.direct(live);
        RT_FOR_R {
            long long idx = base + (long long)r * BLOCK + threadIdx.x;
            if (idx < P.n) {
                P.out_t[idx] = I.best_t[r];
                P.out_id[idx] = (I.best_k[r] >= 0) ? __ldg(&P.sc.orig_id[I.best_k[r]]) : -1;
            }
        }
    }
}

__global__ void __launch_bounds__(128) cull_check_kernel(const __grid_constant__ DevScene sc, int n, const float* origins, const float* dirs,
                                                         const float* times, double tmin, double tmax,
                                                         unsigned long long* out) {
    const int idx = blockIdx.x * blockDim.x + threadIdx.x;
    unsigned long long lost = 0, surv = 0, cand = 0;
    if (idx < n) {
        const float ox = origins[3 * idx], oy = origins[3 * idx + 1], oz = origins[3 * idx + 2];
        const float dx = dirs[3 * idx], dy = dirs[3 * idx + 1], dz = dirs[3 * idx + 2];
        const float tm = times ? times[idx] : 0.f;
        Culler<1, 128> K;
        K.set_ray(0, ox, oy, oz, dx, dy, dz);
        K.pin();
        for (int k = 0; k < sc.n_list; ++k) {
            const bool culled = (K.key_bits(__ldg(&sc.cull_a[k]), 0) >> 31) != 0u;
            const double t = sc.generic ? refine_leaf<true>(&sc, k, ox, oy, oz, dx, dy, dz, tm, tmin, tmax, false, make_uint2(0u, 0u), 0u, 0u, 0u)
                                        : refine_leaf<false>(&sc, k, ox, oy, oz, dx, dy, dz, tm, tmin, tmax, false, make_uint2(0u, 0u), 0u, 0u, 0u);
            surv += culled ? 0u : 1u;
            if (t < CUDART_INF) {
                cand++;
                lost += culled ? 1u : 0u;
            }
        }
    }
    if (lost) atomicAdd(&out[0], lost);
    if (surv) atomicAdd(&out[1], surv);
    if (cand) atomicAdd(&out[2], cand);
}

__global__ void sampler_kernel(int kind, int n, uint2 key, float* out) {
    const int i = blockIdx.x * blockDim.x + threadIdx.x;
    if (i >= n) return;
    if (kind == 0) {
        const float3 p = rand_in_unit_sphere(key, (uint32_t)i, 0u, 1u, 1u);
        out[3 * i] = p.x; out[3 * i + 1] = p.y; out[3 * i + 2] = p.z;
    } else {
        const float2 p = rand_in_unit_disk(key, (uint32_t)i, 0u, 1u);
        out[2 * i] = p.x; out[2 * i + 1] = p.y;
    }
}

__global__ void genrays_kernel(DevCamera cam, int n, int nx, int ny, const int* ij, const int* s, uint2 key, float* out_o,
                               float* out_d, float* out_t, float* out_rnd) {
    int idx = blockIdx.x * blockDim.x + threadIdx.x;
    if (idx >= n) return;
    int i = ij[2 * idx], j = ij[2 * idx + 1];
    float3 o, d;
    float tm;
    float rnd[5];
    generate_ray(cam, nx, ny, i, j, (uint32_t)j * (uint32_t)nx + (uint32_t)i, (uint32_t)s[idx], key, o, d, tm, rnd);
    out_o[3 * idx] = o.x; out_o[3 * idx + 1] = o.y; out_o[3 * idx + 2] = o.z;
    out_d[3 * idx] = d.x; out_d[3 * idx + 1] = d.y; out_d[3 * idx + 2] = d.z;
    out_t[idx] = tm;
    if (out_rnd)
        for (int k = 0; k < 5; ++k) out_rnd[5 * idx + k] = rnd[k];
}

__global__ void shade_kernel(const __grid_constant__ DevScene sc, int n, const float* origins, const float* dirs, const float* times,
                             const int* hit_id, const double* hit_t, const float* ball, const float* u01v, float* out_o,
                             float* out_d, float* out_att, float* out_em, int* out_flags) {
    int idx = blockIdx.x * blockDim.x + threadIdx.x;
    if (idx >= n) return;
    float3 o = f3(origins[3 * idx], origins[3 * idx + 1], origins[3 * idx + 2]);
    float3 d = f3(dirs[3 * idx], dirs[3 * idx + 1], dirs[3 * idx + 2]);
    float3 att = f3(0.f, 0.f, 0.f), em = f3(0.f, 0.f, 0.f);
    int flag = -1;
    int id = hit_id[idx];
    if (id >= 0 && id < sc.n) {
        int k = sc.cull_of_orig[id];
        int reason = TERM_NONE;
        ScatterRng rng{make_uint2(0u, 0u), 0u, 0u, 0u, ball + 3 * idx, u01v + idx};
        float tmv = times ? times[idx] : 0.f;
        bool cont = sc.generic ? shade_hit<true>(sc, &sc, k, (float)hit_t[idx], o, d, tmv, true, rng, att, em, reason)
                               : shade_hit<false>(sc, &sc, k, (float)hit_t[idx], o, d, tmv, true, rng, att, em, reason);
        flag = cont ? 1 : 0;
        if (!cont) {
            o = f3(0.f, 0.f, 0.f); d = o; att = o;
        }
// ... 69 lines not shown
```

Before: 1.622 billion.

## Merge tiebreak into refine via 128-bit CAS on packed (t,key) best record

Packs the per-ray best hit distance and tie key into one 16-byte record and updates it with a 128-bit atomic compare-and-swap loop during refine. This removes the separate tiebreak kernel launch per wavefront iteration and the candidate buffers (cands, cand_t, cand_count) that refine wrote and tiebreak reread. Refine also deduplicates same-entry updates within a warp via match_any and defers each CAS by one iteration to overlap it with loads. The cost is CAS retry loops under contention and a dependence on b128 atomics being available on the target.

Result: no change. 1.628 billion (median of 6 runs) (+0.4%).

```diff
diff --git a/raytrace_clj_b200/csrc/rt_api.cu b/raytrace_clj_b200/csrc/rt_api.cu
--- a/raytrace_clj_b200/csrc/rt_api.cu
+++ b/raytrace_clj_b200/csrc/rt_api.cu
@@ -45,11 +45,8 @@
     unsigned long long* d_counters = nullptr;
     struct WaveLane {
         float4* queue = nullptr;
-        unsigned long long* best = nullptr;
+        ulonglong2* best = nullptr;
         uint2* pairs = nullptr;
-        uint2* cands = nullptr;
-        double* cand_t = nullptr;
-        unsigned* cand_count = nullptr;
         WaveState* state = nullptr;
         LaneStatus* h_status = nullptr;
         LaneStatus* d_status = nullptr;
@@ -202,10 +199,7 @@
     if (L.queue) cudaFree(L.queue);
     if (L.best) cudaFree(L.best);
     if (L.pairs) cudaFree(L.pairs);
-    if (L.cands) cudaFree(L.cands);
-    if (L.cand_t) cudaFree(L.cand_t);
-    if (L.cand_count) cudaFree(L.cand_count);
-    L.queue = nullptr; L.best = nullptr; L.pairs = nullptr; L.cands = nullptr; L.cand_t = nullptr; L.cand_count = nullptr;
+    L.queue = nullptr; L.best = nullptr; L.pairs = nullptr;
     L.entries = 0;
 }
 
@@ -245,12 +239,8 @@
     if (L.entries >= entries) return RT_OK;
     free_lane(L);
     RT_CUDA(ctx, cudaMalloc(&L.queue, entries * 2 * 3 * sizeof(float4)));
-    RT_CUDA(ctx, cudaMalloc(&L.best, entries * 2 * sizeof(unsigned long long)));
+    RT_CUDA(ctx, cudaMalloc(&L.best, entries * sizeof(ulonglong2)));
     RT_CUDA(ctx, cudaMalloc(&L.pairs, entries * kPairsPerEntry * sizeof(uint2)));
-    const size_t cand_slots = entries * kPairsPerEntry + (size_t)d.sm_count * 8 * 8 * 32;
-    RT_CUDA(ctx, cudaMalloc(&L.cands, cand_slots * sizeof(uint2)));
-    RT_CUDA(ctx, cudaMalloc(&L.cand_t, cand_slots * sizeof(double)));
-    RT_CUDA(ctx, cudaMalloc(&L.cand_count, (size_t)d.sm_count * 8 * 8 * sizeof(unsigned)));
     L.entries = entries;
     L.best_clean = false;
     return RT_OK;
@@ -395,12 +385,8 @@
         W[l].base = P;
         W[l].queue[0] = L.queue;
         W[l].queue[1] = L.queue + 3 * capacity;
-        W[l].best_t = L.best;
-        W[l].best_key = L.best + L.entries;
+        W[l].best = L.best;
         W[l].pairs = L.pairs;
-        W[l].cands = L.cands;
-        W[l].cand_t = L.cand_t;
-        W[l].cand_count = L.cand_count;
         W[l].st = L.state;
         W[l].capacity = (int)capacity;
         W[l].pair_cap = (unsigned)std::min<size_t>(capacity * kPairsPerEntry, 0xfffffff0u);
@@ -453,7 +439,7 @@
         I.count[l] = count0[l];
         first += count0[l];
         if (!L.best_clean) {
-            wf_fill_best<<<d.sm_count * 4, 256, 0, stream>>>(L.best, L.best + L.entries, L.entries);
+            wf_fill_best<<<d.sm_count * 4, 256, 0, stream>>>(L.best, L.entries);
             ctx->n_launches += 1;
         }
         L.best_clean = false;
@@ -482,7 +468,7 @@
             all_done = false;
             DeviceBuffers::WaveLane& L = d.lanes[l];
             while (!tailed[l] && enq[l] - seen[l] < depth) {
-                cudaEvent_t e[5] = {nullptr, nullptr, nullptr, nullptr, nullptr};
+                cudaEvent_t e[4] = {nullptr, nullptr, nullptr, nullptr};
                 if (ctx->profile)
                     for (auto& x : e) { RT_CUDA(ctx, cudaEventCreate(&x)); evs.push_back(x); }
                 if (ctx->profile) cudaEventRecord(e[0], st[l]);
@@ -491,11 +477,11 @@
                 if (bvh) {
                     W[l].trace = trace_slot("bvh", l, iter_no[l]);
                     k_bvh<<<light_grid, 128, 0, st[l]>>>(W[l]);
-                    if (ctx->profile) { cudaEventRecord(e[1], st[l]); cudaEventRecord(e[2], st[l]); cudaEventRecord(e[3], st[l]); }
+                    if (ctx->profile) { cudaEventRecord(e[1], st[l]); cudaEventRecord(e[2], st[l]); }
                     W[l].trace = trace_slot("shade", l, iter_no[l]);
                     k_shade<<<light_grid, light_block, 0, st[l]>>>(W[l]);
-                    if (ctx->profile) cudaEventRecord(e[4], st[l]);
-                    ctx->n_launches -= 2;
+                    if (ctx->profile) cudaEventRecord(e[3], st[l]);
+                    ctx->n_launches -= 1;
                 } else if (claims) {
                     W[l].trace = trace_slot("cull", l, iter_no[l]);
                     if (debug_sync) {
@@ -519,9 +505,6 @@
                     W[l].trace = trace_slot("refine", l, iter_no[l]);
                     k_refine<<<light_grid, light_block, 0, L.stage_stream>>>(W[l]);
                     if ((rc = dbg("wf_refine", l, enq[l]))) return rc;
-                    W[l].trace = trace_slot("tiebreak", l, iter_no[l]);
-                    wf_tiebreak<<<light_grid, light_block, 0, L.stage_stream>>>(W[l]);
-                    if ((rc = dbg("wf_tiebreak", l, enq[l]))) return rc;
                     W[l].trace = trace_slot("shade", l, iter_no[l]);
                     k_shade<<<light_grid, light_block, 0, L.stage_stream>>>(W[l]);
                     if ((rc = dbg("wf_shade", l, enq[l]))) return rc;
@@ -538,17 +521,14 @@
                     W[l].trace = trace_slot("refine", l, iter_no[l]);
                     k_refine<<<light_grid, light_block, 0, st[l]>>>(W[l]);
                     if (ctx->profile) cudaEventRecord(e[2], st[l]);
-                    W[l].trace = trace_slot("tiebreak", l, iter_no[l]);
-                    wf_tiebreak<<<light_grid, light_block, 0, st[l]>>>(W[l]);
-                    if (ctx->profile) cudaEventRecord(e[3], st[l]);
                     W[l].trace = trace_slot("shade", l, iter_no[l]);
                     k_shade<<<light_grid, light_block, 0, st[l]>>>(W[l]);
-                    if (ctx->profile) cudaEventRecord(e[4], st[l]);
+                    if (ctx->profile) cudaEventRecord(e[3], st[l]);
                 }
                 RT_CUDA(ctx, cudaGetLastError());
                 W[l].cur ^= 1;
                 ++iter_no[l];
-                ctx->n_launches += 4;
+                ctx->n_launches += 3;
                 ++enq[l];
                 progressed = true;
             }
@@ -599,10 +579,11 @@
     for (int l = 0; l < n_lanes; ++l) d.lanes[l].best_clean = true;
     if (ctx->profile) {
         RT_CUDA(ctx, cudaStreamSynchronize(stream));
-        for (size_t i = 0; i + 4 < evs.size(); i += 5)
-            for (int sgi = 0; sgi < 4; ++sgi) {
+        constexpr int kStage[3] = {0, 1, 3};
+        for (size_t i = 0; i + 3 < evs.size(); i += 4)
+            for (int sgi = 0; sgi < 3; ++sgi) {
                 float ms = 0.f;
-                if (cudaEventElapsedTime(&ms, evs[i + sgi], evs[i + sgi + 1]) == cudaSuccess) ctx->stage_ms[sgi] += ms;
+                if (cudaEventElapsedTime(&ms, evs[i + sgi], evs[i + sgi + 1]) == cudaSuccess) ctx->stage_ms[kStage[sgi]] += ms;
             }
         for (auto x : evs) cudaEventDestroy(x);
     }
@@ -1958,16 +1939,12 @@
         W.base.max_depth = 1;
         W.queue[0] = L.queue;
         W.queue[1] = L.queue + 3 * L.entries;
-        W.best_t = L.best;
-        W.best_key = L.best + L.entries;
+        W.best = L.best;
         W.pairs = L.pairs;
-        W.cands = L.cands;
-        W.cand_t = L.cand_t;
-        W.cand_count = L.cand_count;
         W.st = L.state;
         W.capacity = (int)L.entries;
         W.pair_cap = (unsigned)std::min<size_t>(L.entries * kPairsPerEntry, 0xfffffff0u);
-        wf_fill_best<<<d.sm_count * 4, 256, 0, d.stream>>>(L.best, L.best + L.entries, L.entries);
+        wf_fill_best<<<d.sm_count * 4, 256, 0, d.stream>>>(L.best, L.entries);
 #ifdef RT_TC_CHECK
         RT_CUDA(ctx, cudaMemsetAsync(L.pairs, 0xDD, (size_t)W.pair_cap * sizeof(uint2), d.stream));
 #endif
diff --git a/raytrace_clj_b200/csrc/rt_cull_tc.cuh b/raytrace_clj_b200/csrc/rt_cull_tc.cuh
--- a/raytrace_clj_b200/csrc/rt_cull_tc.cuh
+++ b/raytrace_clj_b200/csrc/rt_cull_tc.cuh
@@ -262,7 +262,7 @@
         const unsigned w = E.pos + __popc(bal & ((1u << lane) - 1u));
         TC_CHECK(entry < (unsigned)W.capacity && k < (unsigned)W.base.sc.n_list, "pair", entry, k);
         if (w < E.end) W.pairs[w] = make_uint2(entry, k);
-        else W.best_key[entry] = BEST_KEY_OVERFLOW;
+        else W.best[entry] = best_overflow();
     }
     E.pos = min(E.pos + total, E.end);
 }
@@ -287,7 +287,7 @@
             if (!tc_confirm(S, r0, r1, (unsigned)j * tc::TILE_N + cb * 64u + q, kk)) continue;
             const unsigned w = atomicAdd(&W.st->npairs, 1u);
             if (w < W.pair_cap) W.pairs[w] = make_uint2(entry, (unsigned)kk);
-            else W.best_key[entry] = BEST_KEY_OVERFLOW;
+            else W.best[entry] = best_overflow();
         }
 }
 
@@ -599,7 +599,7 @@
     unsigned long long lost = 0, surv = 0, cand = 0;
     if (idx < n) {
         const float4 a = W.queue[0][3 * (size_t)idx], b = W.queue[0][3 * (size_t)idx + 1];
-        const bool overflow = W.best_key[idx] == BEST_KEY_OVERFLOW;
+        const bool overflow = W.best[idx].y == BEST_KEY_OVERFLOW;
         for (int k = 0; k < sc.n_list; ++k) {
             const bool kept = overflow || ((mask[(size_t)idx * words + (k >> 5)] >> (k & 31)) & 1u);
             const double t = sc.generic ? refine_leaf<true>(&W.base.sc, k, a.x, a.y, a.z, b.x, b.y, b.z, a.w, tmin, tmax, false, make_uint2(0u, 0u), 0u, 0u, 0u)
diff --git a/raytrace_clj_b200/csrc/rt_kernels.cuh b/raytrace_clj_b200/csrc/rt_kernels.cuh
--- a/raytrace_clj_b200/csrc/rt_kernels.cuh
+++ b/raytrace_clj_b200/csrc/rt_kernels.cuh
@@ -358,12 +358,8 @@
 struct WaveParams {
     RenderParams base;
     float4* queue[2];
-    unsigned long long* best_t;
-    unsigned long long* best_key;
+    ulonglong2* best;
     uint2* pairs;
-    uint2* cands;
-    double* cand_t;
-    unsigned* cand_count;
     WaveState* st;
     int capacity;
     unsigned pair_cap;
@@ -394,6 +390,39 @@
 constexpr unsigned long long BEST_KEY_MISS = ~0ull;
 constexpr unsigned long long BEST_KEY_OVERFLOW = 0ull;
 constexpr unsigned PAIR_NULL = 0xffffffffu;
+__device__ __forceinline__ ulonglong2 best_reset() { return make_ulonglong2(BEST_T_INIT, BEST_KEY_MISS); }
+__device__ __forceinline__ ulonglong2 best_overflow() { return make_ulonglong2(0ull, BEST_KEY_OVERFLOW); }
+__device__ __forceinline__ bool best_below(ulonglong2 a, ulonglong2 b) { return a.x < b.x || (a.x == b.x && a.y < b.y); }
+__device__ __forceinline__ ulonglong2 best_cas(ulonglong2* p, ulonglong2 expect, ulonglong2 want) {
+    ulonglong2 old;
+    asm volatile("{ .reg .b128 e, n, o;\n\t"
+                 "mov.b128 e, {%2, %3};\n\t"
+                 "mov.b128 n, {%4, %5};\n\t"
+                 "atom.global.cas.b128 o, [%6], e, n;\n\t"
+                 "mov.b128 {%0, %1}, o; }"
+                 : "=l"(old.x), "=l"(old.y)
+                 : "l"(expect.x), "l"(expect.y), "l"(want.x), "l"(want.y), "l"(p)
+                 : "memory");
+    return old;
+}
+
+__device__ __forceinline__ void best_merge(ulonglong2* p, ulonglong2 seen, ulonglong2 want) {
+    for (;;) {
+        const ulonglong2 old = best_cas(p, seen, want);
+        if ((old.x == seen.x && old.y == seen.y) || !best_below(want, old)) return;
+        seen = old;
+    }
+}
+__device__ __forceinline__ ulonglong2 best_read(const ulonglong2* p) {
+    ulonglong2 v;
+    asm volatile("{ .reg .b128 o;\n\t"
+                 "ld.relaxed.gpu.global.b128 o, [%2];\n\t"
+                 "mov.b128 {%0, %1}, o; }"
+                 : "=l"(v.x), "=l"(v.y)
+                 : "l"(p)
+                 : "memory");
+    return v;
+}
 
 __device__ __forceinline__ unsigned warp_claim(unsigned* counter, bool pred, unsigned lane) {
     unsigned m = __ballot_sync(0xffffffffu, pred);
@@ -459,11 +488,8 @@
     *I.work_counter = I.total0;
     atomicAdd(&I.counters[DC_SAMPLES], I.total0);
 }
-__global__ void wf_fill_best(unsigned long long* best_t, unsigned long long* best_key, size_t n) {
-    for (size_t i = blockIdx.x * (size_t)blockDim.x + threadIdx.x; i < n; i += (size_t)gridDim.x * blockDim.x) {
-        best_t[i] = 0x7ff0000000000000ull;
-        best_key[i] = ~0ull;
-    }
+__global__ void wf_fill_best(ulonglong2* best, size_t n) {
+    for (size_t i = blockIdx.x * (size_t)blockDim.x + threadIdx.x; i < n; i += (size_t)gridDim.x * blockDim.x) best[i] = best_reset();
 }
 
 template <int R, int BLOCK>
@@ -475,7 +501,7 @@
     unsigned long long live;
     uint2* pairs;
     unsigned pair_cap;
-    unsigned long long* best_key;
+    ulonglong2* best;
     WaveState* st;
 
     __device__ __forceinline__ void flush(const uint32_t* list, unsigned long long nz, int count, int kbase) {
@@ -508,7 +534,7 @@
                 pairs[w] = make_uint2(entry(v), (unsigned)(kbase + k));
             } else {
                 if (w < pair_cap) pairs[w] = make_uint2(PAIR_NULL, 0u);
-                if (v < n) best_key[entry(v)] = BEST_KEY_OVERFLOW;
+                if (v < n) best[entry(v)] = best_overflow();
             }
             ++w;
         }
@@ -538,7 +564,7 @@
     sink.p0 = p0;
     sink.pairs = W.pairs;
     sink.pair_cap = W.pair_cap;
-    sink.best_key = W.best_key;
+    sink.best = W.best;
     sink.st = W.st;
     unsigned item = sc_.bid * warps + warp;
     const unsigned uniform_end = (n_items + warps - 1) / warps * warps;
@@ -651,15 +677,10 @@
 
 #include "rt_cull_tc.cuh"
 
-__device__ __forceinline__ unsigned wf_cand_region(const WaveParams& W, unsigned total_warps) {
-    return ((W.pair_cap + total_warps * 32u - 1u) / (total_warps * 32u)) * 32u;
-}
-
 template <bool GEN>
 __device__ __forceinline__ void wf_refine_body(const WaveParams& W, const DevScene* scp, Scope sc_, int cur) {
     const RenderParams& P = W.base;
     const unsigned npairs = min(W.st->npairs, W.pair_cap);
-    const unsigned lane = threadIdx.x & 31u;
     if (sc_.bid == 0 && threadIdx.x == 0) {
         W.st->batch = 0;
         W.st->cnt[cur ^ 1][0] = 0;
@@ -667,23 +688,30 @@
         atomicAdd(&P.counters[DC_CANDIDATES], (unsigned long long)(npairs - min(npairs, W.st->pad)));
         W.st->pad = 0;
     }
-    const unsigned total_warps = sc_.nblk * (blockDim.x >> 5);
-    const unsigned warp_id = sc_.bid * (blockDim.x >> 5) + (threadIdx.x >> 5);
-    const size_t region = (size_t)warp_id * wf_cand_region(W, total_warps);
-    unsigned cnt = 0;
+    const float4* qc = cur ? W.queue[1] : W.queue[0];
     const unsigned stride = sc_.nblk * blockDim.x;
-    const unsigned i_first = sc_.bid * blockDim.x + threadIdx.x;
-    uint2 pr_next = i_first < npairs ? W.pairs[i_first] : make_uint2(PAIR_NULL, 0u);
-    for (unsigned i0 = i_first - lane; i0 < npairs; i0 += stride) {
+    const unsigned lane = threadIdx.x & 31u;
+    unsigned i0 = sc_.bid * blockDim.x + threadIdx.x - lane;
+    uint2 pr_next = i0 + lane < npairs ? W.pairs[i0 + lane] : make_uint2(PAIR_NULL, 0u);
+    unsigned pend = 0;
+    ulonglong2 pend_seen = best_reset(), pend_want = best_reset();
+    bool pend_go = false;
+    for (; i0 < npairs; i0 += stride) {
         const uint2 pr = pr_next;
-        const unsigned i_next = i0 + lane + stride;
-        pr_next = i_next < npairs ? W.pairs[i_next] : make_uint2(PAIR_NULL, 0u);
-        bool cand = false;
+        pr_next = i0 + lane + stride < npairs ? W.pairs[i0 + lane + stride] : make_uint2(PAIR_NULL, 0u);
+        const bool real = pr.x != PAIR_NULL;
+        float4 a = make_float4(0.f, 0.f, 0.f, 0.f), b = a;
+        ulonglong2 seen = best_reset();
+        unsigned long long kk = BEST_KEY_MISS;
+        if (real) {
+            a = qc[3 * (size_t)pr.x];
+            b = qc[3 * (size_t)pr.x + 1];
+            seen = best_read(&W.best[pr.x]);
+            kk = (((unsigned long long)__ldg(&P.sc.tie_hi[pr.y])) << 32) | pr.y;
+        }
+        if (pend_go) best_merge(&W.best[pend], pend_seen, pend_want);
         double t = CUDART_INF;
-        if (pr.x != PAIR_NULL) {
-            const float4* qc = cur ? W.queue[1] : W.queue[0];
-            const float4 a = qc[3 * (size_t)pr.x], b = qc[3 * (size_t)pr.x + 1];
-            const unsigned long long seen = __ldcg(&W.best_t[pr.x]);
+        if (real) {
             if (!GEN) {
                 t = refine_candidate(P.sc.ex_c0r, P.sc.ex_c1, P.sc.ex_t0t1, P.sc.flags, (int)pr.y, a.x, a.y, a.z, b.x, b.y, b.z,
                                      a.w, 0.001, (double)FLT_MAX);
@@ -697,46 +725,28 @@
                 }
                 t = refine_leaf<true>(scp, (int)pr.y, a.x, a.y, a.z, b.x, b.y, b.z, a.w, 0.001, (double)FLT_MAX, true, P.key, pixq, smpq, bq);
             }
-            const unsigned long long tb = (unsigned long long)__double_as_longlong(t);
-            if (t < CUDART_INF && tb <= seen) {
-                atomicMin(&W.best_t[pr.x], tb);
-                cand = true;
-            }
-        }
-        const unsigned m = __ballot_sync(0xffffffffu, cand);
-        if (cand) {
-            const size_t slot = region + cnt + __popc(m & ((1u << lane) - 1u));
-            W.cands[slot] = pr;
-            W.cand_t[slot] = t;
-        }
-        cnt += __popc(m);
-    }
-    if (lane == 0) W.cand_count[warp_id] = cnt;
+        }
+        const ulonglong2 want = make_ulonglong2((unsigned long long)__double_as_longlong(t), kk);
+        bool go = t < CUDART_INF && best_below(want, seen);
+        const unsigned grp = __match_any_sync(0xffffffffu, go ? pr.x : 0x80000000u | lane);
+        if (go && grp != (1u << lane))
+            for (unsigned m = grp; m; m &= m - 1u) {
+                const int j = __ffs((int)m) - 1;
+                const ulonglong2 o = make_ulonglong2(__shfl_sync(grp, want.x, j), __shfl_sync(grp, want.y, j));
+                if (best_below(o, want)) go = false;
+            }
+        pend = pr.x;
+        pend_seen = seen;
+        pend_want = want;
+        pend_go = go;
+    }
+    if (pend_go) best_merge(&W.best[pend], pend_seen, pend_want);
 }
 template <bool GEN>
 __global__ void __launch_bounds__(256) wf_refine(const __grid_constant__ WaveParams W) {
     if (W.st->mode != MODE_RUN) return;
     TraceScope trace(W.trace);
     wf_refine_body<GEN>(W, &W.base.sc, grid_scope(), W.cur);
-}
-
-__device__ __forceinline__ void wf_tiebreak_body(const WaveParams& W, Scope sc_) {
-    const RenderParams& P = W.base;
-    const unsigned lane = threadIdx.x & 31u;
-    const unsigned total_warps = sc_.nblk * (blockDim.x >> 5);
-    const unsigned warp_id = sc_.bid * (blockDim.x >> 5) + (threadIdx.x >> 5);
-    const size_t region = (size_t)warp_id * wf_cand_region(W, total_warps);
-    const unsigned cnt = W.cand_count[warp_id];
-    for (unsigned j = lane; j < cnt; j += 32) {
-        const uint2 pr = W.cands[region + j];
-        if ((unsigned long long)__double_as_longlong(W.cand_t[region + j]) == W.best_t[pr.x])
-            atomicMin(&W.best_key[pr.x], (((unsigned long long)__ldg(&P.sc.tie_hi[pr.y])) << 32) | pr.y);
-    }
-}
-__global__ void __launch_bounds__(256) wf_tiebreak(const __grid_constant__ WaveParams W) {
-    if (W.st->mode != MODE_RUN) return;
-    TraceScope trace(W.trace);
-    wf_tiebreak_body(W, grid_scope());
 }
 
 template <bool GEN>
@@ -774,16 +784,16 @@
         float4 a, b, c;
         if (have) {
             a = qc[3 * (size_t)idx]; b = qc[3 * (size_t)idx + 1]; c = qc[3 * (size_t)idx + 2];
-            unsigned long long key = W.best_key[idx];
+            const ulonglong2 rec = W.best[idx];
+            unsigned long long key = rec.y;
             const uint32_t slot = __float_as_uint(b.w), sd = __float_as_uint(c.w);
             const uint32_t pix = rng_pixel(P, slot);
             const uint32_t smp = sd >> 8;
             const int depth = (int)(sd & 255u);
             const uint32_t bounce = (uint32_t)(P.max_depth - depth + 1);
             int k = (int)(unsigned)key;
-            double td = __longlong_as_double((long long)W.best_t[idx]);
-            W.best_key[idx] = BEST_KEY_MISS;
-            W.best_t[idx] = BEST_T_INIT;
+            double td = __longlong_as_double((long long)rec.x);
+            W.best[idx] = best_reset();
             if (key == BEST_KEY_OVERFLOW) {
                 exact_closest_hit<GEN>(scp, a.x, a.y, a.z, b.x, b.y, b.z, a.w, P.key, pix, smp, bounce, &td, &k);
                 key = k < 0 ? BEST_KEY_MISS : 1ull;
@@ -978,8 +988,7 @@
                                           rng_pixel(P, __float_as_uint(b.w)), sd >> 8, (uint32_t)(P.max_depth - (int)(sd & 255u) + 1));
         n_leaf += H.n_leaf; n_node += H.n_node;
         if (H.k >= 0) {
-            W.best_t[idx] = (unsigned long long)__double_as_longlong(H.t);
-            W.best_key[idx] = ((unsigned long long)H.tie << 32) | (unsigned)H.k;
+            W.best[idx] = make_ulonglong2((unsigned long long)__double_as_longlong(H.t), ((unsigned long long)H.tie << 32) | (unsigned)H.k);
         }
     }
     atomicAdd(&s_ctr[DC_CANDIDATES], n_leaf);
@@ -1147,18 +1156,12 @@
             s_st.mode = MODE_RUN;
             s_st.pad = 0;
         }
-        const unsigned warps = BLOCK / 32;
         WaveParams L = W;
         L.queue[0] = W.queue[0] + 3 * (size_t)first;
         L.queue[1] = W.queue[1] + 3 * (size_t)first;
-        L.best_t = W.best_t + first;
-        L.best_key = W.best_key + first;
+        L.best = W.best + first;
         L.pairs = W.pairs + (size_t)first * kPairsPerEntry;
         L.pair_cap = min(K, (unsigned)W.capacity - first) * kPairsPerEntry;
-        const size_t cand_slice = (size_t)wf_cand_region(L, warps) * warps;
-        L.cands = W.cands + (size_t)blockIdx.x * cand_slice;
-        L.cand_t = W.cand_t + (size_t)blockIdx.x * cand_slice;
-        L.cand_count = W.cand_count + blockIdx.x * warps;
         L.st = &s_st;
         L.status = nullptr;
         L.capacity = (int)K;
@@ -1192,15 +1195,10 @@
 #ifdef RT_TAIL_DIAG
             unsigned long long dt2 = global_timer_ns();
 #endif
-            wf_tiebreak_body(L, solo);
-            __syncthreads();
-#ifdef RT_TAIL_DIAG
-            unsigned long long dt3 = global_timer_ns();
-#endif
             wf_shade_body<GEN>(L, &W.base.sc, solo, cur, s_ctr);
 #ifdef RT_TAIL_DIAG
             __syncthreads();
-            if (diag) printf("tail cta %u n %u pairs %u: cull %llu refine %llu tie %llu shade %llu ns\n", blockIdx.x, n, np_, dt1 - dt0, dt2 - dt1, dt3 - dt2, global_timer_ns() - dt3);
+            if (diag) printf("tail cta %u n %u pairs %u: cull %llu refine %llu shade %llu ns\n", blockIdx.x, n, np_, dt1 - dt0, dt2 - dt1, global_timer_ns() - dt2);
 #endif
             cur ^= 1;
         }
```
